# miguelmartin75/txt2vid

Measured on AMD Instinct MI355X. Metric: TGANv2 GAN train throughput (G+D steps x global batch), 16x64x64 videos/sec, higher is better.
Workload: dtype f32; 1 GPU; BASELINE configs[1]: unconditional TGANv2 16x64x64x1, per-GPU batch 32, fp32, RSGAN + GP 0.5, Adam 2e-4 (0.5,0.999), 1 D + 1 G step, subsample_input pyramid 8/16/32/64; global_batch=32, per_gpu_batch=32, parallelism=dp1

## Files before the change

include/t2v_hip.h:

```cpp
#ifndef T2V_HIP_H
#define T2V_HIP_H

#include <stddef.h>
#include <stdint.h>

#ifdef __cplusplus
extern "C" {
#endif

#define T2V_OK 0
#define T2V_EINVAL (-1)
#define T2V_ELAUNCH (-2)

#define T2V_MAX_TAPS 27

typedef struct {
    int32_t N, Cin, D, H, W, Cout;
    int32_t ntaps;
    int8_t dz[T2V_MAX_TAPS], dy[T2V_MAX_TAPS], dx[T2V_MAX_TAPS];
    int8_t pad_[3];
} t2v_conv_geom;

#define T2V_MAX_GROUPS 8
typedef struct {
    const float* x;
    float* y;
    const float* mask;
    int32_t N, D, H, W;
    int32_t ntaps;
    int32_t dstride;
    int32_t ydstride;
    int32_t yoff, Dy;
    int8_t dz[T2V_MAX_TAPS], dy[T2V_MAX_TAPS], dx[T2V_MAX_TAPS], widx[T2V_MAX_TAPS];
} t2v_conv_group;

#define T2V_CONV_BIAS 1
#define T2V_CONV_RELU_IN 2
#define T2V_CONV_ACCUM 4
#define T2V_CONV_ACCUM_BIAS 16
#define T2V_CONV_BF16 32
#define T2V_CONV_MASK_OUT 8

int t2v_pack_weight(const float* w, float* wp, int Cout, int Cin, int T, const int32_t* taps, int ntaps,
                    int mode, void* stream);

int t2v_pack_weight_into(const float* w, float* wp, int Cout, int Cin, int T, const int32_t* taps, int ntaps,
                         int mode, int dst_rows, int dst_cols, int row_off, int col_off, void* stream);

typedef struct {
    const float* src;
    float* dst;
    int32_t Cout, Cin, T, ntaps, mode, dst_rows, dst_cols, row_off, col_off;
    int32_t block_begin;
    int32_t bx, by;
    int8_t taps[T2V_MAX_TAPS];
    int8_t pad_[5];
} t2v_pack_job;
int t2v_pack_job_bytes(void);
int t2v_pack_job_groups(int T, int ntaps, int mode);
int t2v_pack_multi(const void* table , int njobs, int total_blocks, void* stream);

int t2v_conv_fwd(const float* x, const float* wp, const float* bias, float* y, float* ws, const t2v_conv_geom* g,
                 int flags, void* stream);
int64_t t2v_conv_fwd_ws_floats(const t2v_conv_geom* g);

int64_t t2v_conv_wgrad_slab_floats(const t2v_conv_geom* g, int T);
int t2v_conv_wgrad(const float* x, const float* gy, float* dw, float* slab, const t2v_conv_geom* g,
                   const int32_t* taps, int T, int flags, void* stream);

int64_t t2v_conv_fwd_grouped_ws_floats(const t2v_conv_group* groups, int ngroups, int Cin, int Cout);
int t2v_conv_fwd_grouped(const t2v_conv_group* groups, int ngroups, int Cin, int Cout, const float* wp,
                         const float* bias, float* ws, int flags, void* stream);
int64_t t2v_conv_wgrad_grouped_slab_floats(const t2v_conv_group* groups, int ngroups, int Cin, int Cout, int kD,
                                           int kH, int kW);
int t2v_conv_wgrad_grouped(const t2v_conv_group* groups, int ngroups, int Cin, int Cout, int kD, int kH, int kW,
                           float* dw, float* slab, int flags, void* stream);
#define T2V_WGRAD_MAX_SRC 6
typedef struct {
    const float* slab;
    const float* bias_slab;
    int32_t ntaps, S;
    int8_t map[T2V_MAX_TAPS];
    int8_t pad_[5];
    int64_t tap_stride;
    int64_t split_stride;
} t2v_wgrad_src;
typedef struct {
    float* dw;
    float* dbias;
    int64_t CoCi;
    int32_t T, Cout, nsrc;
    int32_t accum, accum_bias;
    int32_t kind;
    int32_t block_begin, nblocks;
    int32_t tap_major;
    int32_t pad_;
    t2v_wgrad_src src[T2V_WGRAD_MAX_SRC];
} t2v_wgrad_dest;
int t2v_conv_wgrad_grouped_partial(const t2v_conv_group* groups, int ngroups, int Cin, int Cout, int kD, int kH, int kW,
                                   float* slab, int want_bias, int flags, t2v_wgrad_src* out_src, void* stream);
int t2v_wgrad_dest_bytes(void);
int t2v_wgrad_reduce_multi(const void* table , int ndest, int total_blocks, void* stream);

int t2v_conv_fwd_plan(const t2v_conv_group* groups, int ngroups, int Cin, int Cout, int flags, int32_t* out);
int t2v_conv_wgrad_plan(const t2v_conv_group* groups, int ngroups, int Cin, int Cout, int kD, int kH, int kW, int32_t* out);
int64_t t2v_conv_wgrad_grouped_bias_slab_floats(const t2v_conv_group* groups, int ngroups, int Cin, int Cout, int kD,
                                                int kH, int kW);
int t2v_conv_wgrad_grouped_bias(const t2v_conv_group* groups, int ngroups, int Cin, int Cout, int kD, int kH, int kW,
                                float* dw, float* dbias, float* slab, int flags, void* stream);

int t2v_pack_weight_bf16(const float* w, void* wpb, int Cout, int Cin, int T, const int32_t* taps, int ntaps, int mode, void* stream);
int t2v_conv_fwd_grouped_bf16_ok(const t2v_conv_group* groups, int ngroups, int Cin, int Cout);
int t2v_conv_fwd_bf16_plan(const t2v_conv_group* groups, int ngroups, int Cin, int Cout, int flags, int32_t* out);
int t2v_conv_fwd_grouped_bf16(const t2v_conv_group* groups, int ngroups, int Cin, int Cout, const void* wpb, const float* bias,
                              float* ws, int flags, void* stream);

int64_t t2v_channel_sum_ws_floats(int N, int C, int64_t S);
int t2v_channel_sum(const float* x, float* out, float* ws, int N, int C, int64_t S, int accum, void* stream);
int64_t t2v_channel_sum_grouped_ws_floats(const t2v_conv_group* groups, int ngroups, int C);
int t2v_channel_sum_grouped(const t2v_conv_group* groups, int ngroups, int C, float* out, float* ws, int accum, void* stream);

int t2v_relu(const float* x, float* y, int64_t n, void* stream);
int t2v_relu_mask(const float* g, const float* x, float* gx, int64_t n, void* stream);
int t2v_add(const float* a, const float* b, float* y, int64_t n, void* stream);
int t2v_axpby(float alpha, const float* a, float beta, const float* b, float* y, int64_t n, void* stream);
int t2v_fill(float* y, float v, int64_t n, void* stream);
int t2v_tanh(const float* x, float* y, int64_t n, void* stream);
int t2v_tanh_bwd(const float* g, const float* y, float* gx, int64_t n, void* stream);

int t2v_avgpool3d(const float* x, const float* x2, float* y, int NC, int D, int H, int W, int Do, int Ho, int Wo,
                  const int32_t k[3], const int32_t s[3], const int32_t p[3], void* stream);
int t2v_avgpool3d_bwd(const float* gy, float* gx, int NC, int D, int H, int W, int Do, int Ho, int Wo,
                      const int32_t k[3], const int32_t s[3], const int32_t p[3], void* stream);
typedef struct t2v_pool_job {
    const float* x; const float* x2; float* y;
    const float* add;
    int32_t NC, D, H, W, Do, Ho, Wo;
    int32_t k[3], s[3], p[3];
} t2v_pool_job;
int t2v_avgpool3d_multi(const t2v_pool_job* jobs, int njobs, void* stream);
int t2v_avgpool3d_bwd_multi(const t2v_pool_job* jobs, int njobs, void* stream);

int t2v_rowsum(const float* x, float* y, int64_t rows, int64_t S, void* stream);
int t2v_rowbcast(const float* g, float* gx, int64_t rows, int64_t S, void* stream);

int t2v_upsample2x(const float* x, float* y, int64_t planes, int H, int W, void* stream);
int t2v_upsample2x_bwd(const float* gy, float* gx, int64_t planes, int H, int W, void* stream);
int t2v_upsample2x_add(const float* x, const float* h, float* y, int64_t planes, int H, int W, void* stream);

int64_t t2v_bn_ws_floats(int N, int C, int64_t S);
int t2v_bn_plan(int N, int C, int64_t S, int32_t* out );
int t2v_bn_stats(const float* x, float* stats, float* running_mean, float* running_var, float* ws, int N, int C,
                 int64_t S, float momentum, float eps, void* stream);
int t2v_bn_apply(const float* x, const float* stats, const float* gamma, const float* beta, float* y,
                 int N, int C, int64_t S, int relu, void* stream);
// ... 281 lines not shown
```

txt2vid_amd/_lib.py:

```python
import ctypes as C
import os

_HERE = os.path.dirname(os.path.abspath(__file__))
LIB_PATH = os.environ.get('T2V_LIB') or os.path.join(_HERE, 'csrc', 'libt2v_hip.so')

MAX_TAPS = 27


class ConvGeom(C.Structure):
    _fields_ = [('N', C.c_int32), ('Cin', C.c_int32), ('D', C.c_int32), ('H', C.c_int32), ('W', C.c_int32),
                ('Cout', C.c_int32), ('ntaps', C.c_int32),
                ('dz', C.c_int8 * MAX_TAPS), ('dy', C.c_int8 * MAX_TAPS), ('dx', C.c_int8 * MAX_TAPS),
                ('pad_', C.c_int8 * 3)]


class ConvGroup(C.Structure):
    _fields_ = [('x', C.c_void_p), ('y', C.c_void_p), ('mask', C.c_void_p), ('N', C.c_int32), ('D', C.c_int32), ('H', C.c_int32), ('W', C.c_int32),
                ('ntaps', C.c_int32), ('dstride', C.c_int32), ('ydstride', C.c_int32), ('yoff', C.c_int32), ('Dy', C.c_int32),
                ('dz', C.c_int8 * MAX_TAPS), ('dy', C.c_int8 * MAX_TAPS), ('dx', C.c_int8 * MAX_TAPS), ('widx', C.c_int8 * MAX_TAPS)]


class AdamJob(C.Structure):
    _fields_ = [('p', C.c_void_p), ('g', C.c_void_p), ('m', C.c_void_p), ('v', C.c_void_p), ('n', C.c_int64)]

# ... 11 lines not shown


class PoolJob(C.Structure):
    _fields_ = [('x', C.c_void_p), ('x2', C.c_void_p), ('y', C.c_void_p), ('add', C.c_void_p), ('NC', C.c_int32), ('D', C.c_int32), ('H', C.c_int32),
                ('W', C.c_int32), ('Do', C.c_int32), ('Ho', C.c_int32), ('Wo', C.c_int32), ('k', C.c_int32 * 3), ('s', C.c_int32 * 3),
                ('p', C.c_int32 * 3)]


class PoolBoxJob(C.Structure):
    _fields_ = [('in_', C.c_void_p), ('mask', C.c_void_p), ('out', C.c_void_p), ('bias', C.c_void_p), ('NC', C.c_int32), ('D', C.c_int32),
                ('H', C.c_int32), ('W', C.c_int32), ('tmode', C.c_int32), ('relu', C.c_int32), ('scale', C.c_float), ('C', C.c_int32)]


class MultiJob(C.Structure):
    _fields_ = [('a', C.c_void_p), ('b', C.c_void_p), ('c', C.c_void_p), ('out', C.c_void_p), ('out2', C.c_void_p), ('n', C.c_int64),
                ('d0', C.c_int32), ('d1', C.c_int32), ('d2', C.c_int32), ('f0', C.c_int32), ('f1', C.c_int32), ('reserved', C.c_int32)]


class PackJob(C.Structure):
    _fields_ = [('src', C.c_void_p), ('dst', C.c_void_p), ('Cout', C.c_int32), ('Cin', C.c_int32), ('T', C.c_int32),
                ('ntaps', C.c_int32), ('mode', C.c_int32), ('dst_rows', C.c_int32), ('dst_cols', C.c_int32),
                ('row_off', C.c_int32), ('col_off', C.c_int32), ('block_begin', C.c_int32), ('bx', C.c_int32), ('by', C.c_int32),
                ('taps', C.c_int8 * MAX_TAPS), ('pad_', C.c_int8 * 5)]


WGRAD_MAX_SRC = 6


class WgradSrc(C.Structure):
    _fields_ = [('slab', C.c_void_p), ('bias_slab', C.c_void_p), ('ntaps', C.c_int32), ('S', C.c_int32),
                ('map', C.c_int8 * MAX_TAPS), ('pad_', C.c_int8 * 5), ('tap_stride', C.c_int64), ('split_stride', C.c_int64)]


class WgradDest(C.Structure):
    _fields_ = [('dw', C.c_void_p), ('dbias', C.c_void_p), ('CoCi', C.c_int64), ('T', C.c_int32), ('Cout', C.c_int32),
                ('nsrc', C.c_int32), ('accum', C.c_int32), ('accum_bias', C.c_int32), ('kind', C.c_int32),
                ('block_begin', C.c_int32), ('nblocks', C.c_int32), ('tap_major', C.c_int32), ('pad_', C.c_int32),
                ('src', WgradSrc * WGRAD_MAX_SRC)]


class AugMember(C.Structure):
    _fields_ = [('x', C.c_void_p), ('y', C.c_void_p), ('u', C.c_void_p), ('N', C.c_int32), ('C', C.c_int32), ('T', C.c_int32),
                ('S', C.c_int32), ('row_stride', C.c_int32), ('rows', C.c_int32), ('policy', C.c_int32), ('reserved', C.c_int32)]


class AdaLevel(C.Structure):
    _fields_ = [('real', C.c_void_p), ('fake', C.c_void_p), ('count', C.c_int32), ('reserved', C.c_int32)]


class LecamGrad(C.Structure):
    _fields_ = [('real', C.c_void_p), ('fake', C.c_void_p), ('d_real', C.c_void_p), ('d_fake', C.c_void_p), ('count', C.c_int32),
                ('reserved', C.c_int32)]


class ProjMember(C.Structure):
    _fields_ = [('g', C.c_void_p), ('f', C.c_void_p), ('s', C.c_void_p), ('base', C.c_void_p), ('out', C.c_void_p), ('b', C.c_int32),
                ('reserved', C.c_int32)]


class MbstdMember(C.Structure):
    _fields_ = [('f', C.c_void_p), ('g', C.c_void_p * 2), ('base', C.c_void_p * 2), ('gam', C.c_void_p), ('y', C.c_void_p * 2),
                ('stat', C.c_void_p), ('out', C.c_void_p), ('b', C.c_int32), ('seg', C.c_int32)]


MAX_GROUPS = 8
_P = C.c_void_p
_I = C.c_int
_L = C.c_int64
_F = C.c_float
_I3 = C.POINTER(C.c_int32)
_G = C.POINTER(ConvGeom)

SIGNATURES = {
    't2v_pack_weight': [_P, _P, _I, _I, _I, _I3, _I, _I, _P],
    't2v_pack_job_bytes': [],
    't2v_pack_multi': [_P, _I, _I, _P],
    't2v_pack_job_groups': [_I, _I, _I],
    't2v_pack_weight_into': [_P, _P, _I, _I, _I, _I3, _I, _I, _I, _I, _I, _I, _P],
    't2v_conv_fwd': [_P, _P, _P, _P, _P, _G, _I, _P],
    't2v_conv_fwd_ws_floats': [_G],
    't2v_conv_wgrad_slab_floats': [_G, _I],
    't2v_conv_fwd_grouped_ws_floats': [_P, _I, _I, _I],
    't2v_conv_fwd_grouped': [_P, _I, _I, _I, _P, _P, _P, _I, _P],
    't2v_conv_wgrad_grouped_slab_floats': [_P, _I, _I, _I, _I, _I, _I],
    't2v_conv_fwd_plan': [_P, _I, _I, _I, _I, _I3],
    't2v_nonlocal_ok': [_I, _I],
    't2v_nonlocal_fwd': [_P, _P, _P, _P, _P, _I, _I, _I, _I, _I, _P],
    't2v_nonlocal_bwd': [_P, _P, _P, _P, _P, _P, _P, _P, _P, _P, _I, _I, _I, _I, _I, _P],
    't2v_conv_wgrad_grouped_partial': [_P, _I, _I, _I, _I, _I, _I, _P, _I, _I, _P, _P],
    't2v_wgrad_dest_bytes': [],
    't2v_wgrad_reduce_multi': [_P, _I, _I, _P],
    't2v_conv_wgrad_plan': [_P, _I, _I, _I, _I, _I, _I, _I3],
    't2v_pack_weight_bf16': [_P, _P, _I, _I, _I, _P, _I, _I, _P],
    't2v_conv_fwd_grouped_bf16_ok': [_P, _I, _I, _I],
    't2v_conv_fwd_bf16_plan': [_P, _I, _I, _I, _I, _I3],
    't2v_conv_fwd_grouped_bf16': [_P, _I, _I, _I, _P, _P, _P, _I, _P],
    't2v_conv_wgrad_grouped': [_P, _I, _I, _I, _I, _I, _I, _P, _P, _I, _P],
    't2v_conv_wgrad_grouped_bias_slab_floats': [_P, _I, _I, _I, _I, _I, _I],
    't2v_conv_wgrad_grouped_bias': [_P, _I, _I, _I, _I, _I, _I, _P, _P, _P, _I, _P],
    't2v_conv_wgrad': [_P, _P, _P, _P, _G, _I3, _I, _I, _P],
    't2v_channel_sum_ws_floats': [_I, _I, _L],
    't2v_channel_sum': [_P, _P, _P, _I, _I, _L, _I, _P],
    't2v_channel_sum_grouped_ws_floats': [_P, _I, _I],
    't2v_channel_sum_grouped': [_P, _I, _I, _P, _P, _I, _P],
    't2v_relu': [_P, _P, _L, _P],
    't2v_relu_mask': [_P, _P, _P, _L, _P],
    't2v_add': [_P, _P, _P, _L, _P],
    't2v_axpby': [_F, _P, _F, _P, _P, _L, _P],
    't2v_fill': [_P, _F, _L, _P],
    't2v_tanh': [_P, _P, _L, _P],
    't2v_tanh_bwd': [_P, _P, _P, _L, _P],
    't2v_avgpool3d': [_P, _P, _P, _I, _I, _I, _I, _I, _I, _I, _I3, _I3, _I3, _P],
    't2v_avgpool3d_bwd': [_P, _P, _I, _I, _I, _I, _I, _I, _I, _I3, _I3, _I3, _P],
    't2v_avgpool3d_multi': [_P, _I, _P],
    't2v_avgpool3d_bwd_multi': [_P, _I, _P],
    't2v_rowsum': [_P, _P, _L, _L, _P],
    't2v_rowbcast': [_P, _P, _L, _L, _P],
    't2v_upsample2x': [_P, _P, _L, _I, _I, _P],
    't2v_upsample2x_bwd': [_P, _P, _L, _I, _I, _P],
    't2v_upsample2x_add': [_P, _P, _P, _L, _I, _I, _P],
    't2v_rsgan_mean_multi': [_P, _I, _P, _P],
    't2v_rsgan_mean_multi_bwd': [_P, _I, _P, _P],
    't2v_bn_ws_floats': [_I, _I, _L],
    't2v_bn_plan': [_I, _I, _L, _I3],
    't2v_bn_stats': [_P, _P, _P, _P, _P, _I, _I, _L, _F, _F, _P],
    't2v_bn_apply': [_P, _P, _P, _P, _P, _I, _I, _L, _I, _P],
    't2v_bn_bwd': [_P, _P, _P, _P, _P, _P, _P, _P, _P, _I, _I, _L, _I, _P],
    't2v_bn_train_fwd': [_P, _P, _P, _P, _P, _P, _P, _P, _I, _I, _L, _F, _F, _I, _P, _P],
    't2v_bn_train_bwd': [_P, _P, _P, _P, _P, _P, _P, _P, _P, _I, _I, _L, _I, _P],
    't2v_bn_train_fwd_up': [_P, _P, _P, _P, _P, _P, _P, _P, _I, _I, _I, _I, _F, _F, _I, _P, _P],
    't2v_bn_train_bwd_up': [_P, _P, _P, _P, _P, _P, _P, _P, _P, _I, _I, _I, _I, _I, _P],
    't2v_bn_train_bwd_add': [_P, _P, _P, _P, _P, _P, _P, _P, _P, _P, _I, _I, _I, _I, _I, _I, _P],
    't2v_bn_eval': [_P, _P, _P, _P, _P, _P, _I, _I, _L, _F, _I, _P],
    't2v_cbn_ws_floats': [_I, _I, _L],
    't2v_cbn_train_fwd': [_P] * 9 + [_I] * 9 + [_F, _F, _I, _P, _P],
    't2v_cbn_train_fwd_up': [_P] * 9 + [_I] * 9 + [_F, _F, _I, _P, _P],
    't2v_cbn_train_bwd': [_P] * 11 + [_I] * 9 + [_I, _P],
    't2v_cbn_train_bwd_up': [_P] * 11 + [_I] * 9 + [_I, _P],
    't2v_cbn_train_bwd_add': [_P] * 12 + [_I] * 9 + [_I, _I, _P],
    't2v_cbn_eval': [_P] * 7 + [_I] * 9 + [_F, _I, _P],
    't2v_lstm_gates': [_P, _P, _P, _P, _P, _I, _L, _P],
    't2v_lstm_gates_bwd': [_P, _P, _P, _P, _P, _P, _P, _I, _L, _P],
    't2v_skinny_gemm_splits': [_I, _I, _I],
    't2v_skinny_gemm_slab': [_P, _P, _P, _I, _I, _I, _P],
    't2v_lstm_gates_slab': [_P, _I, _P, _P, _P, _P, _P, _I, _I, _P],
    't2v_lstm_gates_bwd_slab': [_P, _P, _I, _P, _P, _P, _P, _P, _P, _I, _I, _P],
    't2v_concat4': [_P, _P, _P, _P, _P, _I, _P],
    't2v_lstm_step_fused_ok': [_I, _I, _I],
    't2v_lstm_pack_major': [_P, _P, _I, _I, _P],
    't2v_lstm_step_fused': [_P, _P, _P, _P, _P, _P, _P, _I, _I, _I, _P],
    't2v_lstm_step_bwd_fused': [_P, _P, _P, _P, _P, _P, _P, _P, _P, _I, _I, _P],
    't2v_lstm_pack_cols': [_P, _P, _I, _I, _P],
    't2v_bmm': [_P, _P, _P, _I, _I, _I, _I, _I, _I, _I, _P],
    't2v_lstm_seq_step': [_P, _L, _P, _P, _P, _P, _P, _P, _L, _P, _I, _I, _I, _P],
    't2v_lstm_seq_step2': [_P, _P, _L, _L, _P, _I, _I, _P],
    't2v_lstm_train_step': [_P, _L, _P, _P, _L, _P, _L, _P, _L, _P, _L, _P, _L, _P, _L, _P, _I, _I, _I, _P],
    't2v_lstm_train_step_bwd': [_P, _L, _P, _L, _I, _P, _P, _P, _P, _L, _P, _L, _P, _L, _P, _L, _P, _I, _I, _I, _I, _I, _P],
    't2v_embedding_bwd': [_P, _P, _P, _L, _I, _I, _P],
    't2v_xent_fwd': [_P, _P, _P, _P, _L, _I, _P],
    't2v_xent_bwd': [_P, _P, _P, _P, _P, _L, _I, _P],
    't2v_argmax_rows': [_P, _P, _L, _I, _P],
    't2v_multi_ws_floats': [_I, _P, _I],
    't2v_multi': [_I, _P, _I, _P, _P, _P],
    't2v_rsgan': [_P, _P, _P, _I, _P],
    't2v_rsgan_bwd': [_P, _P, _P, _P, _P, _I, _P],
    't2v_gan_loss': [_P, _P, _P, _I, _I, _I, _I, _F, _P],
# ... 104 lines not shown
```

txt2vid_amd/csrc/conv.hip:

```cpp
#include <hip/hip_runtime.h>
#include <stdint.h>
#include "../../include/t2v_hip.h"

typedef float f32x16 __attribute__((ext_vector_type(16)));

#ifdef T2V_STAMPS
__device__ unsigned long long* g_stamps = nullptr;
__device__ unsigned int g_stamps_cap = 0;
extern "C" int t2v_stamps_set(void* buf, unsigned int cap_records) {
    if (hipMemcpyToSymbol(HIP_SYMBOL(g_stamps), &buf, sizeof(buf)) != hipSuccess) return -1;
    if (hipMemcpyToSymbol(HIP_SYMBOL(g_stamps_cap), &cap_records, sizeof(cap_records)) != hipSuccess) return -1;
    return 0;
}
__device__ __forceinline__ unsigned long long stamp_now() {
    unsigned long long t;
    __builtin_amdgcn_sched_barrier(0);
    asm volatile("s_memtime %0\n\ts_waitcnt lgkmcnt(0)" : "=s"(t) :: "memory");
    __builtin_amdgcn_sched_barrier(0);
    return t;
}
#define STAMP(v) const unsigned long long v = stamp_now()
#define STAMP_ACC(acc, a, b) acc += (b) - (a)
#else
#define STAMP(v)
// ... 206 lines not shown
    }
}

__global__ __launch_bounds__(256) void pack_weight_kernel(const float* __restrict__ w, void* __restrict__ wp,
                                                          int Cout, int Cin, int T, TapList taps, int mode, int dst_rows,
                                                          int dst_cols, int row_off, int col_off) {
    __shared__ float lds[32 * PK_PITCH];
    __shared__ int s_taps[T2V_MAX_TAPS];
    if ((int)threadIdx.x < taps.n) s_taps[threadIdx.x] = taps.t[threadIdx.x];
    __syncthreads();
    const int bx = (Cin + 31) / 32, by = (Cout + 31) / 32;
    const int b = blockIdx.x;
    pack_tile(lds, w, wp, Cout, Cin, T, taps.n, s_taps, mode, dst_rows, dst_cols, row_off, col_off, b % bx, (b / bx) % by, b / (bx * by));
}

extern "C" int t2v_pack_weight_into(const float* w, float* wp, int Cout, int Cin, int T, const int32_t* taps, int ntaps,
                                    int mode, int dst_rows, int dst_cols, int row_off, int col_off, void* stream) {
    if (!w || !wp || ntaps < 1 || ntaps > T2V_MAX_TAPS || T > T2V_MAX_TAPS || row_off < 0 || col_off < 0) return T2V_EINVAL;
    if ((mode & ~8) != 0 && (mode & ~8) != 1) return T2V_EINVAL;
    const int rows = (mode & 7) ? Cout : Cin, cols = (mode & 7) ? Cin : Cout;
    if (row_off + rows > dst_rows || col_off + cols > dst_cols) return T2V_EINVAL;
    TapList tl;
    tl.n = ntaps;
    for (int i = 0; i < ntaps; ++i) {
        if (taps[i] < 0 || taps[i] >= T) return T2V_EINVAL;
        tl.t[i] = taps[i];
    }
    const long nb = (long)((Cin + 31) / 32) * ((Cout + 31) / 32) * pack_job_groups(T, ntaps, mode);
    if (nb > 0x7fffffffL) return T2V_EINVAL;
    T2V_LAUNCH(pack_weight_kernel, dim3((unsigned)nb), dim3(256), 0, (hipStream_t)stream, w, (void*)wp, Cout, Cin, T, tl, mode, dst_rows,
               dst_cols, row_off, col_off);
    return launch_status();
}

extern "C" int t2v_pack_weight(const float* w, float* wp, int Cout, int Cin, int T, const int32_t* taps, int ntaps,
                               int mode, void* stream) {
    return t2v_pack_weight_into(w, wp, Cout, Cin, T, taps, ntaps, mode, (mode & 7) ? Cout : Cin, (mode & 7) ? Cin : Cout, 0, 0, stream);
}


struct PackJob {
    const float* src;
    float* dst;
    int32_t Cout, Cin, T, ntaps, mode, dst_rows, dst_cols, row_off, col_off, block_begin, bx, by;
    int8_t taps[T2V_MAX_TAPS];
    int8_t pad_[5];
};

__global__ __launch_bounds__(256) void pack_multi_kernel(const PackJob* __restrict__ table, int njobs) {
    __shared__ float lds[32 * PK_PITCH];
    __shared__ PackJob job;
    if (threadIdx.x == 0) {
        int lo = 0, hi = njobs - 1;
        while (lo < hi) {
            const int mid = (lo + hi + 1) >> 1;
            if (table[mid].block_begin <= (int)blockIdx.x) lo = mid; else hi = mid - 1;
        }
        job = table[lo];
    }
    __syncthreads();
    const int b = (int)blockIdx.x - __builtin_amdgcn_readfirstlane(job.block_begin);
    const int bx = __builtin_amdgcn_readfirstlane(job.bx), by = __builtin_amdgcn_readfirstlane(job.by);
    const int bxi = b % bx, byi = (b / bx) % by, z = b / (bx * by);
    pack_tile(lds, job.src, job.dst, __builtin_amdgcn_readfirstlane(job.Cout), __builtin_amdgcn_readfirstlane(job.Cin),
              __builtin_amdgcn_readfirstlane(job.T), __builtin_amdgcn_readfirstlane(job.ntaps), job.taps,
              __builtin_amdgcn_readfirstlane(job.mode), job.dst_rows, job.dst_cols, job.row_off, job.col_off, bxi, byi, z);
}

extern "C" int t2v_pack_job_bytes(void) { return (int)sizeof(PackJob); }

extern "C" int t2v_pack_multi(const void* table, int njobs, int total_blocks, void* stream) {
    if (!table || njobs < 1 || total_blocks < 1) return T2V_EINVAL;
    T2V_LAUNCH(pack_multi_kernel, dim3((unsigned)total_blocks), dim3(256), 0, (hipStream_t)stream, (const PackJob*)table, njobs);
    return launch_status();
}

struct GroupTable {
    t2v_conv_group g[T2V_MAX_GROUPS];
    int32_t tile_start[T2V_MAX_GROUPS + 1];
    int64_t out_start[T2V_MAX_GROUPS + 1];
    int32_t n;
};

template <int NCO, int NM, int WCO, int WM>
__device__ __forceinline__ void igemm_epilogue(f32x16 (&acc)[NCO][NM], const GroupTable& tab, const int gi, const t2v_conv_group& gd,
                                               const float* __restrict__ bias, float* __restrict__ slab, const int Cout,
                                               const int flags, const int nsplit, const int m0, const int co0, const int M,
                                               const int DHW, const int wm, const int wco, const int l31, const int hi,
                                               const int yds = 1, const int yoff = 0, const int DHWy = 0, const int HW = 1) {
    const bool split = nsplit > 1;
    const bool has_bias = !split && (flags & T2V_CONV_BIAS) && bias != nullptr;
    const bool accum = !split && (flags & T2V_CONV_ACCUM);
    const bool mask_out = !split && (flags & T2V_CONV_MASK_OUT) && gd.mask != nullptr;
    float* out = split ? slab + (size_t)blockIdx.z * (size_t)tab.out_start[tab.n] + (size_t)tab.out_start[gi] : gd.y;
#pragma unroll
    for (int j = 0; j < NM; ++j) {
        const int m = m0 + wm * WM + j * 32 + l31;
        if (m >= M) continue;
        const int n = m / DHW;
        int sp = m - n * DHW;
        int cs = DHW;
        if (yds == 2) {
            const int e = sp / HW;
            sp += (e + yoff) * HW;
            cs = DHWy;
        }
        float* py = out + (size_t)n * Cout * cs + sp;
        if (mask_out) {
            const float* pm = gd.mask + (size_t)n * Cout * cs + sp;
#pragma unroll
            for (int i = 0; i < NCO; ++i) {
                float mv[16];
#pragma unroll
                for (int r = 0; r < 16; ++r) {
                    const int co = co0 + wco * WCO + i * 32 + (r & 3) + 8 * (r >> 2) + 4 * hi;
                    mv[r] = pm[(size_t)(co < Cout ? co : Cout - 1) * cs];
                }
#pragma unroll
                for (int r = 0; r < 16; ++r) {
                    const int co = co0 + wco * WCO + i * 32 + (r & 3) + 8 * (r >> 2) + 4 * hi;
                    const float v = acc[i][j][r] + (has_bias ? bias[co < Cout ? co : 0] : 0.f);
                    if (co < Cout) py[(size_t)co * cs] = mv[r] > 0.f ? v : 0.f;
                }
            }
        } else if (!accum) {
#pragma unroll
            for (int i = 0; i < NCO; ++i) {
#pragma unroll
                for (int r = 0; r < 16; ++r) {
                    const int co = co0 + wco * WCO + i * 32 + (r & 3) + 8 * (r >> 2) + 4 * hi;
                    if (co < Cout) py[(size_t)co * cs] = acc[i][j][r] + (has_bias ? bias[co] : 0.f);
                }
            }
        } else {
#pragma unroll
            for (int i = 0; i < NCO; ++i) {
#pragma unroll
                for (int r = 0; r < 16; ++r) {
                    const int co = co0 + wco * WCO + i * 32 + (r & 3) + 8 * (r >> 2) + 4 * hi;
                    if (co < Cout) py[(size_t)co * cs] += acc[i][j][r] + (has_bias ? bias[co] : 0.f);
                }
            }
        }
    }
}


template <int BM, int BN, int WAVES_CO, int BKT, bool FAST, bool VECB>
__global__ __launch_bounds__(256) void conv_igemm_kernel(const GroupTable tab, const float* __restrict__ wp,
                                                         const float* __restrict__ bias, float* __restrict__ slab,
                                                         const int Cin, const int Cout, const int flags, const int nsplit) {
    constexpr int WAVES_M = 4 / WAVES_CO;
    constexpr int WCO = BN / WAVES_CO;
    constexpr int WM = BM / WAVES_M;
    constexpr int NCO = WCO / 32, NM = WM / 32;
    constexpr int LA = BKT * BM / 256;
    constexpr int KSA = 256 / BM;
    constexpr int LB = BKT * BN / 256;
    constexpr int KSB = 256 / BN;
    constexpr int NV = BKT * BN / 4;
    constexpr int LBV = NV >= 256 ? NV / 256 : 1;
    constexpr int KSBV = 1024 / BN;
    static_assert(NCO >= 1 && NM >= 1 && LA >= 1 && LB >= 1, "tile");

    __shared__ __attribute__((aligned(16))) float As[2 * BKT * BM];
    __shared__ __attribute__((aligned(16))) float Bs[2 * BKT * BN];
    __shared__ int s_off[T2V_MAX_TAPS];
    __shared__ int s_widx[T2V_MAX_TAPS];

    const int tid = threadIdx.x;
    const int lane = tid & 63, wave = tid >> 6;
    const int l31 = lane & 31, hi = lane >> 5;
    const int wco = wave % WAVES_CO, wm = wave / WAVES_CO;

    const int tile = xcd_remap((int)blockIdx.x, (int)gridDim.x);
    int gi = 0;
#pragma unroll
    for (int k = 1; k < T2V_MAX_GROUPS; ++k)
        if (k < tab.n && tile >= tab.tile_start[k]) gi = k;
    const t2v_conv_group& gd = tab.g[gi];
    const float* __restrict__ x = gd.x;
    const int D = gd.D, H = gd.H, W = gd.W;
    const int HW = H * W, DHW = D * HW;
    const int M = gd.N * DHW;
    const int m0 = (tile - tab.tile_start[gi]) * BM, co0 = blockIdx.y * BN;
    const int ntaps = gd.ntaps;

    const int lane_t = lane < ntaps ? lane : 0;
    const int tab_tdz = gd.dz[lane_t], tab_tdy = gd.dy[lane_t], tab_tdx = gd.dx[lane_t];
    if (tid < ntaps) {
        s_off[tid] = tab_tdz * HW + tab_tdy * W + tab_tdx;
        s_widx[tid] = gd.widx[tid];
    }

    const int ma_l = tid % BM, ka_l = tid / BM;
    const int m_a = m0 + ma_l;
    uint32_t tapmask = 0;
    size_t xbase = 0;
    if (m_a < M) {
        int n = m_a / DHW, sp = m_a - n * DHW;
        int d = sp / HW, r = sp - d * HW;
        int h = r / W, w_ = r - h * W;
        xbase = (size_t)n * Cin * DHW + sp;
        for (int t = 0; t < ntaps; ++t) {
            int dd = d + __builtin_amdgcn_readlane(tab_tdz, t), hh = h + __builtin_amdgcn_readlane(tab_tdy, t),
                ww = w_ + __builtin_amdgcn_readlane(tab_tdx, t);
            if ((unsigned)dd < (unsigned)D && (unsigned)hh < (unsigned)H && (unsigned)ww < (unsigned)W) tapmask |= 1u << t;
        }
    }
    const int cob_l = tid % BN, kb_l = tid / BN;
    const int cv_l = (tid % (BN / 4)) * 4, kv_l = tid / (BN / 4);
    const bool vact = (NV >= 256) || (tid < NV);
    const bool co_ok = VECB ? (vact && (co0 + cv_l) < Cout) : (co0 + cob_l) < Cout;
    const bool relu_in = flags & T2V_CONV_RELU_IN;

    f32x16 acc[NCO][NM];
#pragma unroll
    for (int i = 0; i < NCO; ++i)
#pragma unroll
        for (int j = 0; j < NM; ++j)
#pragma unroll
            for (int r = 0; r < 16; ++r) acc[i][j][r] = 0.f;

    float ra[LA];
    float rb[VECB ? 1 : LB];
    float4 rbv[VECB ? LBV : 1];
    const int Ktot = ntaps * Cin;
    const int nchunks = FAST ? ntaps * (Cin / BKT) : (Ktot + BKT - 1) / BKT;
    const int cps = (nchunks + nsplit - 1) / nsplit;
    const int q0 = blockIdx.z * cps;
    int q1 = q0 + cps;
    if (q1 > nchunks) q1 = nchunks;
    __syncthreads();

// ... 19 lines not shown
                for (int j = 0; j < LB; ++j) rb[j] = pw[(size_t)j * KSB * Cout];
            }
        } else {
            pend_a = 0;
#pragma unroll
            for (int j = 0; j < LA; ++j) {
                const int kk = q * BKT + ka_l + j * KSA;
                const int kc = kk < Ktot ? kk : Ktot - 1;
                const int tt = kc / Cin, ci = kc - tt * Cin;
                const bool v = kk < Ktot && ((tapmask >> tt) & 1u);
                pend_a |= (v ? 1u : 0u) << j;
                const ptrdiff_t off = v ? (ptrdiff_t)s_off[tt] : 0;
                ra[j] = x[xbase + off + (size_t)ci * DHW];
            }
#pragma unroll
            for (int j = 0; j < LB; ++j) {
                const int kk = q * BKT + kb_l + j * KSB;
                const int kc = kk < Ktot ? kk : Ktot - 1;
                const int tt = kc / Cin, ci = kc - tt * Cin;
                rb[j] = wp[((size_t)s_widx[tt] * Cin + ci) * Cout + (co_ok ? co0 + cob_l : 0)];
            }
        }
    };

    int t_cur = 0, c_cur = 0;
    if (FAST) {
        const int cpt = Cin / BKT;
        t_cur = q0 / cpt;
        c_cur = (q0 - t_cur * cpt) * BKT;
    }
    auto advance = [&]() {
        c_cur += BKT;
        if (FAST && c_cur >= Cin) { c_cur = 0; ++t_cur; }
    };
    auto stage = [&](int b) {
        float* as = As + b * (BKT * BM);
        float* bs = Bs + b * (BKT * BN);
#pragma unroll
        for (int j = 0; j < LA; ++j) {
            float val = ((pend_a >> j) & 1u) ? ra[j] : 0.f;
            as[(ka_l + j * KSA) * BM + ma_l] = relu_in ? fmaxf(val, 0.f) : val;
        }
        if (VECB) {
#pragma unroll
            for (int j = 0; j < LBV; ++j)
                if (vact) *reinterpret_cast<float4*>(&bs[(kv_l + j * KSBV) * BN + cv_l]) = co_ok ? rbv[j] : make_float4(0.f, 0.f, 0.f, 0.f);
        } else {
#pragma unroll
            for (int j = 0; j < LB; ++j) bs[(kb_l + j * KSB) * BN + cob_l] = co_ok ? rb[j] : 0.f;
        }
    };
    int cur = 0;
    if (q0 < q1) {
        load_chunk(q0, t_cur, c_cur);
        stage(0);
        __syncthreads();
        if (q0 + 1 < q1) { advance(); load_chunk(q0 + 1, t_cur, c_cur); }
    }
    for (int q = q0; q < q1; ++q) {
        const float* as = As + cur * (BKT * BM);
        const float* bs = Bs + cur * (BKT * BN);
        __builtin_amdgcn_s_setprio(1);
#pragma unroll
        for (int k2 = 0; k2 < BKT / 2; ++k2) {
            float a[NCO], b[NM];
            const int krow = k2 * 2 + hi;
#pragma unroll
            for (int i = 0; i < NCO; ++i) a[i] = bs[krow * BN + wco * WCO + i * 32 + l31];
#pragma unroll
            for (int j = 0; j < NM; ++j) b[j] = as[krow * BM + wm * WM + j * 32 + l31];
#pragma unroll
            for (int i = 0; i < NCO; ++i)
#pragma unroll
                for (int j = 0; j < NM; ++j)
                    acc[i][j] = __builtin_amdgcn_mfma_f32_32x32x2f32(a[i], b[j], acc[i][j], 0, 0, 0);
        }
        __builtin_amdgcn_s_setprio(0);
        if (q + 1 < q1 && !dbg_nostage) stage(cur ^ 1);
        __syncthreads();
        if (q + 2 < q1) { advance(); load_chunk(q + 2, t_cur, c_cur); }
        cur ^= 1;
    }

    igemm_epilogue<NCO, NM, WCO, WM>(acc, tab, gi, gd, bias, slab, Cout, flags, nsplit, m0, co0, M, DHW, wm, wco, l31, hi);
}

template <int BM, int BN, int WAVES_CO, int BKT, bool VECB>
__global__ __launch_bounds__(256) void conv_igemm_strip_kernel(const GroupTable tab, const float* __restrict__ wp,
                                                               const float* __restrict__ bias, float* __restrict__ slab,
                                                               const int Cin, const int Cout, const int flags, const int nsplit) {
    constexpr int WAVES_M = 4 / WAVES_CO;
    constexpr int WCO = BN / WAVES_CO;
    constexpr int WM = BM / WAVES_M;
    constexpr int NCO = WCO / 32, NM = WM / 32;
    constexpr int AP = BM + 4;
    constexpr int LA = BKT * BM / 256;
    constexpr int KSA = 256 / BM;
    constexpr int LB = BKT * BN / 256;
    constexpr int KSB = 256 / BN;
    constexpr int NV = BKT * BN / 4;
    constexpr int LBV = NV >= 256 ? NV / 256 : 1;
    constexpr int KSBV = 1024 / BN;
    static_assert(NCO >= 1 && NM >= 1 && LA >= 1 && LB >= 1 && 2 * BKT <= 256, "tile");

    __shared__ __attribute__((aligned(16))) float As[2 * BKT * AP];
    __shared__ __attribute__((aligned(16))) float Bs[2 * BKT * BN];

    const int tid = threadIdx.x;
    const int lane = tid & 63, wave = tid >> 6;
    const int l31 = lane & 31, hi = lane >> 5;
    const int wco = wave % WAVES_CO, wm = (wave / WAVES_CO) % WAVES_M;

    const int tile = xcd_remap((int)blockIdx.x, (int)gridDim.x);
    int gi = 0;
#pragma unroll
    for (int k = 1; k < T2V_MAX_GROUPS; ++k)
        if (k < tab.n && tile >= tab.tile_start[k]) gi = k;
    const t2v_conv_group& gd = tab.g[gi];
    const int D = gd.D, H = gd.H, W = gd.W;
    const int HW = H * W, DHW = D * HW;
    const int M = gd.N * DHW;
    const int m0 = (tile - tab.tile_start[gi]) * BM, co0 = blockIdx.y * BN;
    const int ntaps = gd.ntaps;
    const int ndx = gd.dx[0] < 0 ? 3 : 1;
    const int nrow = ntaps / ndx;

    const int lane_r = lane < nrow ? lane : 0, lane_t = lane < ntaps ? lane : 0;
    const int tab_rdz = gd.dz[lane_r * ndx], tab_rdy = gd.dy[lane_r * ndx];
    const int tab_roff = (tab_rdz * HW + tab_rdy * W) * 4;
    const int tab_widx = gd.widx[lane_t];
    const __amdgpu_buffer_rsrc_t rx = __builtin_amdgcn_make_buffer_rsrc((void*)gd.x, 0, (int)((uint32_t)M * (uint32_t)Cin * 4u), 0x00020000);
    const __amdgpu_buffer_rsrc_t rw = __builtin_amdgcn_make_buffer_rsrc((void*)wp, 0, -1, 0x00020000);

    const int ma_l = tid % BM, ka_l = tid / BM;
    const int he = tid / BKT, hk = tid % BKT;
    const bool halo_thread = tid < 2 * BKT;
    uint32_t rowmask = 0, rowmask_h = 0;
    uint32_t xbase = 0, xbase_h = 0;
    {
        const int m_a = m0 + ma_l;
        if (m_a < M) {
            const int n = m_a / DHW, sp = m_a - n * DHW;
            const int d = sp / HW, r = sp - d * HW;
            const int h = r / W;
            xbase = (uint32_t)n * (uint32_t)Cin * (uint32_t)DHW + (uint32_t)sp;
            for (int t = 0; t < nrow; ++t) {
                const int dd = d + __builtin_amdgcn_readlane(tab_rdz, t), hh = h + __builtin_amdgcn_readlane(tab_rdy, t);
                if ((unsigned)dd < (unsigned)D && (unsigned)hh < (unsigned)H) rowmask |= 1u << t;
            }
        }
        const int m_h = he ? m0 + BM : m0 - 1;
        if (halo_thread && m_h >= 0 && m_h < M) {
            const int n = m_h / DHW, sp = m_h - n * DHW;
            const int d = sp / HW, r = sp - d * HW;
            const int h = r / W;
            xbase_h = (uint32_t)n * (uint32_t)Cin * (uint32_t)DHW + (uint32_t)sp;
            for (int t = 0; t < nrow; ++t) {
                const int dd = d + __builtin_amdgcn_readlane(tab_rdz, t), hh = h + __builtin_amdgcn_readlane(tab_rdy, t);
                if ((unsigned)dd < (unsigned)D && (unsigned)hh < (unsigned)H) rowmask_h |= 1u << t;
            }
        }
    }
    bool can_l[NM], can_r[NM];
#pragma unroll
    for (int j = 0; j < NM; ++j) {
        const int m = m0 + wm * WM + j * 32 + l31;
        const int w_ = m % W;
        can_l[j] = w_ > 0;
        can_r[j] = w_ < W - 1;
    }
    const int cob_l = tid % BN, kb_l = tid / BN;
    const int cv_l = (tid % (BN / 4)) * 4, kv_l = tid / (BN / 4);
    const bool vact = (NV >= 256) || (tid < NV);
// ... 42 lines not shown
                ra[j] = __builtin_bit_cast(float, __builtin_amdgcn_raw_buffer_load_b32(rx, vo, sx + j * (KSA * 4) * DHW, 0));
            if (halo_thread) {
                pend_hv = (rowmask_h >> r_cur) & 1u;
                rah = __builtin_bit_cast(float, __builtin_amdgcn_raw_buffer_load_b32(rx, xoff_h + (pend_hv ? (uint32_t)roff : 0u), sx, 0));
            }
        }
        const int t = r_cur * ndx + d_cur;
        const int sw = (__builtin_amdgcn_readlane(tab_widx, t) * Cin + c0) * Cout * 4;
        if (VECB) {
#pragma unroll
            for (int j = 0; j < LBV; ++j)
                rbv[j] = __builtin_bit_cast(float4, __builtin_amdgcn_raw_buffer_load_b128(rw, woff, sw + j * (KSBV * 4) * Cout, 0));
        } else {
#pragma unroll
            for (int j = 0; j < LB; ++j)
                rb[j] = __builtin_bit_cast(float, __builtin_amdgcn_raw_buffer_load_b32(rw, woff, sw + j * (KSB * 4) * Cout, 0));
        }
    };
    auto stage = [&](int ab, int bb) {
        if (pend_has_a) {
            float* as = As + ab * (BKT * AP);
#pragma unroll
            for (int j = 0; j < LA; ++j) {
                as[(ka_l + j * KSA) * AP + 1 + ma_l] = pend_av ? fmaxf(ra[j], relu_floor) : 0.f;
            }
            if (halo_thread) {
                as[hk * AP + (he ? BM + 1 : 0)] = pend_hv ? fmaxf(rah, relu_floor) : 0.f;
            }
        }
        float* bs = Bs + bb * (BKT * BN);
        if (VECB) {
#pragma unroll
            for (int j = 0; j < LBV; ++j)
                if (vact) *reinterpret_cast<float4*>(&bs[(kv_l + j * KSBV) * BN + cv_l]) = co_ok ? rbv[j] : make_float4(0.f, 0.f, 0.f, 0.f);
        } else {
#pragma unroll
            for (int j = 0; j < LB; ++j) bs[(kb_l + j * KSB) * BN + cob_l] = co_ok ? rb[j] : 0.f;
        }
    };

    int acur = 0, bcur = 0, dx_now = 0;
    if (q0 < q1) {
        load_chunk(true);
        stage(0, 0);
        dx_now = pend_dx;
        __syncthreads();
        if (q0 + 1 < q1) { advance(); load_chunk(false); }
    }
    for (int q = q0; q < q1; ++q) {
        const float* as = As + acur * (BKT * AP) + 1 + dx_now + wm * WM + l31;
        const float* bs = Bs + bcur * (BKT * BN) + wco * WCO + l31;
        bool keep[NM];
#pragma unroll
        for (int j = 0; j < NM; ++j) keep[j] = dx_now < 0 ? can_l[j] : (dx_now > 0 ? can_r[j] : true);
        __builtin_amdgcn_s_setprio(1);
#pragma unroll
        for (int k2 = 0; k2 < BKT / 2; ++k2) {
            float a[NCO], b[NM];
            const int krow = k2 * 2 + hi;
#pragma unroll
            for (int i = 0; i < NCO; ++i) a[i] = bs[krow * BN + i * 32];
#pragma unroll
            for (int j = 0; j < NM; ++j) {
                const float v = as[krow * AP + j * 32];
                b[j] = keep[j] ? v : 0.f;
            }
#pragma unroll
            for (int i = 0; i < NCO; ++i)
#pragma unroll
                for (int j = 0; j < NM; ++j)
                    acc[i][j] = __builtin_amdgcn_mfma_f32_32x32x2f32(a[i], b[j], acc[i][j], 0, 0, 0);
        }
        __builtin_amdgcn_s_setprio(0);
        const bool more = q + 1 < q1;
        const bool next_a = more && pend_has_a;
        int dx_next = dx_now;
        if (more) { stage(acur ^ 1, bcur ^ 1); dx_next = pend_dx; }
        __syncthreads();
        if (q + 2 < q1) { advance(); load_chunk(false); }
        bcur ^= 1;
        if (next_a) acur ^= 1;
        dx_now = dx_next;
    }
    igemm_epilogue<NCO, NM, WCO, WM>(acc, tab, gi, gd, bias, slab, Cout, flags, nsplit, m0, co0, M, DHW, wm, wco, l31, hi);
}

#ifndef DB_STAGE_LATE
#define DB_STAGE_LATE 1
#endif
template <int BM, int BKT, int WAVES_CO, bool VECB, bool DB = false>
__global__ __launch_bounds__(256, ((BM == 256 || (DB && BKT == 32)) ? 2 : (DB ? 4 : 3))) void conv_igemm_strip3_kernel(const GroupTable tab, const float* __restrict__ wp,
                                                                const float* __restrict__ bias, float* __restrict__ slab,
                                                                const int Cin, const int Cout, const int flags, const int nsplit) {
#ifdef T2V_STAMPS
    const unsigned long long t_real = __builtin_amdgcn_s_memrealtime();
#endif
    STAMP(t_entry);
    constexpr int BN = 64, WAVES_M = 4 / WAVES_CO;
    constexpr int WCO = BN / WAVES_CO, WM = BM / WAVES_M;
    constexpr int NCO = WCO / 32, NM = WM / 32;
    constexpr int AP = BM + 4;
    constexpr int LA = BKT * BM / 256;
    constexpr int KSA = 256 / BM;
    constexpr int NV = BKT * BN / 4;
    constexpr int LBV = NV / 256;
    constexpr int KSBV = 1024 / BN;
    constexpr int LB = BKT * BN / 256;
    constexpr int KSB = 256 / BN;
    static_assert(NCO >= 1 && NM >= 1 && LA >= 1 && LBV >= 1 && 2 * BKT <= 256, "tile");

    __shared__ __attribute__((aligned(16))) float As[(DB ? 2 : 1) * BKT * AP];
    __shared__ __attribute__((aligned(16))) float Bs[(DB ? 2 : 1) * 3 * BKT * BN];

    const int tid = threadIdx.x;
    const int lane = tid & 63, wave = tid >> 6;
    const int l31 = lane & 31, hi = lane >> 5;
    const int wco = wave % WAVES_CO, wm = wave / WAVES_CO;

    const int tile = xcd_remap((int)blockIdx.x, (int)gridDim.x);
    int gi = 0;
#pragma unroll
    for (int k = 1; k < T2V_MAX_GROUPS; ++k)
        if (k < tab.n && tile >= tab.tile_start[k]) gi = k;
    const t2v_conv_group& gd = tab.g[gi];
    const int D = gd.D, H = gd.H, W = gd.W;
    const int HW = H * W, DHW = D * HW;
    const int ds = gd.dstride == 2 ? 2 : 1;
    const int yds = gd.ydstride == 2 ? 2 : 1;
    const int Do = yds == 2 ? (gd.Dy + 1 - gd.yoff) / 2 : (ds == 2 ? (D + 1) / 2 : D);
    const int DHWo = Do * HW;
    const int M = gd.N * DHWo;
    const int m0 = (tile - tab.tile_start[gi]) * BM, co0 = blockIdx.y * BN;
    const int ntaps = gd.ntaps;
    const int ndx = gd.dx[0] < 0 ? 3 : 1;
    const int nrow = ntaps / ndx;

    const int lane_r = lane < nrow ? lane : 0, lane_t = lane < ntaps ? lane : 0;
    const int tab_rdz = gd.dz[lane_r * ndx], tab_rdy = gd.dy[lane_r * ndx];
    const int tab_roff = (tab_rdz * HW + tab_rdy * W) * 4;
    const int tab_widx = gd.widx[lane_t];
    const __amdgpu_buffer_rsrc_t rx = __builtin_amdgcn_make_buffer_rsrc((void*)gd.x, 0, (int)((uint32_t)(gd.N * DHW) * (uint32_t)Cin * 4u), 0x00020000);
    const __amdgpu_buffer_rsrc_t rw = __builtin_amdgcn_make_buffer_rsrc((void*)wp, 0, -1, 0x00020000);

    const int ma_l = tid % BM, ka_l = tid / BM;
    const int he = tid / BKT, hk = tid % BKT;
    const bool halo_thread = tid < 2 * BKT;
    uint32_t rowmask = 0, rowmask_h = 0;
    uint32_t xbase = 0, xbase_h = 0;
    {
        const int m_a = m0 + ma_l;
        if (m_a < M) {
            const int n = m_a / DHWo, spo = m_a - n * DHWo;
            const int d_o = spo / HW, r = spo - d_o * HW;
            const int d = d_o * ds, sp = d * HW + r;
            const int h = r / W;
            xbase = (uint32_t)n * (uint32_t)Cin * (uint32_t)DHW + (uint32_t)sp;
            for (int t = 0; t < nrow; ++t) {
                const int dd = d + __builtin_amdgcn_readlane(tab_rdz, t), hh = h + __builtin_amdgcn_readlane(tab_rdy, t);
                if ((unsigned)dd < (unsigned)D && (unsigned)hh < (unsigned)H) rowmask |= 1u << t;
            }
        }
        const int m_h = he ? m0 + BM : m0 - 1;
        if (halo_thread && m_h >= 0 && m_h < M) {
            const int n = m_h / DHWo, spo = m_h - n * DHWo;
            const int d_o = spo / HW, r = spo - d_o * HW;
            const int d = d_o * ds, sp = d * HW + r;
            const int h = r / W;
            xbase_h = (uint32_t)n * (uint32_t)Cin * (uint32_t)DHW + (uint32_t)sp;
            for (int t = 0; t < nrow; ++t) {
                const int dd = d + __builtin_amdgcn_readlane(tab_rdz, t), hh = h + __builtin_amdgcn_readlane(tab_rdy, t);
                if ((unsigned)dd < (unsigned)D && (unsigned)hh < (unsigned)H) rowmask_h |= 1u << t;
            }
        }
    }
    bool can_l[NM], can_r[NM];
#pragma unroll
// ... 47 lines not shown
            l_sx[st] = c0 * DHW * 4;
            pav[st] = (rowmask >> r_cur) & 1u;
            phv[st] = halo_thread && ((rowmask_h >> r_cur) & 1u);
            l_vo[st] = xoff + (pav[st] ? (uint32_t)roff : 0u);
            l_vh[st] = xoff_hd + (phv[st] ? (uint32_t)roff : 0u);
#pragma unroll
            for (int d = 0; d < 3; ++d) l_sw[st][d] = (__builtin_amdgcn_readlane(tab_widx, r_cur * 3 + d) * Cin + c0) * Cout * 4;
        };
        auto load_item = [&](int st, int i) {
            if (i < LA) ra2[st][i] = __builtin_bit_cast(float, __builtin_amdgcn_raw_buffer_load_b32(rx, l_vo[st], l_sx[st] + i * (KSA * 4) * DHW, 0));
            else if (i == LA) rah2[st] = __builtin_bit_cast(float, __builtin_amdgcn_raw_buffer_load_b32(rx, l_vh[st], l_sx[st], 0));
            else if (i < LA + 1 + 3 * LBV) {
                const int e = i - LA - 1, d = e / LBV, j = e - d * LBV;
                rb2[st][e] = __builtin_bit_cast(float4, __builtin_amdgcn_raw_buffer_load_b128(rw, woff, l_sw[st][d] + j * (KSBV * 4) * Cout, 0));
            }
        };
        auto stage_item = [&](int st, float* A, float* B, int i) {
            if (i < LA) A[(ka_l + i * KSA) * AP + 1 + ma_l] = pav[st] ? fmaxf(ra2[st][i], relu_floor) : 0.f;
            else if (i == LA) A[halo_row * AP + halo_col] = phv[st] ? fmaxf(rah2[st], relu_floor) : 0.f;
            else if (i < LA + 1 + 3 * LBV) {
                const int e = i - LA - 1, d = e / LBV, j = e - d * LBV;
                *reinterpret_cast<float4*>(&B[d * (BKT * BN) + (kv_l + j * KSBV) * BN + cv_l]) = co_ok ? rb2[st][e] : make_float4(0.f, 0.f, 0.f, 0.f);
            }
        };
        const float* a_tap[3][NM];
#pragma unroll
        for (int d = 0; d < 3; ++d)
#pragma unroll
            for (int j = 0; j < NM; ++j) {
                const bool keep = d == 0 ? can_l[j] : (d == 2 ? can_r[j] : true);
                a_tap[d][j] = keep ? As + d + wm * WM + j * 32 + l31 : As + (BM + 3);
            }
        auto round = [&](auto CUR, int q) {
            constexpr int cur = decltype(CUR)::value, nxt = cur ^ 1;
            prep(cur, q + 2);
            const float* Ab = As + cur * ASZ;
            const float* Bb = Bs + cur * BSZ + wco * WCO + l31;
            float* An = As + nxt * ASZ;
            float* Bn = Bs + nxt * BSZ;
#pragma unroll
            for (int d = 0; d < 3; ++d) {
#pragma unroll
                for (int k2 = 0; k2 < BKT / 2; ++k2) {
                    const int krow = k2 * 2 + hi, slot = d * (BKT / 2) + k2;
                    float a[NCO], b[NM];
#pragma unroll
                    for (int i = 0; i < NCO; ++i) a[i] = Bb[d * (BKT * BN) + krow * BN + i * 32];
#pragma unroll
                    for (int j = 0; j < NM; ++j) b[j] = (a_tap[d][j] + cur * ASZ)[krow * AP];
#pragma unroll
                    for (int i = 0; i < NCO; ++i)
#pragma unroll
                        for (int j = 0; j < NM; ++j) acc[i][j] = __builtin_amdgcn_mfma_f32_32x32x2f32(a[i], b[j], acc[i][j], 0, 0, 0);
                    constexpr int SS = DB_STAGE_LATE ? NSLOT - HS : HS;
#pragma unroll
                    for (int e = 0; e < IPS; ++e) {
                        if (slot < HS) load_item(cur, slot * IPS + e);
                        else if (slot >= SS && slot < SS + HS) stage_item(nxt, An, Bn, (slot - SS) * IPS + e);
                    }
                    if (slot == HS - 1 || slot == SS - 1 || slot == SS + HS - 1) __builtin_amdgcn_sched_barrier(0);
                }
            }
            (void)Ab;
            __syncthreads();
        };
        if (tid < BKT) { As[tid * AP + BM + 3] = 0.f; As[ASZ + tid * AP + BM + 3] = 0.f; }
        if (q0 < q1) {
            prep(0, q0);
#pragma unroll
            for (int i = 0; i < NI; ++i) load_item(0, i);
            prep(1, q0 + 1);
#pragma unroll
            for (int i = 0; i < NI; ++i) load_item(1, i);
#pragma unroll
            for (int i = 0; i < NI; ++i) stage_item(0, As, Bs, i);
        }
        __syncthreads();
        __builtin_amdgcn_s_setprio(1);
        for (int q = q0; q < q1; q += 2) {
            round(std::integral_constant<int, 0>{}, q);
            if (q + 1 < q1) round(std::integral_constant<int, 1>{}, q + 1);
        }
        __builtin_amdgcn_s_setprio(0);
        igemm_epilogue<NCO, NM, WCO, WM>(acc, tab, gi, gd, bias, slab, Cout, flags, nsplit, m0, co0, M, DHWo, wm, wco, l31, hi, yds, gd.yoff,
                                         gd.Dy * HW, HW);
        return;
    }
    float ra[LA], rah = 0.f;
    float rb[VECB ? 1 : 3 * LB];
    float4 rbv[VECB ? 3 * LBV : 1];
    const int ncb = Cin / BKT;
    const int nrounds = nrow * ncb;
    const int rps = (nrounds + nsplit - 1) / nsplit;
    const int q0 = blockIdx.z * rps;
    int q1 = q0 + rps;
    if (q1 > nrounds) q1 = nrounds;
    bool pend_av = false, pend_hv = false;

    auto load_round = [&](int q) {
        const int r_cur = q / ncb, cb = q - r_cur * ncb;
        const int c0 = cb * BKT;
        const int roff = __builtin_amdgcn_readlane(tab_roff, r_cur);
        const int sx = c0 * DHW * 4;
        pend_av = (rowmask >> r_cur) & 1u;
        const uint32_t vo = xoff + (pend_av ? (uint32_t)roff : 0u);
#pragma unroll
        for (int j = 0; j < LA; ++j)
            ra[j] = __builtin_bit_cast(float, __builtin_amdgcn_raw_buffer_load_b32(rx, vo, sx + j * (KSA * 4) * DHW, 0));
        if (halo_thread) {
            pend_hv = (rowmask_h >> r_cur) & 1u;
            rah = __builtin_bit_cast(float, __builtin_amdgcn_raw_buffer_load_b32(rx, xoff_h + (pend_hv ? (uint32_t)roff : 0u), sx, 0));
        }
#pragma unroll
        for (int d = 0; d < 3; ++d) {
            if (d < ndx) {
                const int sw = (__builtin_amdgcn_readlane(tab_widx, r_cur * ndx + d) * Cin + c0) * Cout * 4;
                if (VECB) {
#pragma unroll
                    for (int j = 0; j < LBV; ++j)
                        rbv[d * LBV + j] = __builtin_bit_cast(float4, __builtin_amdgcn_raw_buffer_load_b128(rw, woff, sw + j * (KSBV * 4) * Cout, 0));
                } else {
#pragma unroll
                    for (int j = 0; j < LB; ++j)
                        rb[d * LB + j] = __builtin_bit_cast(float, __builtin_amdgcn_raw_buffer_load_b32(rw, woff, sw + j * (KSB * 4) * Cout, 0));
                }
            }
        }
    };
    auto stage = [&]() {
#pragma unroll
        for (int j = 0; j < LA; ++j) As[(ka_l + j * KSA) * AP + 1 + ma_l] = pend_av ? fmaxf(ra[j], relu_floor) : 0.f;
        if (halo_thread) As[hk * AP + (he ? BM + 1 : 0)] = pend_hv ? fmaxf(rah, relu_floor) : 0.f;
#pragma unroll
        for (int d = 0; d < 3; ++d) {
            if (d < ndx) {
                float* bs = Bs + d * (BKT * BN);
                if (VECB) {
#pragma unroll
                    for (int j = 0; j < LBV; ++j)
                        *reinterpret_cast<float4*>(&bs[(kv_l + j * KSBV) * BN + cv_l]) = co_ok ? rbv[d * LBV + j] : make_float4(0.f, 0.f, 0.f, 0.f);
                } else {
#pragma unroll
                    for (int j = 0; j < LB; ++j) bs[(kb_l + j * KSB) * BN + cob_l] = co_ok ? rb[d * LB + j] : 0.f;
                }
            }
        }
    };

    if (tid < BKT) As[tid * AP + BM + 3] = 0.f;
    if (q0 < q1) load_round(q0);
#ifdef T2V_STAMPS
    unsigned long long st_stage = 0, st_bar1 = 0, st_load = 0, st_mfma = 0, st_bar2 = 0;
#endif
#ifdef T2V_ABLATION
    const bool ab_noload = flags & 64, ab_nostage = flags & 128, ab_nobar = flags & 256, ab_nomfma = flags & 512, ab_nostore = flags & 1024;
#else
    constexpr bool ab_noload = false, ab_nostage = false, ab_nobar = false, ab_nomfma = false, ab_nostore = false;
#endif
    STAMP(t_loop0);
    for (int q = q0; q < q1; ++q) {
        STAMP(ta);
        if (!ab_nostage || q == q0) stage();
        STAMP(tb);
        if (!ab_nobar || q == q0) __syncthreads();
        STAMP(tc);
        if (q + 1 < q1 && !ab_noload) load_round(q + 1);
        STAMP(td);
        __builtin_amdgcn_s_setprio(1);
#pragma unroll
        for (int d = 0; d < 3; ++d) {
            if (d < ndx && !ab_nomfma) {
                const int dx = ndx == 3 ? d - 1 : 0;
                const float* bs = Bs + d * (BKT * BN) + wco * WCO + l31;
                const float* as[NM];
#pragma unroll
                for (int j = 0; j < NM; ++j) {
                    const bool keep = dx < 0 ? can_l[j] : (dx > 0 ? can_r[j] : true);
                    as[j] = keep ? As + 1 + dx + wm * WM + j * 32 + l31 : As + (BM + 3);
                }
#pragma unroll
                for (int k2 = 0; k2 < BKT / 2; ++k2) {
                    const int krow = k2 * 2 + hi;
                    float a[NCO], b[NM];
#pragma unroll
                    for (int i = 0; i < NCO; ++i) a[i] = bs[krow * BN + i * 32];
#pragma unroll
                    for (int j = 0; j < NM; ++j) b[j] = as[j][krow * AP];
#pragma unroll
                    for (int i = 0; i < NCO; ++i)
#pragma unroll
                        for (int j = 0; j < NM; ++j)
                            acc[i][j] = __builtin_amdgcn_mfma_f32_32x32x2f32(a[i], b[j], acc[i][j], 0, 0, 0);
                }
            }
        }
        __builtin_amdgcn_s_setprio(0);
        STAMP(te);
        if (!ab_nobar) __syncthreads();
        STAMP(tf);
        STAMP_ACC(st_stage, ta, tb); STAMP_ACC(st_bar1, tb, tc); STAMP_ACC(st_load, tc, td); STAMP_ACC(st_mfma, td, te); STAMP_ACC(st_bar2, te, tf);
    }
    STAMP(t_loop1);
    if (ab_nostore && acc[0][0][0] != 12345.678f) return;
    igemm_epilogue<NCO, NM, WCO, WM>(acc, tab, gi, gd, bias, slab, Cout, flags, nsplit, m0, co0, M, DHWo, wm, wco, l31, hi, yds, gd.yoff,
                                     gd.Dy * HW, HW);
#ifdef T2V_STAMPS
    {
        STAMP(t_exit);
        const unsigned int rec = ((blockIdx.z * gridDim.y + blockIdx.y) * gridDim.x + blockIdx.x) * 4 + wave;
        if (g_stamps && rec < g_stamps_cap && lane == 0) {
            unsigned long long* o = g_stamps + (size_t)rec * 16;
            o[0] = t_entry; o[1] = t_loop0; o[2] = t_loop1; o[3] = t_exit;
            o[4] = st_stage; o[5] = st_bar1; o[6] = st_load; o[7] = st_mfma; o[8] = st_bar2;
            o[9] = (unsigned long long)(q1 - q0);
            o[10] = __builtin_amdgcn_s_getreg((4) | (0 << 6) | (31 << 11));
            o[11] = __builtin_amdgcn_s_getreg((20) | (0 << 6) | (31 << 11));
            o[12] = t_real;
            o[13] = (unsigned long long)gi;
            o[14] = __builtin_amdgcn_s_memrealtime();
        }
    }
#endif
}

template <int BM, bool DB = false>
__global__ __launch_bounds__(256, 3) void conv_pool_fwd_kernel(const GroupTable tab, const float* __restrict__ wp,
                                                               const float* __restrict__ bias, float* __restrict__ slab,
                                                               const int Cin, const int Cout, const int flags, const int nsplit) {
    constexpr bool VECB = true;
    constexpr int BN = 64, BKT = DB ? 16 : 32, WAVES_CO = 2, WAVES_M = 2;
    constexpr int WCO = BN / WAVES_CO, WM = BM / WAVES_M;
    constexpr int NCO = WCO / 32, NM = WM / 32;
    constexpr int AP = BM + 4;
    constexpr int LA = BKT * BM / 256;
    constexpr int KSA = 256 / BM;
    constexpr int NV = BKT * BN / 4;
    constexpr int LBV = NV / 256;
    constexpr int KSBV = 1024 / BN;
    constexpr int LB = BKT * BN / 256;
    constexpr int KSB = 256 / BN;
    static_assert(NCO == 1 && NM >= 1 && LA >= 1 && LBV >= 1, "tile");

    __shared__ __attribute__((aligned(16))) float As[(DB ? 2 : 1) * 3 * BKT * AP];
    __shared__ __attribute__((aligned(16))) float Bs[(DB ? 2 : 1) * 3 * BKT * BN];

    const int tid = threadIdx.x;
    const int lane = tid & 63, wave = tid >> 6;
    const int l31 = lane & 31, hi = lane >> 5;
    const int wco = wave % WAVES_CO, wm = wave / WAVES_CO;

    const int tile = xcd_remap((int)blockIdx.x, (int)gridDim.x);
    int gi = 0;
#pragma unroll
    for (int k = 1; k < T2V_MAX_GROUPS; ++k)
        if (k < tab.n && tile >= tab.tile_start[k]) gi = k;
    const t2v_conv_group& gd = tab.g[gi];
    const int tm = gd.dstride;
    const int Dn = tm ? gd.D / 2 : 1, Hn = gd.H / 2, Wn = gd.W / 2;
    const int Hp = gd.H + 1, Wp = gd.W + 2, Dp = tm ? gd.D + 1 : 1;
    const int Vp = Dp * Hp * Wp;
    const int HWn = Hn * Wn, DHWn = Dn * HWn;
    const int M = gd.N * DHWn;
    const int m0 = (tile - tab.tile_start[gi]) * BM, co0 = blockIdx.y * BN;
    const int ntaps = gd.ntaps;
    const int nrow = ntaps / 3;

    const int lane_r = lane < nrow ? lane : 0, lane_t = lane < ntaps ? lane : 0;
    const int tab_roff = ((tm ? gd.dz[lane_r * 3] + 1 : 0) * Hp + gd.dy[lane_r * 3] + 1) * Wp * 4;
    const int tab_widx = gd.widx[lane_t];
    const __amdgpu_buffer_rsrc_t rx = __builtin_amdgcn_make_buffer_rsrc((void*)gd.x, 0, (int)((uint32_t)(gd.N * Vp) * (uint32_t)Cin * 4u), 0x00020000);
    const __amdgpu_buffer_rsrc_t rw = __builtin_amdgcn_make_buffer_rsrc((void*)wp, 0, -1, 0x00020000);

    const int ma_l = tid % BM, ka_l = tid / BM;
    uint32_t xbase = 0;
    {
        const int m_a = m0 + ma_l;
        if (m_a < M) {
            const int n = m_a / DHWn, sp = m_a - n * DHWn;
            const int e = sp / HWn, r = sp - e * HWn;
            const int i = r / Wn, j = r - i * Wn;
            xbase = (uint32_t)n * (uint32_t)Cin * (uint32_t)Vp + (uint32_t)(((tm ? 2 * e : 0) * Hp + 2 * i) * Wp + 2 * j);
        }
    }
    const int cob_l = tid % BN, kb_l = tid / BN;
    const int cv_l = (tid % (BN / 4)) * 4, kv_l = tid / (BN / 4);
    const bool co_ok = VECB ? (co0 + cv_l) < Cout : (co0 + cob_l) < Cout;
    const uint32_t xoff = (xbase + (uint32_t)ka_l * (uint32_t)Vp) * 4u;
    const uint32_t woff = co_ok ? (uint32_t)((VECB ? kv_l : kb_l) * Cout + co0 + (VECB ? cv_l : cob_l)) * 4u : 0u;

    f32x16 acc[NM];
#pragma unroll
    for (int j = 0; j < NM; ++j)
#pragma unroll
        for (int r = 0; r < 16; ++r) acc[j][r] = 0.f;

    if constexpr (DB) {
        static_assert(BM == 64 && NM == 1 && LA == 4 && LBV == 1, "double-buffered form: 64 x 64 x 16 tiles");
        constexpr int ASZ = 3 * BKT * AP, BSZ = 3 * BKT * BN;
        constexpr int NSLOT = 3 * (BKT / 2);
        constexpr int NLD = 2 * LA + 3 * LBV;
        constexpr int NST = 3 * LA + 3 * LBV;
        const int ncb = Cin / BKT;
        const int nrounds = nrow * ncb;
        const int rps = (nrounds + nsplit - 1) / nsplit;
        const int q0 = blockIdx.z * rps;
        int q1 = q0 + rps;
        if (q1 > nrounds) q1 = nrounds;
        float2 ra2[2][LA];
        float ra1[2][LA];
        float4 rb2[2][3 * LBV];
        uint32_t l_vo[2] = {0u, 0u};
        int l_sx[2] = {0, 0}, l_sw[2][3] = {{0, 0, 0}, {0, 0, 0}};
        auto prep = [&](int st, int q) {
            const int qq = q < q1 ? q : q1 - 1;
            const int r_cur = qq / ncb, cb = qq - r_cur * ncb;
            const int c0 = cb * BKT;
            l_vo[st] = xoff + (uint32_t)__builtin_amdgcn_readlane(tab_roff, r_cur);
            l_sx[st] = c0 * Vp * 4;
#pragma unroll
            for (int d = 0; d < 3; ++d) l_sw[st][d] = (__builtin_amdgcn_readlane(tab_widx, r_cur * 3 + d) * Cin + c0) * Cout * 4;
        };
        auto load_item = [&](int st, int i) {
            if (i < LA) ra2[st][i] = __builtin_bit_cast(float2, __builtin_amdgcn_raw_buffer_load_b64(rx, l_vo[st], l_sx[st] + i * (KSA * 4) * Vp, 0));
            else if (i < 2 * LA) ra1[st][i - LA] = __builtin_bit_cast(float, __builtin_amdgcn_raw_buffer_load_b32(rx, l_vo[st] + 8u, l_sx[st] + (i - LA) * (KSA * 4) * Vp, 0));
            else if (i < NLD) {
                const int d = i - 2 * LA;
                rb2[st][d] = __builtin_bit_cast(float4, __builtin_amdgcn_raw_buffer_load_b128(rw, woff, l_sw[st][d], 0));
            }
        };
        auto stage_item = [&](int st, float* A, float* B, int i) {
            if (i < 3 * LA) {
                const int j = i / 3, d = i - j * 3;
                A[d * (BKT * AP) + (ka_l + j * KSA) * AP + ma_l] = d == 0 ? ra2[st][j].x : (d == 1 ? ra2[st][j].y : ra1[st][j]);
            } else if (i < NST) {
                const int d = i - 3 * LA;
                *reinterpret_cast<float4*>(&B[d * (BKT * BN) + kv_l * BN + cv_l]) = co_ok ? rb2[st][d] : make_float4(0.f, 0.f, 0.f, 0.f);
            }
        };
        auto round = [&](auto CUR, int q) {
            constexpr int cur = decltype(CUR)::value, nxt = cur ^ 1;
            prep(cur, q + 2);
            const float* Ab = As + cur * ASZ + wm * WM + l31;
            const float* Bb = Bs + cur * BSZ + wco * WCO + l31;
            float* An = As + nxt * ASZ;
            float* Bn = Bs + nxt * BSZ;
#pragma unroll
            for (int d = 0; d < 3; ++d) {
#pragma unroll
                for (int k2 = 0; k2 < BKT / 2; ++k2) {
                    const int krow = k2 * 2 + hi, slot = d * (BKT / 2) + k2;
                    const float a = Bb[d * (BKT * BN) + krow * BN];
                    const float b = Ab[d * (BKT * AP) + krow * AP];
                    acc[0] = __builtin_amdgcn_mfma_f32_32x32x2f32(a, b, acc[0], 0, 0, 0);
                    if (2 * slot < NLD) load_item(cur, 2 * slot);
                    if (2 * slot + 1 < NLD) load_item(cur, 2 * slot + 1);
                    if (slot >= NSLOT - NST) stage_item(nxt, An, Bn, slot - (NSLOT - NST));
                    if (slot == (NLD + 1) / 2 - 1 || slot == NSLOT - NST - 1) __builtin_amdgcn_sched_barrier(0);
                }
            }
            __syncthreads();
        };
        if (q0 < q1) {
            prep(0, q0);
#pragma unroll
            for (int i = 0; i < NLD; ++i) load_item(0, i);
            prep(1, q0 + 1);
#pragma unroll
            for (int i = 0; i < NLD; ++i) load_item(1, i);
#pragma unroll
            for (int i = 0; i < NST; ++i) stage_item(0, As, Bs, i);
        }
        __syncthreads();
        __builtin_amdgcn_s_setprio(1);
        for (int q = q0; q < q1; q += 2) {
            round(std::integral_constant<int, 0>{}, q);
            if (q + 1 < q1) round(std::integral_constant<int, 1>{}, q + 1);
        }
        __builtin_amdgcn_s_setprio(0);
        f32x16 (&accd)[1][NM] = reinterpret_cast<f32x16 (&)[1][NM]>(acc);
        igemm_epilogue<1, NM, WCO, WM>(accd, tab, gi, gd, bias, slab, Cout, flags, nsplit, m0, co0, M, DHWn, wm, wco, l31, hi);
        return;
    }
    float2 ra2[LA];
    float ra1[LA];
    float rb[VECB ? 1 : 3 * LB];
    float4 rbv[VECB ? 3 * LBV : 1];
    const int ncb = Cin / BKT;
    const int nrounds = nrow * ncb;
    const int rps = (nrounds + nsplit - 1) / nsplit;
    const int q0 = blockIdx.z * rps;
    int q1 = q0 + rps;
    if (q1 > nrounds) q1 = nrounds;

    auto load_round = [&](int q) {
        const int r_cur = q / ncb, cb = q - r_cur * ncb;
        const int c0 = cb * BKT;
        const uint32_t vo = xoff + (uint32_t)__builtin_amdgcn_readlane(tab_roff, r_cur);
        const int sx = c0 * Vp * 4;
#pragma unroll
        for (int j = 0; j < LA; ++j) {
            ra2[j] = __builtin_bit_cast(float2, __builtin_amdgcn_raw_buffer_load_b64(rx, vo, sx + j * (KSA * 4) * Vp, 0));
            ra1[j] = __builtin_bit_cast(float, __builtin_amdgcn_raw_buffer_load_b32(rx, vo + 8u, sx + j * (KSA * 4) * Vp, 0));
        }
#pragma unroll
        for (int d = 0; d < 3; ++d) {
            const int sw = (__builtin_amdgcn_readlane(tab_widx, r_cur * 3 + d) * Cin + c0) * Cout * 4;
            if (VECB) {
#pragma unroll
                for (int j = 0; j < LBV; ++j)
                    rbv[d * LBV + j] = __builtin_bit_cast(float4, __builtin_amdgcn_raw_buffer_load_b128(rw, woff, sw + j * (KSBV * 4) * Cout, 0));
            } else {
#pragma unroll
                for (int j = 0; j < LB; ++j)
                    rb[d * LB + j] = __builtin_bit_cast(float, __builtin_amdgcn_raw_buffer_load_b32(rw, woff, sw + j * (KSB * 4) * Cout, 0));
            }
        }
    };
    auto stage = [&]() {
#pragma unroll
        for (int j = 0; j < LA; ++j) {
            float* a = As + (ka_l + j * KSA) * AP + ma_l;
            a[0] = ra2[j].x;
            a[BKT * AP] = ra2[j].y;
            a[2 * BKT * AP] = ra1[j];
        }
#pragma unroll
        for (int d = 0; d < 3; ++d) {
            float* bs = Bs + d * (BKT * BN);
            if (VECB) {
#pragma unroll
                for (int j = 0; j < LBV; ++j)
                    *reinterpret_cast<float4*>(&bs[(kv_l + j * KSBV) * BN + cv_l]) = co_ok ? rbv[d * LBV + j] : make_float4(0.f, 0.f, 0.f, 0.f);
            } else {
#pragma unroll
                for (int j = 0; j < LB; ++j) bs[(kb_l + j * KSB) * BN + cob_l] = co_ok ? rb[d * LB + j] : 0.f;
            }
        }
    };

    if (q0 < q1) load_round(q0);
    for (int q = q0; q < q1; ++q) {
        stage();
        __syncthreads();
        if (q + 1 < q1) load_round(q + 1);
        __builtin_amdgcn_s_setprio(1);
#pragma unroll
        for (int d = 0; d < 3; ++d) {
            const float* bs = Bs + d * (BKT * BN) + wco * WCO + l31;
            const float* as = As + d * (BKT * AP) + wm * WM + l31;
#pragma unroll
            for (int k2 = 0; k2 < BKT / 2; ++k2) {
                const int krow = k2 * 2 + hi;
                const float a = bs[krow * BN];
                float b[NM];
#pragma unroll
                for (int j = 0; j < NM; ++j) b[j] = as[krow * AP + j * 32];
#pragma unroll
                for (int j = 0; j < NM; ++j) acc[j] = __builtin_amdgcn_mfma_f32_32x32x2f32(a, b[j], acc[j], 0, 0, 0);
            }
        }
        __builtin_amdgcn_s_setprio(0);
        __syncthreads();
    }
    f32x16 (&acc2)[1][NM] = reinterpret_cast<f32x16 (&)[1][NM]>(acc);
    igemm_epilogue<1, NM, WCO, WM>(acc2, tab, gi, gd, bias, slab, Cout, flags, nsplit, m0, co0, M, DHWn, wm, wco, l31, hi);
}

template <bool DB>
__global__ __launch_bounds__(256, 3) void conv_pool_dgrad_kernel(const GroupTable tab, const float* __restrict__ wp,
                                                                 const int K, const int C) {
    constexpr bool VECB = true;
    constexpr int BM = 64, BN = 64, BKT = DB ? 16 : 32, WAVES_CO = 2;
    constexpr int WCO = 32, WM = 32;
    constexpr int AP = BM + 4;
    constexpr int LA = BKT * BM / 256;
    constexpr int KSA = 256 / BM;
    constexpr int LBV = BKT * BN / 4 / 256;
    constexpr int KSBV = 1024 / BN;
    constexpr int LB = BKT * BN / 256;
    constexpr int KSB = 256 / BN;

    __shared__ __attribute__((aligned(16))) float As[(DB ? 2 : 1) * BKT * AP];
    __shared__ __attribute__((aligned(16))) float Bs[(DB ? 2 : 1) * 3 * BKT * BN];

    const int tid = threadIdx.x;
    const int lane = tid & 63, wave = tid >> 6;
    const int l31 = lane & 31, hi = lane >> 5;
    const int wco = wave % WAVES_CO, wm = wave / WAVES_CO;

    const int tile = xcd_remap((int)blockIdx.x, (int)gridDim.x);
    int gi = 0;
#pragma unroll
    for (int k = 1; k < T2V_MAX_GROUPS; ++k)
        if (k < tab.n && tile >= tab.tile_start[k]) gi = k;
    const t2v_conv_group& gd = tab.g[gi];
    const int tm = gd.dstride;
    const int nct = (int)gridDim.y >> 2;
    const int pair = (int)blockIdx.y / nct, ct = pair >> 1, cy = pair & 1;
    if (tm == 0 && ct) return;
    const int co0 = ((int)blockIdx.y - pair * nct) * BN;
    const int Dn = tm ? gd.D / 2 : 1, Hn = gd.H / 2, Wn = gd.W / 2;
    const int Dq = tm ? Dn + 1 : 1, Hq = Hn + 1, Wq = Wn + 1;
    const int HWn = Hn * Wn, Vn = Dn * HWn;
    const int HWq = Hq * Wq, Vq = Dq * HWq;
    const int De = (tm && ct) ? Dn : Dq, He = cy ? Hn : Hq;
    const int HWe = He * Wq, Ve = De * HWe;
    const int M = gd.N * Ve;
    const int m0 = (tile - tab.tile_start[gi]) * BM;
    if (m0 >= M) return;
    const int ndz = (tm && ct == 0) ? 2 : 1, ndy = cy == 0 ? 2 : 1;
    const int nrow = ndz * ndy;
    const int lane_t = lane < 27 ? lane : 0;
    const int tab_widx = gd.widx[lane_t];
    const __amdgpu_buffer_rsrc_t rx = __builtin_amdgcn_make_buffer_rsrc((void*)gd.x, 0, (int)((uint32_t)(gd.N * Vn) * (uint32_t)K * 4u), 0x00020000);
    const __amdgpu_buffer_rsrc_t rw = __builtin_amdgcn_make_buffer_rsrc((void*)wp, 0, -1, 0x00020000);

    const int ma_l = tid % BM, ka_l = tid / BM;
    const int hk = tid % BKT;
    const bool halo_thread = tid < BKT;
    int s_at = 0, s_a = 0, s_b = Wn;
    uint32_t s_n = 0;
    int h_at = 0, h_a = 0, h_b = Wn;
    uint32_t h_n = 0;
    {
        const int m_a = m0 + ma_l;
        if (m_a < M) {
            const int n = m_a / Ve, sp = m_a - n * Ve;
            s_at = sp / HWe;
            const int r = sp - s_at * HWe;
            s_a = r / Wq;
            s_b = r - s_a * Wq;
            s_n = (uint32_t)n;
        }
        if (m0 < M) {
            const int n = m0 / Ve, sp = m0 - n * Ve;
            h_at = sp / HWe;
            const int r = sp - h_at * HWe;
            h_a = r / Wq;
            h_b = r - h_a * Wq - 1;
            h_n = (uint32_t)n;
            if (h_b < 0) h_b = Wn;
        }
    }
    bool can_l[1];
    {
        const int m = m0 + wm * WM + l31;
        can_l[0] = (m % Wq) >= 1;
    }
// ... 140 lines not shown
#pragma unroll
        for (int d = 0; d < 3; ++d) {
            const int sw = (__builtin_amdgcn_readlane(tab_widx, f0 + d) * K + c0) * C * 4;
            if (VECB) {
#pragma unroll
                for (int j = 0; j < LBV; ++j)
                    rbv[d * LBV + j] = __builtin_bit_cast(float4, __builtin_amdgcn_raw_buffer_load_b128(rw, woff, sw + j * (KSBV * 4) * C, 0));
            } else {
#pragma unroll
                for (int j = 0; j < LB; ++j)
                    rb[d * LB + j] = __builtin_bit_cast(float, __builtin_amdgcn_raw_buffer_load_b32(rw, woff, sw + j * (KSB * 4) * C, 0));
            }
        }
    };
    auto stage = [&]() {
#pragma unroll
        for (int j = 0; j < LA; ++j) As[(ka_l + j * KSA) * AP + 1 + ma_l] = pend_av ? ra[j] : 0.f;
        if (halo_thread) As[hk * AP] = pend_hv ? rah : 0.f;
#pragma unroll
        for (int d = 0; d < 3; ++d) {
            float* bs = Bs + d * (BKT * BN);
            if (VECB) {
#pragma unroll
                for (int j = 0; j < LBV; ++j)
                    *reinterpret_cast<float4*>(&bs[(kv_l + j * KSBV) * BN + cv_l]) = co_ok ? rbv[d * LBV + j] : make_float4(0.f, 0.f, 0.f, 0.f);
            } else {
#pragma unroll
                for (int j = 0; j < LB; ++j) bs[(kb_l + j * KSB) * BN + cob_l] = co_ok ? rb[d * LB + j] : 0.f;
            }
        }
    };

    if (tid < BKT) As[tid * AP + BM + 3] = 0.f;
    if (nrounds > 0) load_round(0);
    for (int q = 0; q < nrounds; ++q) {
        stage();
        __syncthreads();
        if (q + 1 < nrounds) load_round(q + 1);
        __builtin_amdgcn_s_setprio(1);
        {
            const float* a_own = As + 1 + wm * WM + l31;
            const float* a_left = can_l[0] ? As + wm * WM + l31 : As + (BM + 3);
            const float* b0 = Bs + 0 * (BKT * BN) + wco * WCO + l31;
            const float* b1 = Bs + 1 * (BKT * BN) + wco * WCO + l31;
            const float* b2 = Bs + 2 * (BKT * BN) + wco * WCO + l31;
#pragma unroll
            for (int k2 = 0; k2 < BKT / 2; ++k2) {
                const int krow = k2 * 2 + hi;
                const float xo = a_own[krow * AP], xl = a_left[krow * AP];
                acc0 = __builtin_amdgcn_mfma_f32_32x32x2f32(b0[krow * BN], xo, acc0, 0, 0, 0);
                acc1 = __builtin_amdgcn_mfma_f32_32x32x2f32(b1[krow * BN], xo, acc1, 0, 0, 0);
                acc0 = __builtin_amdgcn_mfma_f32_32x32x2f32(b2[krow * BN], xl, acc0, 0, 0, 0);
            }
        }
        __builtin_amdgcn_s_setprio(0);
        __syncthreads();
    }
    }
    const int m = m0 + wm * WM + l31;
    if (m < M) {
        const int n = m / Ve, spe = m - n * Ve;
        const int at = spe / HWe, r2 = spe - at * HWe;
        const int a = r2 / Wq, b = r2 - a * Wq;
        const int sp = (at * Hq + a) * Wq + b;
        constexpr bool row_ok = true;
        const bool ok1 = b < Wn;
        const size_t plane = (size_t)gd.N * C * Vq;
        float* p0 = gd.y + ((size_t)blockIdx.z * 8 + (size_t)((ct * 2 + cy) * 2 + 0)) * plane + (size_t)n * C * Vq + sp;
        float* p1 = p0 + plane;
#pragma unroll
        for (int r = 0; r < 16; ++r) {
            const int co = co0 + wco * WCO + (r & 3) + 8 * (r >> 2) + 4 * hi;
            if (co < C) {
                if (row_ok) p0[(size_t)co * Vq] = acc0[r];
                if (ok1) p1[(size_t)co * Vq] = acc1[r];
            }
        }
    }
}

typedef __attribute__((ext_vector_type(8))) __bf16 bf16x8;
#define B16_KP 40

template <int BM>
__global__ __launch_bounds__(256) void conv_igemm_bf16_kernel(const GroupTable tab, const __bf16* __restrict__ wpb,
                                                              const float* __restrict__ bias, float* __restrict__ slab,
                                                              const int Cin, const int Cout, const int flags, const int nsplit) {
    constexpr int BN = 64, BKT = 32, WAVES_CO = 2;
    constexpr int WAVES_M = 2;
    constexpr int WCO = BN / WAVES_CO, WM = BM / WAVES_M;
    constexpr int NCO = WCO / 32, NM = WM / 32;
    constexpr int KPT = BKT * BM / 256;
    static_assert(NCO == 1 && NM >= 1 && (KPT == 16 || KPT == 8), "tile");
    __shared__ __attribute__((aligned(16))) __bf16 Xs[2 * BM * B16_KP];
    __shared__ __attribute__((aligned(16))) __bf16 Ws[2 * BN * B16_KP];
    __shared__ int s_off[T2V_MAX_TAPS];
    __shared__ int s_widx[T2V_MAX_TAPS];

    const int tid = threadIdx.x;
    const int lane = tid & 63, wave = tid >> 6;
    const int l31 = lane & 31, hi = lane >> 5;
    const int wco = wave % WAVES_CO, wm = wave / WAVES_CO;
    const int tile = xcd_remap((int)blockIdx.x, (int)gridDim.x);
    int gi = 0;
#pragma unroll
    for (int k = 1; k < T2V_MAX_GROUPS; ++k)
        if (k < tab.n && tile >= tab.tile_start[k]) gi = k;
    const t2v_conv_group& gd = tab.g[gi];
    const float* __restrict__ x = gd.x;
    const int D = gd.D, H = gd.H, W = gd.W;
    const int HW = H * W, DHW = D * HW;
    const int M = gd.N * DHW;
    const int m0 = (tile - tab.tile_start[gi]) * BM, co0 = blockIdx.y * BN;
    const int ntaps = gd.ntaps;
    const int lane_t = lane < ntaps ? lane : 0;
    const int tab_tdz = gd.dz[lane_t], tab_tdy = gd.dy[lane_t], tab_tdx = gd.dx[lane_t];
    if (tid < ntaps) {
        s_off[tid] = tab_tdz * HW + tab_tdy * W + tab_tdx;
        s_widx[tid] = gd.widx[tid];
    }
    const int ma_l = tid % BM, kq = tid / BM;
    const int m_a = m0 + ma_l;
    uint32_t tapmask = 0;
    size_t xbase = 0;
    if (m_a < M) {
        const int n = m_a / DHW, sp = m_a - n * DHW;
        const int d = sp / HW, r = sp - d * HW;
        const int h = r / W, w_ = r - h * W;
        xbase = (size_t)n * Cin * DHW + sp;
        for (int t = 0; t < ntaps; ++t) {
            const int dd = d + __builtin_amdgcn_readlane(tab_tdz, t), hh = h + __builtin_amdgcn_readlane(tab_tdy, t),
                      ww = w_ + __builtin_amdgcn_readlane(tab_tdx, t);
            if ((unsigned)dd < (unsigned)D && (unsigned)hh < (unsigned)H && (unsigned)ww < (unsigned)W) tapmask |= 1u << t;
        }
    }
    const int wc_l = tid >> 2, wk_l = (tid & 3) * 8;
    const bool w_ok = co0 + wc_l < Cout;
    const bool relu_in = flags & T2V_CONV_RELU_IN;

    f32x16 acc[NCO][NM];
#pragma unroll
    for (int j = 0; j < NM; ++j)
#pragma unroll
        for (int r = 0; r < 16; ++r) acc[0][j][r] = 0.f;

    float ra[KPT];
    bf16x8 rw;
    bool pend_v = false;
    const int cpt = Cin / BKT;
    const int nchunks = ntaps * cpt;
    const int cps = (nchunks + nsplit - 1) / nsplit;
    const int q0 = blockIdx.z * cps;
    int q1 = q0 + cps;
    if (q1 > nchunks) q1 = nchunks;
    __syncthreads();

    int t_cur = q0 / cpt, c_cur = (q0 - t_cur * cpt) * BKT;
    auto advance = [&]() {
        c_cur += BKT;
        if (c_cur >= Cin) { c_cur = 0; ++t_cur; }
    };
    auto load_chunk = [&]() {
        pend_v = (tapmask >> t_cur) & 1u;
        const float* px = x + xbase + (pend_v ? (ptrdiff_t)s_off[t_cur] : 0) + (size_t)(c_cur + kq * KPT) * DHW;
#pragma unroll
        for (int j = 0; j < KPT; ++j) ra[j] = px[(size_t)j * DHW];
        const __bf16* pw = wpb + ((size_t)s_widx[t_cur] * Cout + (w_ok ? co0 + wc_l : 0)) * Cin + c_cur + wk_l;
        rw = *reinterpret_cast<const bf16x8*>(pw);
    };
    auto stage = [&](int b) {
        __bf16* xs = Xs + b * (BM * B16_KP) + ma_l * B16_KP + kq * KPT;
#pragma unroll
        for (int g = 0; g < KPT / 8; ++g) {
            bf16x8 v;
#pragma unroll
            for (int j = 0; j < 8; ++j) {
                float f = pend_v ? ra[g * 8 + j] : 0.f;
                if (relu_in) f = fmaxf(f, 0.f);
                v[j] = (__bf16)f;
            }
            *reinterpret_cast<bf16x8*>(xs + g * 8) = v;
        }
        bf16x8 wv = rw;
        if (!w_ok) {
#pragma unroll
            for (int j = 0; j < 8; ++j) wv[j] = (__bf16)0.f;
        }
        *reinterpret_cast<bf16x8*>(Ws + b * (BN * B16_KP) + wc_l * B16_KP + wk_l) = wv;
    };

    int cur = 0;
    if (q0 < q1) {
        load_chunk();
        stage(0);
        __syncthreads();
        if (q0 + 1 < q1) { advance(); load_chunk(); }
    }
    for (int q = q0; q < q1; ++q) {
        const __bf16* xs = Xs + cur * (BM * B16_KP) + (wm * WM + l31) * B16_KP + 8 * hi;
        const __bf16* ws = Ws + cur * (BN * B16_KP) + (wco * WCO + l31) * B16_KP + 8 * hi;
#pragma unroll
        for (int ks = 0; ks < BKT / 16; ++ks) {
            const bf16x8 a = *reinterpret_cast<const bf16x8*>(ws + ks * 16);
#pragma unroll
            for (int j = 0; j < NM; ++j) {
                const bf16x8 b = *reinterpret_cast<const bf16x8*>(xs + j * 32 * B16_KP + ks * 16);
                acc[0][j] = __builtin_amdgcn_mfma_f32_32x32x16_bf16(a, b, acc[0][j], 0, 0, 0);
            }
        }
        if (q + 1 < q1) stage(cur ^ 1);
        __syncthreads();
        if (q + 2 < q1) { advance(); load_chunk(); }
        cur ^= 1;
    }
    igemm_epilogue<NCO, NM, WCO, WM>(acc, tab, gi, gd, bias, slab, Cout, flags, nsplit, m0, co0, M, DHW, wm, wco, l31, hi);
}

template <int BM>
__global__ __launch_bounds__(256) void conv_igemm_bf16_strip3_kernel(const GroupTable tab, const __bf16* __restrict__ wpb,
                                                                     const float* __restrict__ bias, float* __restrict__ slab,
                                                                     const int Cin, const int Cout, const int flags, const int nsplit) {
    constexpr int BN = 64, BKT = 32, WAVES_CO = 2, WAVES_M = 2;
    constexpr int WCO = BN / WAVES_CO, WM = BM / WAVES_M;
    constexpr int NCO = WCO / 32, NM = WM / 32;
    constexpr int KPT = BKT * BM / 256;
    constexpr int HT = BKT / KPT;
    constexpr int ZROW = BM + 2;
    static_assert(NCO == 1 && NM >= 1 && (KPT == 16 || KPT == 8), "tile");
    __shared__ __attribute__((aligned(16))) __bf16 Xs[(BM + 3) * B16_KP];
    __shared__ __attribute__((aligned(16))) __bf16 Ws[3 * BN * B16_KP];

    const int tid = threadIdx.x;
    const int lane = tid & 63, wave = tid >> 6;
    const int l31 = lane & 31, hi = lane >> 5;
    const int wco = wave % WAVES_CO, wm = wave / WAVES_CO;
    const int tile = xcd_remap((int)blockIdx.x, (int)gridDim.x);
    int gi = 0;
#pragma unroll
    for (int k = 1; k < T2V_MAX_GROUPS; ++k)
        if (k < tab.n && tile >= tab.tile_start[k]) gi = k;
    const t2v_conv_group& gd = tab.g[gi];
    const int D = gd.D, H = gd.H, W = gd.W;
    const int HW = H * W, DHW = D * HW;
    const int ds = gd.dstride == 2 ? 2 : 1;
    const int yds = gd.ydstride == 2 ? 2 : 1;
    const int Do = yds == 2 ? (gd.Dy + 1 - gd.yoff) / 2 : (ds == 2 ? (D + 1) / 2 : D);
    const int DHWo = Do * HW;
    const int M = gd.N * DHWo;
    const int m0 = (tile - tab.tile_start[gi]) * BM, co0 = blockIdx.y * BN;
    const int ntaps = gd.ntaps;
    const int ndx = gd.dx[0] < 0 ? 3 : 1;
    const int nrow = ntaps / ndx;

    const int lane_r = lane < nrow ? lane : 0, lane_t = lane < ntaps ? lane : 0;
    const int tab_rdz = gd.dz[lane_r * ndx], tab_rdy = gd.dy[lane_r * ndx];
    const int tab_roff = (tab_rdz * HW + tab_rdy * W) * 4;
    const int tab_widx = gd.widx[lane_t];
    const __amdgpu_buffer_rsrc_t rx = __builtin_amdgcn_make_buffer_rsrc((void*)gd.x, 0, (int)((uint32_t)(gd.N * DHW) * (uint32_t)Cin * 4u), 0x00020000);
    const __amdgpu_buffer_rsrc_t rw = __builtin_amdgcn_make_buffer_rsrc((void*)wpb, 0, -1, 0x00020000);

    const int ma_l = tid % BM, kq = tid / BM;
    const bool halo_thread = tid < 2 * HT;
    const int he = tid / HT, hq = tid % HT;
    uint32_t rowmask = 0, rowmask_h = 0;
    uint32_t xbase = 0, xbase_h = 0;
    {
        const int m_a = m0 + ma_l;
        if (m_a < M) {
            const int n = m_a / DHWo, spo = m_a - n * DHWo;
            const int d_o = spo / HW, r = spo - d_o * HW;
            const int d = d_o * ds, sp = d * HW + r;
            const int h = r / W;
            xbase = (uint32_t)n * (uint32_t)Cin * (uint32_t)DHW + (uint32_t)sp;
            for (int t = 0; t < nrow; ++t) {
                const int dd = d + __builtin_amdgcn_readlane(tab_rdz, t), hh = h + __builtin_amdgcn_readlane(tab_rdy, t);
                if ((unsigned)dd < (unsigned)D && (unsigned)hh < (unsigned)H) rowmask |= 1u << t;
            }
        }
        const int m_h = he ? m0 + BM : m0 - 1;
        if (halo_thread && m_h >= 0 && m_h < M) {
            const int n = m_h / DHWo, spo = m_h - n * DHWo;
            const int d_o = spo / HW, r = spo - d_o * HW;
            const int d = d_o * ds, sp = d * HW + r;
            const int h = r / W;
            xbase_h = (uint32_t)n * (uint32_t)Cin * (uint32_t)DHW + (uint32_t)sp;
            for (int t = 0; t < nrow; ++t) {
                const int dd = d + __builtin_amdgcn_readlane(tab_rdz, t), hh = h + __builtin_amdgcn_readlane(tab_rdy, t);
                if ((unsigned)dd < (unsigned)D && (unsigned)hh < (unsigned)H) rowmask_h |= 1u << t;
            }
        }
    }
    bool can_l[NM], can_r[NM];
#pragma unroll
    for (int j = 0; j < NM; ++j) {
        const int m = m0 + wm * WM + j * 32 + l31;
        const int w_ = m % W;
        can_l[j] = w_ > 0;
        can_r[j] = w_ < W - 1;
    }
    const int wc_l = tid >> 2, wk_l = (tid & 3) * 8;
    const bool w_ok = co0 + wc_l < Cout;
    const float relu_floor = (flags & T2V_CONV_RELU_IN) ? 0.f : -__builtin_inff();
    const uint32_t xoff = (xbase + (uint32_t)(kq * KPT) * (uint32_t)DHW) * 4u, xoff_h = (xbase_h + (uint32_t)(hq * KPT) * (uint32_t)DHW) * 4u;
    const uint32_t woff = w_ok ? (uint32_t)((co0 + wc_l) * Cin + wk_l) * 2u : 0u;
// ... 7 lines not shown
    float ra[KPT], rh[KPT];
    bf16x8 rw8[3];
    const int ncb = Cin / BKT;
    const int nrounds = nrow * ncb;
    const int rps = (nrounds + nsplit - 1) / nsplit;
    const int q0 = blockIdx.z * rps;
    int q1 = q0 + rps;
    if (q1 > nrounds) q1 = nrounds;
    bool pend_av = false, pend_hv = false;

    auto load_round = [&](int q) {
        const int r_cur = q / ncb, cb = q - r_cur * ncb;
        const int c0 = cb * BKT;
        const int roff = __builtin_amdgcn_readlane(tab_roff, r_cur);
        const int sx = c0 * DHW * 4;
        pend_av = (rowmask >> r_cur) & 1u;
        const uint32_t vo = xoff + (pend_av ? (uint32_t)roff : 0u);
#pragma unroll
        for (int j = 0; j < KPT; ++j) ra[j] = __builtin_bit_cast(float, __builtin_amdgcn_raw_buffer_load_b32(rx, vo, sx + j * 4 * DHW, 0));
        if (halo_thread) {
            pend_hv = (rowmask_h >> r_cur) & 1u;
            const uint32_t vh = xoff_h + (pend_hv ? (uint32_t)roff : 0u);
#pragma unroll
            for (int j = 0; j < KPT; ++j) rh[j] = __builtin_bit_cast(float, __builtin_amdgcn_raw_buffer_load_b32(rx, vh, sx + j * 4 * DHW, 0));
        }
#pragma unroll
        for (int d = 0; d < 3; ++d) {
            if (d < ndx) {
                const int sw = (__builtin_amdgcn_readlane(tab_widx, r_cur * ndx + d) * Cout * Cin + c0) * 2;
                rw8[d] = __builtin_bit_cast(bf16x8, __builtin_amdgcn_raw_buffer_load_b128(rw, woff, sw, 0));
            }
        }
    };
    auto put_row = [&](__bf16* dst, const float* v, bool ok) {
#pragma unroll
        for (int g = 0; g < KPT / 8; ++g) {
            bf16x8 o;
#pragma unroll
            for (int j = 0; j < 8; ++j) o[j] = (__bf16)(ok ? fmaxf(v[g * 8 + j], relu_floor) : 0.f);
            *reinterpret_cast<bf16x8*>(dst + g * 8) = o;
        }
    };
    bf16x8 zero8;
#pragma unroll
    for (int j = 0; j < 8; ++j) zero8[j] = (__bf16)0.f;
    auto stage = [&]() {
        put_row(Xs + (1 + ma_l) * B16_KP + kq * KPT, ra, pend_av);
        if (halo_thread) put_row(Xs + (he ? BM + 1 : 0) * B16_KP + hq * KPT, rh, pend_hv);
#pragma unroll
        for (int d = 0; d < 3; ++d)
            if (d < ndx) *reinterpret_cast<bf16x8*>(Ws + d * (BN * B16_KP) + wc_l * B16_KP + wk_l) = w_ok ? rw8[d] : zero8;
    };

    if (tid < 4) *reinterpret_cast<bf16x8*>(Xs + ZROW * B16_KP + tid * 8) = zero8;
    if (q0 < q1) load_round(q0);
    for (int q = q0; q < q1; ++q) {
        stage();
        __syncthreads();
        if (q + 1 < q1) load_round(q + 1);
#pragma unroll
        for (int d = 0; d < 3; ++d) {
            if (d < ndx) {
                const int dx = ndx == 3 ? d - 1 : 0;
                const __bf16* ws = Ws + d * (BN * B16_KP) + (wco * WCO + l31) * B16_KP + 8 * hi;
                const __bf16* xs[NM];
#pragma unroll
                for (int j = 0; j < NM; ++j) {
                    const bool keep = dx < 0 ? can_l[j] : (dx > 0 ? can_r[j] : true);
                    xs[j] = Xs + (keep ? 1 + dx + wm * WM + j * 32 + l31 : ZROW) * B16_KP + 8 * hi;
                }
#pragma unroll
                for (int ks = 0; ks < BKT / 16; ++ks) {
                    const bf16x8 a = *reinterpret_cast<const bf16x8*>(ws + ks * 16);
#pragma unroll
                    for (int j = 0; j < NM; ++j) {
                        const bf16x8 b = *reinterpret_cast<const bf16x8*>(xs[j] + ks * 16);
                        acc[0][j] = __builtin_amdgcn_mfma_f32_32x32x16_bf16(a, b, acc[0][j], 0, 0, 0);
                    }
                }
            }
        }
        __syncthreads();
    }
    igemm_epilogue<NCO, NM, WCO, WM>(acc, tab, gi, gd, bias, slab, Cout, flags, nsplit, m0, co0, M, DHWo, wm, wco, l31, hi, yds, gd.yoff,
                                     gd.Dy * HW, HW);
}

extern "C" int t2v_pack_weight_bf16(const float* w, void* wpb, int Cout, int Cin, int T, const int32_t* taps, int ntaps, int mode,
                                    void* stream) {
    if (!w || !wpb || !taps || Cout < 1 || Cin < 1 || T < 1 || ntaps < 1 || ntaps > T2V_MAX_TAPS) return T2V_EINVAL;
    mode = mode ? 1 : 0;
    TapList tl;
    tl.n = ntaps;
    for (int i = 0; i < T2V_MAX_TAPS; ++i) tl.t[i] = i < ntaps ? taps[i] : 0;
    const long nb = (long)((Cin + 31) / 32) * ((Cout + 31) / 32) * pack_job_groups(T, ntaps, 2 + mode);
    if (nb > 0x7fffffffL) return T2V_EINVAL;
    T2V_LAUNCH(pack_weight_kernel, dim3((unsigned)nb), dim3(256), 0, (hipStream_t)stream, w, wpb, Cout, Cin, T, tl, 2 + mode,
               mode ? Cin : Cout, mode ? Cout : Cin, 0, 0);
    return launch_status();
}

__global__ __launch_bounds__(256) void splitk_reduce_kernel(const GroupTable tab, const float* __restrict__ slab,
                                                            const float* __restrict__ bias, int S, int Cout, int flags) {
    const bool has_bias = (flags & T2V_CONV_BIAS) && bias != nullptr;
    const bool accum = flags & T2V_CONV_ACCUM;
    const long total = tab.out_start[tab.n];
    for (long i = (long)blockIdx.x * 256 + threadIdx.x; i < total; i += (long)gridDim.x * 256) {
        int gi = 0;
#pragma unroll
        for (int k = 1; k < T2V_MAX_GROUPS; ++k)
            if (k < tab.n && i >= tab.out_start[k]) gi = k;
        const long li = i - tab.out_start[gi];
        float v = 0.f;
#pragma unroll 8
        for (int s = 0; s < S; ++s) v += slab[(size_t)s * total + i];
        if (has_bias) {
            const int DHW = tab.g[gi].D * tab.g[gi].H * tab.g[gi].W;
            v += bias[(li / DHW) % Cout];
        }
        float* y = tab.g[gi].y;
        if ((flags & T2V_CONV_MASK_OUT) && tab.g[gi].mask) v = tab.g[gi].mask[li] > 0.f ? v : 0.f;
        y[li] = accum ? y[li] + v : v;
    }
}


#define THIN_MAX_W 16384

template <int NC>
__global__ __launch_bounds__(256) void conv_thin_kernel(const GroupTable tab, const float* __restrict__ wp,
                                                        const float* __restrict__ bias, const int Cin, const int Cout,
                                                        const int nslots, const int flags) {
    __shared__ float sw[THIN_MAX_W];
    __shared__ int s_off[T2V_MAX_TAPS];
    __shared__ int s_widx[T2V_MAX_TAPS];
    const int tid = threadIdx.x;
    int gi = 0;
#pragma unroll
    for (int k = 1; k < T2V_MAX_GROUPS; ++k)
        if (k < tab.n && (int)blockIdx.x >= tab.tile_start[k]) gi = k;
    const t2v_conv_group& gd = tab.g[gi];
    const int D = gd.D, H = gd.H, W = gd.W, HW = H * W, DHW = D * HW;
    const int M = gd.N * DHW;
    const int ntaps = gd.ntaps;
    for (int i = tid; i < nslots * Cin * Cout; i += 256) sw[i] = wp[i];
    __shared__ int s_d3[T2V_MAX_TAPS];
    if (tid < ntaps) {
        const int dz = gd.dz[tid], dy = gd.dy[tid], dx = gd.dx[tid];
        s_off[tid] = dz * HW + dy * W + dx;
        s_d3[tid] = (dz + 1) | ((dy + 1) << 2) | ((dx + 1) << 4);
        s_widx[tid] = gd.widx[tid];
    }
    __syncthreads();
    const int m = ((int)blockIdx.x - tab.tile_start[gi]) * 256 + tid;
    if (m >= M) return;
    const int n = m / DHW, sp = m - n * DHW;
    const int d = sp / HW, r = sp - d * HW;
    const int h = r / W, w_ = r - h * W;
    const float* __restrict__ px = gd.x + (size_t)n * Cin * DHW + sp;
    const bool relu_in = flags & T2V_CONV_RELU_IN;
    float acc[NC];
#pragma unroll
    for (int c = 0; c < NC; ++c) acc[c] = 0.f;
    for (int t = 0; t < ntaps; ++t) {
        const int d3 = s_d3[t];
        const int dd = d + (d3 & 3) - 1, hh = h + ((d3 >> 2) & 3) - 1, ww = w_ + ((d3 >> 4) & 3) - 1;
        if (!((unsigned)dd < (unsigned)D && (unsigned)hh < (unsigned)H && (unsigned)ww < (unsigned)W)) continue;
// ... 280 lines not shown
#pragma unroll
    for (int t = 0; t < T2V_MAX_TAPS; ++t) {
        const bool live = t < ntaps;
        const int dd = d + __builtin_amdgcn_readlane(tab_dz, t), hh = h + __builtin_amdgcn_readlane(tab_dy, t);
        const int ww = w_ + __builtin_amdgcn_readlane(tab_dx, t);
        const bool ok = live && mv && (unsigned)dd < (unsigned)D && (unsigned)hh < (unsigned)H && (unsigned)ww < (unsigned)W;
        const int off = ok ? (dd * H + hh) * W + ww : 0;
#pragma unroll
        for (int ci = 0; ci < CIN; ++ci) {
            const float v = px[(size_t)ci * DHW + off];
            xv[t * CIN + ci] = ok ? (relu ? fmaxf(v, 0.f) : v) : 0.f;
        }
    }
    float* __restrict__ py = gd.y + (size_t)n * Cout * DHW + sp;
    for (int co = 0; co < Cout; co += 4) {
        float a0 = has_bias ? bias[co] : 0.f, a1 = has_bias ? bias[co + 1] : 0.f;
        float a2 = has_bias ? bias[co + 2] : 0.f, a3 = has_bias ? bias[co + 3] : 0.f;
#pragma unroll
        for (int t = 0; t < T2V_MAX_TAPS; ++t) {
            const float* __restrict__ wt = wp + __builtin_amdgcn_readlane(tab_w, t) + co;
#pragma unroll
            for (int ci = 0; ci < CIN; ++ci) {
                const float4 w4 = *reinterpret_cast<const float4*>(wt + ci * Cout);
                const float v = xv[t * CIN + ci];
                a0 = fmaf(w4.x, v, a0); a1 = fmaf(w4.y, v, a1); a2 = fmaf(w4.z, v, a2); a3 = fmaf(w4.w, v, a3);
            }
        }
        if (mv) {
            py[(size_t)co * DHW] = a0;
            py[(size_t)(co + 1) * DHW] = a1;
            py[(size_t)(co + 2) * DHW] = a2;
            py[(size_t)(co + 3) * DHW] = a3;
        }
    }
}
static bool stem_ok(const t2v_conv_group* groups, int ngroups, int Cin, int Cout, int flags) {
    if ((Cin != 1 && Cin != 3) || Cout < 8 || Cout > 256 || (Cout % 4) != 0) return false;
    if (flags & (T2V_CONV_ACCUM | T2V_CONV_MASK_OUT)) return false;
    long M = 0;
    int taps = 0;
    for (int i = 0; i < ngroups; ++i) {
        if (groups[i].dstride == 2 || groups[i].ydstride == 2) return false;
        M += (long)groups[i].N * groups[i].D * groups[i].H * groups[i].W;
        if (groups[i].ntaps > taps) taps = groups[i].ntaps;
    }
    return M >= 65536 && taps > 18;
}

static bool thin_two_pass(const t2v_conv_group* groups, int ngroups, int Cin, int Cout, int nslots) {
    if (Cout != 1 || nslots < 9 || Cin < 16 || nslots * Cin > THIN_MAX_W) return false;
    long M = 0;
    for (int i = 0; i < ngroups; ++i) M += (long)groups[i].N * groups[i].D * groups[i].H * groups[i].W;
    return M >= 16384;
}

static bool thin_ok(const t2v_conv_group* groups, int ngroups, int Cin, int Cout, int& nslots) {
    if (Cout > 4) return false;
    nslots = 0;
    for (int i = 0; i < ngroups; ++i)
        for (int t = 0; t < groups[i].ntaps; ++t)
            if (groups[i].widx[t] + 1 > nslots) nslots = groups[i].widx[t] + 1;
    return (long)nslots * Cin * Cout <= THIN_MAX_W;
}

struct Tunables {
    long tile128_min;
    long tile256_min;
    long nosplit_chunks;
    long force_splits;
    long split_target;
    bool strip;
    long strip3_db;
    bool strip3_db256;
    bool occ_pad;
    long wgrad_target;
    long wgrad_scap;
    bool wgrad_quantise;
    long wgrad_min_cps;
    bool wgrad_thin;
    bool pool_fwd_db;
    bool pool_dgrad_db;
    long pool_dgrad_split_below;
    long pool_wgrad_min_cps;
};
static long env_long(const char* name, long dflt) { const char* e = getenv(name); return e ? atol(e) : dflt; }
static const Tunables& tun() {
    static const Tunables t = {env_long("T2V_TILE128_MIN", 768), env_long("T2V_TILE256_MIN", 512), env_long("T2V_NOSPLIT_CHUNKS", 8),
                               env_long("T2V_FORCE_S", 0), env_long("T2V_SPLIT_TARGET", 768), getenv("T2V_NO_STRIP") == nullptr,
                               env_long("T2V_STRIP3_DB", 16), env_long("T2V_STRIP3_DB256", 1) != 0, getenv("T2V_NO_OCC_PAD") == nullptr,
                               env_long("T2V_WGRAD_TARGET", 0), env_long("T2V_WGRAD_SCAP", 256), getenv("T2V_WGRAD_NOQ") == nullptr,
                               env_long("T2V_WGRAD_MINCPS", 4), getenv("T2V_NO_WGRAD_THIN") == nullptr,
                               env_long("T2V_POOL_FWD_DB", 1) != 0, env_long("T2V_POOL_DGRAD_DB", 0) != 0,
                               env_long("T2V_POOL_DGRAD_SPLIT_BELOW", 576), env_long("T2V_POOL_WGRAD_MINCPS", 4)};
    return t;
}

static inline int out_frames(const t2v_conv_group& g) {
    if (g.ydstride == 2) return (g.Dy + 1 - g.yoff) / 2;
    return g.dstride == 2 ? (g.D + 1) / 2 : g.D;
}
static inline long samples(const t2v_conv_group& g) { return g.N; }
static inline long voxels(const t2v_conv_group& g) { return (long)g.N * g.D * g.H * g.W; }
static inline long gemm_rows(const t2v_conv_group& g) { return (long)g.N * out_frames(g) * g.H * g.W; }

static long retile(GroupTable& tab, const t2v_conv_group* groups, int ngroups, int rows_per_tile, long (*rows_of)(const t2v_conv_group&)) {
    long mt = 0;
    for (int i = 0; i < ngroups; ++i) {
        tab.tile_start[i] = (int32_t)mt;
        mt += (rows_of(groups[i]) + rows_per_tile - 1) / rows_per_tile;
    }
    for (int i = ngroups; i <= T2V_MAX_GROUPS; ++i) tab.tile_start[i] = (int32_t)mt;
    return mt;
}

struct FwdStats { double flops = 0; long rows = 0; int taps = 0; };
static FwdStats fwd_stats(const t2v_conv_group* groups, int ngroups, int Cin, int Cout, long (*rows_of)(const t2v_conv_group&) = gemm_rows) {
    FwdStats st;
    for (int i = 0; i < ngroups; ++i) {
        st.flops += 2.0 * (double)rows_of(groups[i]) * Cout * Cin * groups[i].ntaps;
        st.rows += rows_of(groups[i]);
        if (groups[i].ntaps > st.taps) st.taps = groups[i].ntaps;
    }
    return st;
}

static void launch_splitk_reduce(const GroupTable& tab, const float* ws, const float* bias, int S, int Cin, int Cout, int flags,
                                 const FwdStats& st, hipStream_t s) {
    long blocks = (tab.out_start[tab.n] + 255) / 256;
    if (blocks > 2048) blocks = 2048;
    ProfScope prof_r(4, 0.0, s, st.rows, Cin, Cout, st.taps, tab.n, S);
    T2V_LAUNCH_PROF(splitk_reduce_kernel, dim3((unsigned)blocks), dim3(256), 0, s, tab, ws, bias, S, Cout, flags);
}

static bool group_ok(const t2v_conv_group& g, bool need_ptrs) {
    if (need_ptrs && (!g.x || !g.y)) return false;
    if (g.dstride < 0 || g.dstride > 2 || g.ydstride < 0 || g.ydstride > 2) return false;
    if (g.ydstride == 2 && (g.dstride == 2 || g.yoff < 0 || g.yoff > 1 || g.Dy < 1 || (g.Dy + 1 - g.yoff) / 2 < 1 || g.D < (g.Dy + 1) / 2)) return false;
    if (g.N < 1 || g.D < 1 || g.H < 1 || g.W < 1 || g.ntaps < 1 || g.ntaps > T2V_MAX_TAPS) return false;
    for (int t = 0; t < g.ntaps; ++t) {
        if (g.dz[t] < -1 || g.dz[t] > 1 || g.dy[t] < -1 || g.dy[t] > 1 || g.dx[t] < -1 || g.dx[t] > 1) return false;
        if (g.widx[t] < 0 || g.widx[t] >= T2V_MAX_TAPS) return false;
    }
    return true;
}

struct ConvPlan { int bm, bn, bk; bool fast, vecb; int S; long tiles; bool dstride2; };

static bool build_table(const t2v_conv_group* groups, int ngroups, int Cin, int Cout, bool need_ptrs, GroupTable& tab,
                        ConvPlan& p) {
    if (!groups || ngroups < 1 || ngroups > T2V_MAX_GROUPS || Cin < 1 || Cout < 1) return false;
    long Mtot = 0;
    int max_chunk_taps = 1;
    p.dstride2 = false;
    for (int i = 0; i < ngroups; ++i) {
        if (!group_ok(groups[i], need_ptrs)) return false;
        if (voxels(groups[i]) * (long)(Cin > Cout ? Cin : Cout) >= (1L << 31)) return false;
        if (groups[i].dstride == 2 || groups[i].ydstride == 2) p.dstride2 = true;
        Mtot += gemm_rows(groups[i]);
        if (groups[i].ntaps > max_chunk_taps) max_chunk_taps = groups[i].ntaps;
    }
    p.bk = (Cin % 64 == 0) ? 64 : (Cin % 32 == 0) ? 32 : 16;
    p.fast = (Cin % 16 == 0);
    p.vecb = (Cout % 4 == 0);
    if (Cout <= 32) { p.bm = 128; p.bn = 32; if (p.bk > 32) p.bk = 32; }
    else {
        p.bn = 64;
        const long t128 = ((Mtot + 127) / 128) * ((Cout + 63) / 64);
        p.bm = (t128 >= tun().tile128_min) ? 128 : 64;
        if (p.fast && ((Mtot + 255) / 256) * ((Cout + 63) / 64) >= tun().tile256_min) { p.bm = 256; p.bk = 16; }
        if (p.bk > 32 && p.bm != 256) p.bk = 32;
    }
    if (!p.fast) p.bk = 16;
    long ot = 0;
    tab.n = ngroups;
    for (int i = 0; i < ngroups; ++i) {
        tab.g[i] = groups[i];
        tab.out_start[i] = ot;
// ... 4 lines not shown
    const long min_chunks = p.fast ? (long)max_chunk_taps * (Cin / p.bk) : ((long)max_chunk_taps * Cin + p.bk - 1) / p.bk;
    long S = 1;
    if (p.tiles < 384 && min_chunks > tun().nosplit_chunks) {
        S = (tun().split_target + p.tiles - 1) / p.tiles;
        long maxS = min_chunks / 2;
        if (S > maxS) S = maxS;
        if (S > 64) S = 64;
        while (S > 1 && (double)S * ot * 4.0 > 256e6) --S;
        if (S < 1) S = 1;
    }
    if (p.dstride2) S = 1;
    const long force_S = tun().force_splits;
    if (force_S > 0 && !p.dstride2) S = force_S > min_chunks / 2 ? (min_chunks / 2 > 0 ? min_chunks / 2 : 1) : force_S;
    p.S = (int)S;
    return true;
}

static bool strip_ok(const GroupTable& tab) {
    bool any3 = false;
    for (int i = 0; i < tab.n; ++i) {
        const t2v_conv_group& g = tab.g[i];
        const int ndx = g.dx[0] < 0 ? 3 : 1;
        if (g.ntaps % ndx) return false;
        for (int r = 0; r < g.ntaps / ndx; ++r)
            for (int d = 0; d < ndx; ++d) {
                const int t = r * ndx + d;
                if (g.dx[t] != (ndx == 3 ? d - 1 : 0) || g.dz[t] != g.dz[r * ndx] || g.dy[t] != g.dy[r * ndx]) return false;
            }
        if (ndx == 3 && g.W < 2) return false;
        any3 = any3 || ndx == 3;
    }
    return any3;
}
static bool strip_fits32(const GroupTable& tab, int Cin) {
    for (int i = 0; i < tab.n; ++i)
        if (voxels(tab.g[i]) * (long)Cin >= (1L << 30)) return false;
    return true;
}

struct OccInfo { int occ = 0, lds = 0, cus = 0; };
template <class K>
static int occupancy_pad(K kernel, OccInfo& info, long nwg) {
    if (!info.occ) {
        hipFuncAttributes a;
        int dev = 0, n = 0, cus = 0;
        if (hipFuncGetAttributes(&a, (const void*)kernel) != hipSuccess || hipGetDevice(&dev) != hipSuccess ||
            hipDeviceGetAttribute(&cus, hipDeviceAttributeMultiprocessorCount, dev) != hipSuccess ||
            hipOccupancyMaxActiveBlocksPerMultiprocessor(&n, kernel, 256, 0) != hipSuccess || n < 1 || cus < 1) {
            (void)hipGetLastError();
            info.occ = -1;
        } else {
            info.occ = n; info.lds = (int)a.sharedSizeBytes; info.cus = cus;
        }
    }
    if (info.occ < 3 || !tun().occ_pad) return 0;
    long best = -1;
    int pick = info.occ;
    for (int o = info.occ; o >= 2; --o) {
        const long cost = ((nwg + (long)info.cus * o - 1) / ((long)info.cus * o)) * o;
        if (best < 0 || cost < best) { best = cost; pick = o; }
    }
    if (pick == info.occ) return 0;
    const int lds_total = 160 * 1024;
    const int need = lds_total / (pick + 1) + 512;
    return need > info.lds ? need - info.lds : 0;
}

enum class FwdKernel {
    Igemm = 0,
    Strip = 1,
    Thin = 2,
    Linear = 3,
    ThinTwoPass = 4,
    Strip3 = 5,
    Stem = 12
};
static inline bool is_gemm(FwdKernel k) { return k == FwdKernel::Igemm || k == FwdKernel::Strip || k == FwdKernel::Strip3; }
struct FwdLaunch : ConvPlan {
    FwdKernel kernel;
    int db;
    bool occ_pad;
    int nslots;
    dim3 grid, block;
    bool reduce;
    int64_t ws_floats;
    bool needs_ws;
    bool launchable;
    int64_t ws_query;
};

static int strip3_db(const GroupTable& tab, const ConvPlan& p) {
    const long db = tun().strip3_db;
    if (!p.vecb || p.bn != 64 || (p.bm != 64 && p.bm != 256)) return 0;
    if (p.bm == 64 ? (db != 16 && db != 32) : !tun().strip3_db256) return 0;
    for (int i = 0; i < tab.n; ++i)
        if (tab.g[i].dx[0] >= 0) return 0;
    return p.bm == 64 ? (int)db : 16;
}

static bool decide_fwd(const t2v_conv_group* groups, int ngroups, int Cin, int Cout, int flags, bool need_ptrs, GroupTable& tab,
                       FwdLaunch& d) {
    if (!build_table(groups, ngroups, Cin, Cout, need_ptrs, tab, d)) return false;
    const int64_t out_floats = tab.out_start[ngroups];
    const int S_gemm = d.S;
    const bool strip = d.fast && (d.bk == 32 || d.bm == 256) && (Cin % d.bk) == 0 && tun().strip && strip_ok(tab) && strip_fits32(tab, Cin);
    const bool strip3 = strip && d.bn == 64;
    bool one_voxel = Cout <= 4, slot0 = true;
    for (int i = 0; i < ngroups; ++i) {
        one_voxel = one_voxel && groups[i].D == 1 && groups[i].H == 1 && groups[i].W == 1 && groups[i].ntaps == 1;
        slot0 = slot0 && groups[i].widx[0] == 0;
    }
    const bool thin = thin_ok(groups, ngroups, Cin, Cout, d.nslots);
    d.db = 0;
    d.block = dim3(256);
    d.ws_floats = 0;
    d.launchable = !d.dstride2 || (!thin && !(flags & T2V_CONV_ACCUM) && strip3);
    if (one_voxel && slot0) {
        d.kernel = FwdKernel::Linear;
        d.bm = 0; d.bn = Cout == 1 ? 1 : 4;
        d.grid = dim3((unsigned)((retile(tab, groups, ngroups, 1, samples) + 3) / 4));
    } else if (thin) {
        const bool two_pass = thin_two_pass(groups, ngroups, Cin, Cout, d.nslots);
        d.kernel = two_pass ? FwdKernel::ThinTwoPass : FwdKernel::Thin;
        d.bm = 256; d.bn = Cout == 1 ? 1 : 4;
        d.grid = dim3((unsigned)retile(tab, groups, ngroups, 256, voxels));
        if (two_pass) d.ws_floats = (int64_t)d.nslots * out_floats;
    } else if (stem_ok(groups, ngroups, Cin, Cout, flags)) {
        d.kernel = FwdKernel::Stem;
        d.bm = 256; d.bn = Cin;
        d.grid = dim3((unsigned)retile(tab, groups, ngroups, 256, voxels));
        if (Cin == 1 && (Cout % 32) == 0) d.block = dim3(512);
    } else {
        d.kernel = strip3 ? FwdKernel::Strip3 : strip ? FwdKernel::Strip : FwdKernel::Igemm;
        if (strip3) d.db = strip3_db(tab, d);
        d.grid = dim3((unsigned)tab.tile_start[ngroups], (unsigned)((Cout + d.bn - 1) / d.bn), (unsigned)d.S);
        if (d.S > 1) d.ws_floats = (int64_t)d.S * out_floats;
    }
    if (!is_gemm(d.kernel)) { d.bk = 0; d.fast = d.vecb = false; d.S = 1; }
    d.occ_pad = d.kernel == FwdKernel::Strip3 && d.bm == 256 && !d.db;
    d.reduce = d.S > 1;
    d.needs_ws = d.reduce || (d.kernel == FwdKernel::Linear && !thin && S_gemm > 1);
    d.ws_query = d.ws_floats;
    if (d.kernel == FwdKernel::Stem && S_gemm > 1) d.ws_query = (int64_t)S_gemm * out_floats;
    if (is_gemm(d.kernel) && one_voxel) d.ws_query = 0;
    return true;
}

static void fwd_plan_out(const FwdLaunch& d, int32_t* out) {
    const int32_t v[8] = {(int32_t)d.kernel, d.bm, d.bn, d.db ? d.db : d.bk, d.fast ? 1 : 0, (d.fast && d.vecb) ? 1 : 0,
                          is_gemm(d.kernel) ? (d.db ? 2 : 1) : 0, d.S};
    for (int i = 0; i < 8; ++i) out[i] = v[i];
}
extern "C" int t2v_conv_fwd_plan(const t2v_conv_group* groups, int ngroups, int Cin, int Cout, int flags, int32_t* out) {
    GroupTable tab;
    FwdLaunch d;
    if (!out || !decide_fwd(groups, ngroups, Cin, Cout, flags, false, tab, d)) return T2V_EINVAL;
    fwd_plan_out(d, out);
    return T2V_OK;
}
extern "C" int64_t t2v_conv_fwd_grouped_ws_floats(const t2v_conv_group* groups, int ngroups, int Cin, int Cout) {
    GroupTable tab;
    FwdLaunch d;
    if (!decide_fwd(groups, ngroups, Cin, Cout, 0, false, tab, d)) return T2V_EINVAL;
    return d.ws_query;
}

template <int BM, int BN, int WAVES_CO, int BKT>
static void launch_gemm_tile(const FwdLaunch& d, const GroupTable& tab, const float* wp, const float* bias, float* slab, int Cin,
                             int Cout, int flags, hipStream_t s) {
#define GEMM_LAUNCH(kernel, pad) T2V_LAUNCH_PROF(kernel, d.grid, d.block, pad, s, tab, wp, bias, slab, Cin, Cout, flags, d.S)
    switch (d.kernel) {
    case FwdKernel::Strip3:
        if constexpr (BN == 64 && ((BM != 256 && BKT == 32) || (BM == 256 && BKT == 16))) {
            constexpr int WCO3 = BM == 256 ? 1 : 2;
            const long nwg = (long)d.grid.x * d.grid.y * d.grid.z;
            if constexpr (BM == 256) {
                if (d.db) { GEMM_LAUNCH((conv_igemm_strip3_kernel<256, 16, 1, true, true>), 0); return; }
            }
            if constexpr (BM == 64) {
                if (d.db == 32) { GEMM_LAUNCH((conv_igemm_strip3_kernel<64, 32, 2, true, true>), 0); return; }
                if (d.db == 16) { GEMM_LAUNCH((conv_igemm_strip3_kernel<64, 16, 2, true, true>), 0); return; }
            }
            if (d.vecb) {
                static OccInfo oi;
                GEMM_LAUNCH((conv_igemm_strip3_kernel<BM, BKT, WCO3, true>), d.occ_pad ? occupancy_pad(conv_igemm_strip3_kernel<BM, BKT, WCO3, true>, oi, nwg) : 0);
            } else {
                static OccInfo oi;
                GEMM_LAUNCH((conv_igemm_strip3_kernel<BM, BKT, WCO3, false>), d.occ_pad ? occupancy_pad(conv_igemm_strip3_kernel<BM, BKT, WCO3, false>, oi, nwg) : 0);
            }
        }
        return;
    case FwdKernel::Strip:
        if constexpr (BN == 32) {
            if (d.vecb) GEMM_LAUNCH((conv_igemm_strip_kernel<BM, BN, WAVES_CO, BKT, true>), 0);
            else GEMM_LAUNCH((conv_igemm_strip_kernel<BM, BN, WAVES_CO, BKT, false>), 0);
        }
        return;
    default:
        if (!d.fast) GEMM_LAUNCH((conv_igemm_kernel<BM, BN, WAVES_CO, 16, false, false>), 0);
        else if (d.vecb) GEMM_LAUNCH((conv_igemm_kernel<BM, BN, WAVES_CO, BKT, true, true>), 0);
        else GEMM_LAUNCH((conv_igemm_kernel<BM, BN, WAVES_CO, BKT, true, false>), 0);
    }
#undef GEMM_LAUNCH
}

extern "C" int t2v_conv_fwd_grouped(const t2v_conv_group* groups, int ngroups, int Cin, int Cout, const float* wp,
                                    const float* bias, float* ws, int flags, void* stream) {
    GroupTable tab;
    FwdLaunch d;
    if (!wp || !decide_fwd(groups, ngroups, Cin, Cout, flags, true, tab, d)) return T2V_EINVAL;
    if (flags & T2V_CONV_MASK_OUT) {
        if (flags & T2V_CONV_ACCUM) return T2V_EINVAL;
        for (int i = 0; i < ngroups; ++i)
            if (!groups[i].mask) return T2V_EINVAL;
    }
    if ((d.needs_ws && !ws) || !d.launchable) return T2V_EINVAL;
    hipStream_t s = (hipStream_t)stream;
#ifdef T2V_ABLATION
    if (const char* e = getenv("T2V_DEBUG_FLAGS")) flags |= atoi(e);
#endif
    const FwdStats st = fwd_stats(groups, ngroups, Cin, Cout);
    const int taps = d.kernel == FwdKernel::Linear ? 1 : st.taps;
    int32_t plan_[8];
    fwd_plan_out(d, plan_);
    FwdKernel kernel = d.kernel;
    if (kernel == FwdKernel::ThinTwoPass && !ws) kernel = FwdKernel::Thin;
    {
        ProfScope prof(is_gemm(kernel) ? 0 : 3, st.flops, s, st.rows, Cin, Cout, taps, ngroups, d.S);
        ProfScope::set_plan(plan_, 8);
        switch (kernel) {
        case FwdKernel::Linear:
            if (Cout == 1) T2V_LAUNCH_PROF(linear_thin_kernel<1>, d.grid, d.block, 0, s, tab, wp, bias, Cin, Cout, flags);
            else T2V_LAUNCH_PROF(linear_thin_kernel<4>, d.grid, d.block, 0, s, tab, wp, bias, Cin, Cout, flags);
            break;
        case FwdKernel::Thin:
            if (Cout == 1) T2V_LAUNCH_PROF(conv_thin_kernel<1>, d.grid, d.block, 0, s, tab, wp, bias, Cin, Cout, d.nslots, flags);
            else T2V_LAUNCH_PROF(conv_thin_kernel<4>, d.grid, d.block, 0, s, tab, wp, bias, Cin, Cout, d.nslots, flags);
            break;
        case FwdKernel::ThinTwoPass:
            if (Cin == 64) T2V_LAUNCH_PROF(thin_taps_mfma_kernel<32>, d.grid, dim3(512), 0, s, tab, wp, ws, d.nslots, flags);
            else if (Cin == 32) T2V_LAUNCH_PROF(thin_taps_mfma_kernel<16>, d.grid, dim3(512), 0, s, tab, wp, ws, d.nslots, flags);
            else if (Cin == 16) T2V_LAUNCH_PROF(thin_taps_mfma_kernel<8>, d.grid, dim3(512), 0, s, tab, wp, ws, d.nslots, flags);
            else if (Cin == 128) T2V_LAUNCH_PROF(thin_taps_mfma_kernel<64>, d.grid, dim3(512), 0, s, tab, wp, ws, d.nslots, flags);
            else T2V_LAUNCH_PROF(thin_taps_kernel, d.grid, d.block, 0, s, tab, wp, ws, Cin, d.nslots, flags);
            break;
        case FwdKernel::Stem:
            if (Cin == 1 && (Cout % 32) == 0) T2V_LAUNCH_PROF(conv_stem_mfma_kernel, d.grid, d.block, 0, s, tab, wp, bias, Cout, flags);
            else if (Cin == 1) T2V_LAUNCH_PROF(conv_stem_kernel<1>, d.grid, d.block, 0, s, tab, wp, bias, Cout, flags);
            else T2V_LAUNCH_PROF(conv_stem_kernel<3>, d.grid, d.block, 0, s, tab, wp, bias, Cout, flags);
            break;
        default:
            if (d.bn == 32) {
                if (d.bk == 32) launch_gemm_tile<128, 32, 1, 32>(d, tab, wp, bias, ws, Cin, Cout, flags, s);
                else launch_gemm_tile<128, 32, 1, 16>(d, tab, wp, bias, ws, Cin, Cout, flags, s);
            } else if (d.bm == 256) {
                launch_gemm_tile<256, 64, 1, 16>(d, tab, wp, bias, ws, Cin, Cout, flags, s);
            } else if (d.bm == 128) {
                if (d.bk == 32) launch_gemm_tile<128, 64, 2, 32>(d, tab, wp, bias, ws, Cin, Cout, flags, s);
                else launch_gemm_tile<128, 64, 2, 16>(d, tab, wp, bias, ws, Cin, Cout, flags, s);
            } else {
                if (d.bk == 32) launch_gemm_tile<64, 64, 2, 32>(d, tab, wp, bias, ws, Cin, Cout, flags, s);
                else launch_gemm_tile<64, 64, 2, 16>(d, tab, wp, bias, ws, Cin, Cout, flags, s);
            }
        }
    }
    if (kernel == FwdKernel::ThinTwoPass) {
        ProfScope prof2(3, 0.0, s, st.rows, Cin, Cout, taps, ngroups, 2);
        T2V_LAUNCH_PROF(thin_shift_sum_kernel, d.grid, d.block, 0, s, tab, ws, bias, d.nslots, flags);
    }
    int st_ = launch_status();
    if (st_ || !d.reduce) return st_;
    launch_splitk_reduce(tab, ws, bias, d.S, Cin, Cout, flags, st, s);
    return launch_status();
}

extern "C" int t2v_conv_fwd_grouped_bf16_ok(const t2v_conv_group* groups, int ngroups, int Cin, int Cout) {
    GroupTable tab;
    ConvPlan p;
    int nslots;
    if (!build_table(groups, ngroups, Cin, Cout, false, tab, p)) return 0;
    if ((Cin % 32) != 0 || Cout <= 4 || thin_ok(groups, ngroups, Cin, Cout, nslots)) return 0;
    return 1;
}
enum class Bf16Kernel {
    Igemm = 6,
    Strip3 = 8
};
struct Bf16Launch : ConvPlan {
    Bf16Kernel kernel;
    dim3 grid, block;
    bool reduce;
};
static bool decide_bf16(const t2v_conv_group* groups, int ngroups, int Cin, int Cout, int flags, bool need_ptrs, GroupTable& tab,
                        Bf16Launch& d) {
    if (!t2v_conv_fwd_grouped_bf16_ok(groups, ngroups, Cin, Cout) || !build_table(groups, ngroups, Cin, Cout, need_ptrs, tab, d)) return false;
    if (d.bn != 64 || d.bm == 256) {
        d.bn = 64;
        d.bm = 128;
        retile(tab, groups, ngroups, d.bm, gemm_rows);
    }
    d.bk = 32;
    const long wbytes = 2L * T2V_MAX_TAPS * Cout * Cin;
    const bool strip3 = tun().strip && strip_ok(tab) && strip_fits32(tab, Cin) && wbytes < (1L << 31);
    if (d.dstride2 && (!strip3 || (flags & T2V_CONV_ACCUM))) return false;
    d.kernel = strip3 ? Bf16Kernel::Strip3 : Bf16Kernel::Igemm;
    d.grid = dim3((unsigned)tab.tile_start[ngroups], (unsigned)((Cout + 63) / 64), (unsigned)d.S);
    d.block = dim3(256);
    d.reduce = d.S > 1;
    return true;
}
static void bf16_plan_out(const Bf16Launch& d, int32_t* out) {
    const int32_t v[8] = {(int32_t)d.kernel, d.bm, d.bn, d.bk, d.dstride2 ? 1 : 0, 0, 0, d.S};
    for (int i = 0; i < 8; ++i) out[i] = v[i];
}
extern "C" int t2v_conv_fwd_bf16_plan(const t2v_conv_group* groups, int ngroups, int Cin, int Cout, int flags, int32_t* out) {
    GroupTable tab;
    Bf16Launch d;
    if (!out || !decide_bf16(groups, ngroups, Cin, Cout, flags, false, tab, d)) return T2V_EINVAL;
    bf16_plan_out(d, out);
    return T2V_OK;
}
extern "C" int t2v_conv_fwd_grouped_bf16(const t2v_conv_group* groups, int ngroups, int Cin, int Cout, const void* wpb,
                                         const float* bias, float* ws, int flags, void* stream) {
    GroupTable tab;
    Bf16Launch d;
    if (!wpb || !decide_bf16(groups, ngroups, Cin, Cout, flags, true, tab, d)) return T2V_EINVAL;
    if (flags & T2V_CONV_MASK_OUT) {
        if (flags & T2V_CONV_ACCUM) return T2V_EINVAL;
        for (int i = 0; i < ngroups; ++i)
            if (!groups[i].mask) return T2V_EINVAL;
    }
    if (d.reduce && !ws) return T2V_EINVAL;
    hipStream_t s = (hipStream_t)stream;
    const FwdStats st = fwd_stats(groups, ngroups, Cin, Cout);
    const __bf16* w = (const __bf16*)wpb;
    {
        ProfScope prof(5, st.flops, s, st.rows, Cin, Cout, st.taps, ngroups, d.S);
        int32_t plan_[8];
        bf16_plan_out(d, plan_);
        ProfScope::set_plan(plan_, 8);
        if (d.kernel == Bf16Kernel::Strip3) {
            if (d.bm == 128) T2V_LAUNCH_PROF(conv_igemm_bf16_strip3_kernel<128>, d.grid, d.block, 0, s, tab, w, bias, ws, Cin, Cout, flags, d.S);
            else T2V_LAUNCH_PROF(conv_igemm_bf16_strip3_kernel<64>, d.grid, d.block, 0, s, tab, w, bias, ws, Cin, Cout, flags, d.S);
        } else if (d.bm == 128) T2V_LAUNCH_PROF(conv_igemm_bf16_kernel<128>, d.grid, d.block, 0, s, tab, w, bias, ws, Cin, Cout, flags, d.S);
        else T2V_LAUNCH_PROF(conv_igemm_bf16_kernel<64>, d.grid, d.block, 0, s, tab, w, bias, ws, Cin, Cout, flags, d.S);
    }
    int st_ = launch_status();
    if (st_ || !d.reduce) return st_;
    launch_splitk_reduce(tab, ws, bias, d.S, Cin, Cout, flags, st, s);
    return launch_status();
}

static bool geom_ok(const t2v_conv_geom* g) {
    if (!g) return false;
    if (g->N < 1 || g->Cin < 1 || g->Cout < 1 || g->D < 1 || g->H < 1 || g->W < 1) return false;
    if (g->ntaps < 1 || g->ntaps > T2V_MAX_TAPS) return false;
    return true;
}
static t2v_conv_group group_of(const t2v_conv_geom* g, const float* x, float* y) {
    t2v_conv_group q;
    q.x = x; q.y = y; q.mask = nullptr;
    q.N = g->N; q.D = g->D; q.H = g->H; q.W = g->W; q.ntaps = g->ntaps; q.dstride = 0; q.ydstride = 0; q.yoff = 0; q.Dy = 0;
    for (int t = 0; t < T2V_MAX_TAPS; ++t) {
        q.dz[t] = t < g->ntaps ? g->dz[t] : 0; q.dy[t] = t < g->ntaps ? g->dy[t] : 0; q.dx[t] = t < g->ntaps ? g->dx[t] : 0;
        q.widx[t] = (int8_t)(t < g->ntaps ? t : 0);
    }
    return q;
}
extern "C" int64_t t2v_conv_fwd_ws_floats(const t2v_conv_geom* g) {
    if (!geom_ok(g)) return T2V_EINVAL;
    t2v_conv_group q = group_of(g, nullptr, nullptr);
    return t2v_conv_fwd_grouped_ws_floats(&q, 1, g->Cin, g->Cout);
}
extern "C" int t2v_conv_fwd(const float* x, const float* wp, const float* bias, float* y, float* ws, const t2v_conv_geom* g,
                            int flags, void* stream) {
    if (!x || !wp || !y || !geom_ok(g)) return T2V_EINVAL;
    t2v_conv_group q = group_of(g, x, y);
    return t2v_conv_fwd_grouped(&q, 1, g->Cin, g->Cout, wp, bias, ws, flags, stream);
}

#define WG_BK 32
#define WG_PITCH (WG_BK + 1)

struct WGroupTable {
    t2v_conv_group g[T2V_MAX_GROUPS];
    int32_t chunk_start[T2V_MAX_GROUPS + 1];
    int32_t n;
};

struct LiveTaps { int8_t t[T2V_MAX_TAPS]; int32_t n; };

__global__ __launch_bounds__(256) void conv_wgrad_kernel(const WGroupTable tab, float* __restrict__ slab, const int Cin,
                                                         const int Cout, const int T, const int kH, const int kW,
                                                         const int flags, const int chunks_per_split, const LiveTaps live,
                                                         float* __restrict__ bias_slab) {
    __shared__ __attribute__((aligned(16))) float As[64 * WG_PITCH];
    __shared__ __attribute__((aligned(16))) float Bs[64 * WG_PITCH];

    const int tid = threadIdx.x, lane = tid & 63, wave = tid >> 6;
    const int l31 = lane & 31, hi = lane >> 5;
    const int wco = wave & 1, wci = wave >> 1;
    const int nco_t = (Cout + 63) / 64;
    const int co0 = (blockIdx.x % nco_t) * 64, ci0 = (blockIdx.x / nco_t) * 64;
    const int lin = xcd_remap((int)(blockIdx.y + blockIdx.z * gridDim.y), (int)(gridDim.y * gridDim.z));
    const int slot = lin % (int)gridDim.y;
    const int split = lin / (int)gridDim.y;
    const int t = live.t[slot];
    const bool relu_in = flags & T2V_CONV_RELU_IN;
    const int kD = T / (kH * kW);
    const int ta = t / (kH * kW), tb = (t / kW) % kH, tc = t % kW;
    const int dz = ta - kD / 2, dy = tb - kH / 2, dx = tc - kW / 2;

    const int ml = tid & 31, rl = tid >> 5;
    f32x16 acc;
#pragma unroll
    for (int r = 0; r < 16; ++r) acc[r] = 0.f;

    const int nchunks = tab.chunk_start[tab.n];
    const int q0 = split * chunks_per_split;
    int q1 = q0 + chunks_per_split;
    if (q1 > nchunks) q1 = nchunks;

    float ra[8], rb[8];
    bool pend_v = false;
    const bool do_bias = bias_slab != nullptr && ci0 == 0 && t == T / 2;
    bool pend_mv = false;
    float bsum[8];
#pragma unroll
    for (int p = 0; p < 8; ++p) bsum[p] = 0.f;
    const bool full = co0 + 64 <= Cout && ci0 + 64 <= Cin;
    int g_i = -1, g_begin = 0, g_end = 0;
// ... 1411 lines not shown
#ifdef T2V_ABLATION
    if (const char* e = getenv("T2V_DEBUG_FLAGS")) flags |= atoi(e);
#endif
    const int T = kD * kH * kW;
    TapMap map;
    LiveTaps live;
    live.n = 0;
    for (int t = 0; t < T2V_MAX_TAPS; ++t) {
        live.t[t] = 0;
        map.j[t] = -1;
    }
    LiveRows lrows;
    lrows.n = 0;
    for (int r = 0; r < 9; ++r) lrows.r[r] = 0;
    if (d.kernel == WgradKernel::Rows3) {
        for (int r = 0; r < kD * kH; ++r)
            if ((d.liverows >> r) & 1u) {
                for (int c = 0; c < 3; ++c) map.j[r * 3 + c] = lrows.n * 3 + c;
                lrows.r[lrows.n++] = (int8_t)r;
            }
    } else {
        for (int t = 0; t < T; ++t)
            if ((d.live >> t) & 1u) { map.j[t] = live.n; live.t[live.n++] = (int8_t)t; }
    }
    double flops = 0;
    for (int i = 0; i < ngroups; ++i) {
        int live_g = 0;
        for (int a = 0; a < kD; ++a) for (int b = 0; b < kH; ++b) for (int c = 0; c < kW; ++c) {
            const int dz = a - kD / 2, dy = b - kH / 2, dx = c - kW / 2;
            if (!((groups[i].D == 1 && dz) || (groups[i].H == 1 && dy) || (groups[i].W == 1 && dx))) ++live_g;
        }
        flops += 2.0 * (double)gemm_rows(groups[i]) * Cout * Cin * live_g;
    }
    {
        ProfScope prof(1, flops, s, d.nchunks * WG_BK, Cin, Cout, d.nlive, ngroups, d.S);
        int32_t plan_[8];
        wgrad_plan_out(d, plan_, 8);
        ProfScope::set_plan(plan_, 8);
        switch (d.kernel) {
        case WgradKernel::Gemm:
            T2V_LAUNCH_PROF(conv_wgrad_gemm_kernel, d.grid, d.block, 0, s, tab, slab, Cin, Cout, flags, d.cps, bias_part);
            break;
        case WgradKernel::Rows3:
            if (d.bf16) T2V_LAUNCH_PROF(conv_wgrad3_kernel<true>, d.grid, d.block, 0, s, tab, slab, Cin, Cout, kD, kH, flags, d.cps, lrows, bias_part);
            else T2V_LAUNCH_PROF(conv_wgrad3_kernel<false>, d.grid, d.block, 0, s, tab, slab, Cin, Cout, kD, kH, flags, d.cps, lrows, bias_part);
            break;
        case WgradKernel::Thin:
            T2V_LAUNCH_PROF(conv_wgrad_thin_kernel, d.grid, d.block, 0, s, tab, slab, Cin, Cout, T, kH, kW, flags, d.cps, live, bias_part);
            break;
        case WgradKernel::Cols:
            T2V_LAUNCH_PROF(conv_wgrad_cols_kernel, d.grid, d.block, 0, s, tab, slab, Cin, Cout, T, kH, kW, flags, d.cps, live, bias_part);
            break;
        default:
            if (d.bf16) T2V_LAUNCH_PROF(conv_wgrad_bf16_kernel, d.grid, d.block, 0, s, tab, slab, Cin, Cout, T, kH, kW, flags, d.cps, live, bias_part);
            else T2V_LAUNCH_PROF(conv_wgrad_kernel, d.grid, d.block, 0, s, tab, slab, Cin, Cout, T, kH, kW, flags, d.cps, live, bias_part);
        }
    }
    int st = launch_status();
    if (st) return st;
    return wgrad_finish(d, T, map, slab, bias_part, dw, dbias, Cin, Cout, flags, s, out_src);
}
extern "C" int t2v_conv_wgrad_grouped(const t2v_conv_group* groups, int ngroups, int Cin, int Cout, int kD, int kH, int kW,
                                      float* dw, float* slab, int flags, void* stream) {
    return wgrad_impl(groups, ngroups, Cin, Cout, kD, kH, kW, dw, nullptr, false, slab, flags, stream, nullptr);
}
extern "C" int t2v_conv_wgrad_grouped_bias(const t2v_conv_group* groups, int ngroups, int Cin, int Cout, int kD, int kH, int kW,
                                           float* dw, float* dbias, float* slab, int flags, void* stream) {
    if (!dbias) return T2V_EINVAL;
    return wgrad_impl(groups, ngroups, Cin, Cout, kD, kH, kW, dw, dbias, true, slab, flags, stream, nullptr);
}

extern "C" int t2v_conv_wgrad_grouped_partial(const t2v_conv_group* groups, int ngroups, int Cin, int Cout, int kD, int kH,
                                              int kW, float* slab, int want_bias, int flags, t2v_wgrad_src* out_src,
                                              void* stream) {
    if (!out_src) return T2V_EINVAL;
    return wgrad_impl(groups, ngroups, Cin, Cout, kD, kH, kW, nullptr, nullptr, want_bias != 0, slab, flags, stream, out_src);
}
enum class PoolKernel { Fwd = 9, Dgrad = 10 };
struct PoolLaunch {
    PoolKernel kernel;
    bool db;
    bool vecb;
    int S;
    long tiles;
    dim3 grid, block;
    int64_t ws_floats;
};
static bool pool_member_ok(const t2v_conv_group& g, bool need_ptrs) {
    if (need_ptrs && (!g.x || !g.y)) return false;
    if (g.N < 1 || g.H < 2 || g.W < 2 || (g.H & 1) || (g.W & 1)) return false;
    if (g.dstride == 0) return g.D == 1;
    if (g.dstride != 1 && g.dstride != 2) return false;
    return g.D >= 2 && !(g.D & 1);
}
static inline long pool_rows(const t2v_conv_group& g) { return (long)g.N * (g.dstride ? g.D / 2 : 1) * (g.H / 2) * (g.W / 2); }
static inline long pool_padded(const t2v_conv_group& g) { return (long)(g.dstride ? g.D + 1 : 1) * (g.H + 1) * (g.W + 2); }
static inline long pool_grid(const t2v_conv_group& g) { return (long)(g.dstride ? g.D / 2 + 1 : 1) * (g.H / 2 + 1) * (g.W / 2 + 1); }
static inline long pool_grid_rows(const t2v_conv_group& g) { return (long)g.N * pool_grid(g); }

static bool decide_pool_fwd(const t2v_conv_group* groups, int ngroups, int Cin, int Cout, bool need_ptrs, GroupTable& tab, PoolLaunch& d) {
    if (!groups || ngroups < 1 || ngroups > T2V_MAX_GROUPS || Cin < 32 || (Cin % 32) || Cout < 4 || (Cout % 4)) return false;
    long ot = 0;
    int max_rows = 1;
    tab.n = ngroups;
    for (int i = 0; i < ngroups; ++i) {
        const t2v_conv_group& g = groups[i];
        if (!pool_member_ok(g, need_ptrs)) return false;
        if ((long)g.N * pool_padded(g) * Cin >= (1L << 29) || pool_rows(g) * Cout >= (1L << 31)) return false;
        if (g.ntaps != 9 && g.ntaps != 27) return false;
        if (g.dstride == 0 && g.ntaps != 9) return false;
        for (int r = 0; r < g.ntaps / 3; ++r)
            for (int dd = 0; dd < 3; ++dd) {
                const int t = r * 3 + dd;
                if (g.dx[t] != dd - 1 || g.dz[t] != g.dz[r * 3] || g.dy[t] != g.dy[r * 3] || g.dz[t] < -1 || g.dz[t] > 1 || g.dy[t] < -1 ||
                    g.dy[t] > 1 || g.widx[t] < 0 || g.widx[t] >= T2V_MAX_TAPS)
                    return false;
                if (g.dstride == 0 && g.dz[t] != 0) return false;
            }
        if (g.ntaps / 3 > max_rows) max_rows = g.ntaps / 3;
        tab.g[i] = g;
        tab.out_start[i] = ot;
        ot += pool_rows(g) * Cout;
    }
    for (int i = ngroups; i <= T2V_MAX_GROUPS; ++i) tab.out_start[i] = ot;
    const long mt = retile(tab, groups, ngroups, 64, pool_rows);
    d.kernel = PoolKernel::Fwd;
    d.db = tun().pool_fwd_db;
    d.tiles = mt * ((Cout + 63) / 64);
    d.vecb = (Cout % 4) == 0;
    const long rounds = (long)max_rows * (Cin / 32);
    long S = 1;
    if (d.tiles < 384 && rounds > tun().nosplit_chunks) {
        S = (768 + d.tiles - 1) / d.tiles;
        if (S > rounds / 2) S = rounds / 2;
        if (S > 64) S = 64;
        while (S > 1 && (double)S * ot * 4.0 > 256e6) --S;
        if (S < 1) S = 1;
    }
    d.S = (int)S;
    d.grid = dim3((unsigned)mt, (unsigned)((Cout + 63) / 64), (unsigned)d.S);
    d.block = dim3(256);
    d.ws_floats = d.S > 1 ? (int64_t)d.S * ot : 0;
    return true;
}
static bool decide_pool_dgrad(const t2v_conv_group* groups, int ngroups, int K, int C, bool need_ptrs, GroupTable& tab, PoolLaunch& d) {
    if (!groups || ngroups < 1 || ngroups > T2V_MAX_GROUPS || K < 32 || (K % 32) || C < 4 || (C % 4)) return false;
    tab.n = ngroups;
    for (int i = 0; i < ngroups; ++i) {
        const t2v_conv_group& g = groups[i];
        if (!pool_member_ok(g, need_ptrs)) return false;
        if (pool_rows(g) * K >= (1L << 29) || pool_grid_rows(g) * C * 8 >= (1L << 31)) return false;
        for (int f = 0; f < 27; ++f) {
            const bool live = g.dstride != 0 || (f / 9) == 1;
            if (live && (g.widx[f] < 0 || g.widx[f] >= T2V_MAX_TAPS)) return false;
        }
        tab.g[i] = g;
    }
    for (int i = 0; i <= T2V_MAX_GROUPS; ++i) tab.out_start[i] = 0;
    const long mt = retile(tab, groups, ngroups, 64, pool_grid_rows);
    d.kernel = PoolKernel::Dgrad;
    d.db = tun().pool_dgrad_db;
    d.tiles = mt * 4 * ((C + 63) / 64);
    d.vecb = (C % 4) == 0;
    long S = 1;
    const long ncb = K / 32;
    if (d.tiles < tun().pool_dgrad_split_below && ncb >= 4) {
        S = (768 + d.tiles - 1) / d.tiles;
        if (S > ncb / 2) S = ncb / 2;
        if (S > 8) S = 8;
        if (S < 1) S = 1;
    }
    d.S = (int)S;
    d.grid = dim3((unsigned)mt, (unsigned)(4 * ((C + 63) / 64)), (unsigned)d.S);
    d.block = dim3(256);
    d.ws_floats = 0;
    return true;
}
static bool decide_pool_wgrad(const t2v_conv_group* groups, int ngroups, int Cin, int Cout, int kD, bool need_ptrs, WGroupTable& tab, WgradLaunch& d) {
    if (!groups || ngroups < 1 || ngroups > T2V_MAX_GROUPS || Cin < 1 || Cout < 1 || (kD != 1 && kD != 3)) return false;
    long nch = 0;
    bool any_t = false;
    tab.n = ngroups;
    for (int i = 0; i < ngroups; ++i) {
        const t2v_conv_group& g = groups[i];
        if (!pool_member_ok(g, need_ptrs)) return false;
        if ((long)g.N * pool_padded(g) * Cin >= (1L << 29) || pool_rows(g) * Cout >= (1L << 29)) return false;
        any_t = any_t || g.dstride != 0;
        if (kD == 1 && g.dstride != 0) return false;
        tab.g[i] = g;
        tab.chunk_start[i] = (int32_t)nch;
        nch += (pool_rows(g) + WG_BK - 1) / WG_BK;
    }
    for (int i = ngroups; i <= T2V_MAX_GROUPS; ++i) tab.chunk_start[i] = (int32_t)nch;
    d.kernel = WgradKernel::PoolRows3;
    d.bf16 = d.strided = false;
    d.nchunks = nch;
    d.liverows = any_t ? 0x1ffu : 0x038u;
    d.nrows = any_t ? 9 : 3;
    d.live = any_t ? 0x7ffffffu : (0x1ffu << 9);
    d.nlive = d.nrows * 3;
    d.grid = dim3((unsigned)(((Cout + 63) / 64) * ((Cin + 63) / 64)), (unsigned)d.nrows);
    wgrad_set_splits(d, wgrad_ksplit((long)d.grid.x * d.grid.y, nch, tun().pool_wgrad_min_cps), 1, Cin, Cout);
    return true;
}

static void pool_plan_out(const PoolLaunch& d, int32_t* out) {
    const int32_t v[8] = {(int32_t)d.kernel, 64, 64, d.db ? 16 : 32, 1, d.vecb ? 1 : 0, d.db ? 2 : 1, d.S};
    for (int i = 0; i < 8; ++i) out[i] = v[i];
}
extern "C" int t2v_pool_conv_plan(int what, const t2v_conv_group* groups, int ngroups, int Cin, int Cout, int32_t* out) {
    if (!out) return T2V_EINVAL;
    for (int i = 0; i < 8; ++i) out[i] = 0;
    if (what == 0 || what == 1) {
        GroupTable tab;
        PoolLaunch d;
        if (!(what == 0 ? decide_pool_fwd(groups, ngroups, Cin, Cout, false, tab, d) : decide_pool_dgrad(groups, ngroups, Cin, Cout, false, tab, d)))
            return T2V_EINVAL;
        pool_plan_out(d, out);
        return T2V_OK;
    }
    if (what == 2) {
        WGroupTable tab;
        WgradLaunch d;
        if (!decide_pool_wgrad(groups, ngroups, Cin, Cout, 3, false, tab, d)) return T2V_EINVAL;
        wgrad_plan_out(d, out, 8);
        return T2V_OK;
    }
    return T2V_EINVAL;
}
extern "C" int64_t t2v_pool_conv_fwd_ws_floats(const t2v_conv_group* groups, int ngroups, int Cin, int Cout) {
    GroupTable tab;
    PoolLaunch d;
    if (!decide_pool_fwd(groups, ngroups, Cin, Cout, false, tab, d)) return T2V_EINVAL;
    return d.ws_floats;
}
extern "C" int t2v_pool_conv_dgrad_splits(const t2v_conv_group* groups, int ngroups, int K, int C) {
    GroupTable tab;
    PoolLaunch d;
    if (!decide_pool_dgrad(groups, ngroups, K, C, false, tab, d)) return T2V_EINVAL;
    return d.S;
}
extern "C" int64_t t2v_pool_conv_wgrad_slab_floats(const t2v_conv_group* groups, int ngroups, int Cin, int Cout, int kD, int want_bias) {
    WGroupTable tab;
    WgradLaunch d;
    if (!decide_pool_wgrad(groups, ngroups, Cin, Cout, kD, false, tab, d)) return T2V_EINVAL;
    return d.slab_floats + (want_bias ? d.bias_floats : 0);
}

extern "C" int t2v_pool_conv_fwd(const t2v_conv_group* groups, int ngroups, int Cin, int Cout, const float* wp, const float* bias,
                                 float* ws, int flags, void* stream) {
    GroupTable tab;
    PoolLaunch d;
    if (!wp || !decide_pool_fwd(groups, ngroups, Cin, Cout, true, tab, d)) return T2V_EINVAL;
    if (flags & ~(T2V_CONV_BIAS | T2V_CONV_ACCUM)) return T2V_EINVAL;
    if (d.S > 1 && !ws) return T2V_EINVAL;
    hipStream_t s = (hipStream_t)stream;
    const FwdStats st = fwd_stats(groups, ngroups, Cin, Cout, pool_rows);
    {
        ProfScope prof(0, st.flops, s, st.rows, Cin, Cout, st.taps, ngroups, d.S);
        int32_t plan_[8];
        pool_plan_out(d, plan_);
        ProfScope::set_plan(plan_, 8);
        if (d.db) T2V_LAUNCH_PROF((conv_pool_fwd_kernel<64, true>), d.grid, d.block, 0, s, tab, wp, bias, ws, Cin, Cout, flags, d.S);
        else T2V_LAUNCH_PROF(conv_pool_fwd_kernel<64>, d.grid, d.block, 0, s, tab, wp, bias, ws, Cin, Cout, flags, d.S);
    }
    int st_ = launch_status();
    if (st_ || d.S == 1) return st_;
    for (int i = 0; i < ngroups; ++i) {
        tab.g[i].D = groups[i].dstride ? groups[i].D / 2 : 1;
        tab.g[i].H = groups[i].H / 2;
        tab.g[i].W = groups[i].W / 2;
    }
    launch_splitk_reduce(tab, ws, bias, d.S, Cin, Cout, flags, st, s);
    return launch_status();
}
extern "C" int t2v_pool_conv_dgrad(const t2v_conv_group* groups, int ngroups, int K, int C, const float* wp, void* stream) {
    GroupTable tab;
    PoolLaunch d;
    if (!wp || !decide_pool_dgrad(groups, ngroups, K, C, true, tab, d)) return T2V_EINVAL;
    hipStream_t s = (hipStream_t)stream;
    double flops = 0;
    long Mtot = 0;
    for (int i = 0; i < ngroups; ++i) {
        flops += 2.0 * (double)pool_rows(groups[i]) * K * C * (groups[i].dstride ? 27 : 9);
        Mtot += pool_grid_rows(groups[i]);
    }
    ProfScope prof(0, flops, s, Mtot, K, C, 27, ngroups, d.S);
    int32_t plan_[8];
    pool_plan_out(d, plan_);
    ProfScope::set_plan(plan_, 8);
    if (d.db) T2V_LAUNCH_PROF(conv_pool_dgrad_kernel<true>, d.grid, d.block, 0, s, tab, wp, K, C);
    else T2V_LAUNCH_PROF(conv_pool_dgrad_kernel<false>, d.grid, d.block, 0, s, tab, wp, K, C);
    return launch_status();
}
static int pool_wgrad_impl(const t2v_conv_group* groups, int ngroups, int Cin, int Cout, int kD, float* dw, float* dbias, bool want_bias,
                           float* slab, int flags, void* stream, t2v_wgrad_src* out_src) {
    WGroupTable tab;
    WgradLaunch d;
    if ((!dw && !out_src) || !slab || !decide_pool_wgrad(groups, ngroups, Cin, Cout, kD, true, tab, d)) return T2V_EINVAL;
    hipStream_t s = (hipStream_t)stream;
    float* bias_part = want_bias ? slab + d.slab_floats : (float*)nullptr;
    const int T = kD * 9;
    TapMap map;
    for (int t = 0; t < T2V_MAX_TAPS; ++t) map.j[t] = -1;
    LiveRows lrows;
    lrows.n = 0;
    for (int r = 0; r < 9; ++r) lrows.r[r] = 0;
    for (int r = 0; r < 9; ++r)
        if ((d.liverows >> r) & 1u) {
            const int rw = kD == 3 ? r : r - 3;
            for (int c = 0; c < 3; ++c) map.j[rw * 3 + c] = lrows.n * 3 + c;
            lrows.r[lrows.n++] = (int8_t)r;
        }
    double flops = 0;
    for (int i = 0; i < ngroups; ++i) flops += 2.0 * (double)pool_rows(groups[i]) * Cout * Cin * (groups[i].dstride ? 27 : 9);
    {
        ProfScope prof(1, flops, s, d.nchunks * WG_BK, Cin, Cout, d.nlive, ngroups, d.S);
        int32_t plan_[8];
        wgrad_plan_out(d, plan_, 8);
        ProfScope::set_plan(plan_, 8);
        T2V_LAUNCH_PROF(conv_pool_wgrad_kernel, d.grid, d.block, 0, s, tab, slab, Cin, Cout, d.cps, lrows, bias_part);
    }
    int st = launch_status();
    if (st) return st;
    return wgrad_finish(d, T, map, slab, bias_part, dw, dbias, Cin, Cout, flags, s, out_src);
}
extern "C" int t2v_pool_conv_wgrad(const t2v_conv_group* groups, int ngroups, int Cin, int Cout, int kD, float* dw, float* dbias,
                                   float* slab, int flags, void* stream) {
    if (!dw) return T2V_EINVAL;
    return pool_wgrad_impl(groups, ngroups, Cin, Cout, kD, dw, dbias, dbias != nullptr, slab, flags, stream, nullptr);
}
extern "C" int t2v_pool_conv_wgrad_partial(const t2v_conv_group* groups, int ngroups, int Cin, int Cout, int kD, float* slab,
                                           int want_bias, int flags, t2v_wgrad_src* out_src, void* stream) {
    if (!out_src) return T2V_EINVAL;
    return pool_wgrad_impl(groups, ngroups, Cin, Cout, kD, nullptr, nullptr, want_bias != 0, slab, flags, stream, out_src);
}

extern "C" int t2v_wgrad_dest_bytes(void) { return (int)sizeof(t2v_wgrad_dest); }


__global__ __launch_bounds__(256) void wgrad_reduce_multi_kernel(const t2v_wgrad_dest* __restrict__ table, int ndest) {
    __shared__ __attribute__((aligned(16))) float tile[256 * T2V_MAX_TAPS];
    __shared__ __attribute__((aligned(16))) float part[4][256];
    __shared__ int s_dest;
    if (threadIdx.x == 0) {
        int lo = 0, hi = ndest - 1;
        while (lo < hi) {
            const int mid = (lo + hi + 1) >> 1;
            if (table[mid].block_begin <= (int)blockIdx.x) lo = mid; else hi = mid - 1;
        }
// ... 309 lines not shown
```

txt2vid_amd/functional.py:

```python
import contextlib
import ctypes as C
import os
import weakref

import torch
from torch.autograd import Function
from torch.autograd.function import once_differentiable

from ._lib import lib, check, ConvGeom, ConvGroup, PackJob, WgradSrc, WgradDest, WGRAD_MAX_SRC, MAX_TAPS, MAX_GROUPS

FLAG_BIAS, FLAG_RELU_IN, FLAG_ACCUM, FLAG_MASK_OUT, FLAG_ACCUM_BIAS, FLAG_BF16 = 1, 2, 4, 8, 16, 32


from ._ops import _stream, _p, _c


def tap_major(w):
    nd = w.dim()
    fwd = tuple(range(2, nd)) + (0, 1)
    back = tuple(range(nd - 2, nd)) + tuple(range(nd - 2))
    return w.permute(*fwd).contiguous().permute(*back)


def is_tap_major(w):
# ... 1880 lines not shown

def copy_into(src, dst):
    src = _c(src)
    n = src.numel()
    _copy2d(src, 0, n, dst, 0, n, 1, n)


class CatBatch(Function):

    @staticmethod
    def forward(ctx, a, b):
        a, b = _c(a), _c(b)
        ctx.na = a.shape[0]
        out = torch.empty((a.shape[0] + b.shape[0],) + tuple(a.shape[1:]), device=a.device, dtype=torch.float32)
        na, nb = a.numel(), b.numel()
        _copy2d(a, 0, na, out, 0, na, 1, na)
        _copy2d(b, 0, nb, out, na, nb, 1, nb)
        return out

    @staticmethod
    def backward(ctx, g):
        return (g[:ctx.na] if ctx.needs_input_grad[0] else None), (g[ctx.na:] if ctx.needs_input_grad[1] else None)


def cat_batch(a, b):
    return CatBatch.apply(a, b)


from .draws import HostDraws, StaticDraws


draws = HostDraws()


def set_draws(d):
    global draws
    draws = d



class _TapSet(object):
    __slots__ = ('taps', 'taps_c', 'T', 'mask')


_tapset_cache = {}


def _tapset(T, mask):
    key = (T, mask)
    ts = _tapset_cache.get(key)
    if ts is None:
        ts = _TapSet()
        ts.taps = [t for t in range(T) if (mask >> t) & 1]
        ts.taps_c = (C.c_int32 * len(ts.taps))(*ts.taps)
        ts.T, ts.mask = T, mask
        _tapset_cache[key] = ts
    return ts


def _group_table(ins, outs, geoms, slot_of, masks=None, dstride=0):
    arr = (ConvGroup * len(ins))()
    for i, (xi, yi, g) in enumerate(zip(ins, outs, geoms)):
        a = arr[i]
        a.dstride = dstride
        a.x, a.y = xi.data_ptr(), (yi.data_ptr() if yi is not None else 0)
        a.mask = masks[i].data_ptr() if masks is not None else None
        a.N, a.D, a.H, a.W, a.ntaps = g.cg.N, g.cg.D, g.cg.H, g.cg.W, g.cg.ntaps
        for j, t in enumerate(g.taps):
            a.dz[j], a.dy[j], a.dx[j] = g.cg.dz[j], g.cg.dy[j], g.cg.dx[j]
            a.widx[j] = slot_of[t] if slot_of is not None else 0
    return arr


def _conv_table(ins, outs, cin, cout, k, masks=None, dstride=0):
    geoms = [conv_geom(t.shape[0], cin, t.shape[2], t.shape[3], t.shape[4], cout, k[0], k[1], k[2]) for t in ins]
    mask = 0
    for g in geoms:
        mask |= g.mask
    ts = _tapset(geoms[0].T, mask)
    slot_of = {t: j for j, t in enumerate(ts.taps)}
    return _group_table(ins, outs, geoms, slot_of, masks, dstride), ts


def _fwd_workspace(arr, n, cin, cout, device):
    nws = int(lib().t2v_conv_fwd_grouped_ws_floats(arr, n, cin, cout))
    if nws < 0:
        raise RuntimeError('bad grouped conv geometry')
    return torch.empty((nws,), device=device, dtype=torch.float32) if nws > 0 else None


def conv_group_raw(xs5, w5, bias=None, relu_in=False, mode=0, masks=None, outs=None, accum=False, even_frames=False):
    if len(xs5) > MAX_GROUPS:
        raise ValueError('at most %d tensors per grouped convolution' % MAX_GROUPS)
    if even_frames and (mode != 0 or masks is not None or accum or outs is not None):
        raise ValueError('even_frames is a plain forward option')
    xs5 = [_c(t) for t in xs5]
    w5 = _c(w5)
    Cout_w, Cin_w = w5.shape[0], w5.shape[1]
    cin, cout = (Cin_w, Cout_w) if mode == 0 else (Cout_w, Cin_w)
    ys = outs if outs is not None else [torch.empty((t.shape[0], cout, (t.shape[2] + 1) // 2 if even_frames else t.shape[2]) + tuple(t.shape[3:]),
                                                    device=t.device, dtype=torch.float32) for t in xs5]
    if masks is not None:
        masks = [_c(m) for m in masks]
        if any(m.shape != y.shape for m, y in zip(masks, ys)):
            raise ValueError('mask / output shape mismatch')
    arr, ts = _conv_table(xs5, ys, cin, cout, tuple(w5.shape[2:]), masks, 2 if even_frames else 0)
    ws = _fwd_workspace(arr, len(xs5), cin, cout, xs5[0].device)
    flags = ((FLAG_BIAS if bias is not None else 0) | (FLAG_RELU_IN if relu_in else 0) | (FLAG_MASK_OUT if masks is not None else 0) |
             (FLAG_ACCUM if accum else 0))
    if CONV_PRECISION == 'bf16' and lib().t2v_conv_fwd_grouped_bf16_ok(arr, len(xs5), cin, cout):
        wpb = packed_weight_bf16(w5, ts, mode)
        check(lib().t2v_conv_fwd_grouped_bf16(arr, len(xs5), cin, cout, _p(wpb), _p(bias), _p(ws), flags, _stream()),
              't2v_conv_fwd_grouped_bf16')
        return ys
    wp = packed_weight(w5, ts, mode)
    check(lib().t2v_conv_fwd_grouped(arr, len(xs5), cin, cout, _p(wp), _p(bias), _p(ws), flags, _stream()), 't2v_conv_fwd_grouped')
    return ys


def _wgrad_table(xs5, gys5, wshape, want_bias, even_frames, sink=None):
    Cout, Cin = wshape[0], wshape[1]
    k = tuple(wshape[2:])
    geoms = [conv_geom(t.shape[0], Cin, t.shape[2], t.shape[3], t.shape[4], Cout, k[0], k[1], k[2]) for t in xs5]
    arr = _group_table(xs5, gys5, geoms, None, None, 2 if even_frames else 0)
    query = lib().t2v_conv_wgrad_grouped_bias_slab_floats if want_bias else lib().t2v_conv_wgrad_grouped_slab_floats
    n = int(query(arr, len(xs5), Cin, Cout, k[0], k[1], k[2]))
    if n <= 0:
        raise RuntimeError('bad grouped wgrad geometry')
    slab = sink.alloc_slab(n, xs5[0].device) if sink is not None else torch.empty((n,), device=xs5[0].device, dtype=torch.float32)
    return arr, slab


def conv_group_wgrad_raw(xs5, gys5, wshape, relu_in=False, out=None, accum=False, dbias=None, accum_bias=False, even_frames=False):
    xs5, gys5 = [_c(t) for t in xs5], [_c(t) for t in gys5]
    Cout, Cin = wshape[0], wshape[1]
    k = tuple(wshape[2:])
    arr, slab = _wgrad_table(xs5, gys5, wshape, dbias is not None, even_frames)
    dw = out if out is not None else torch.empty(tuple(wshape), device=xs5[0].device, dtype=torch.float32)
    flags = (FLAG_RELU_IN if relu_in else 0) | (FLAG_ACCUM if accum else 0) | (FLAG_BF16 if CONV_PRECISION == 'bf16' else 0)
    if dbias is not None:
        check(lib().t2v_conv_wgrad_grouped_bias(arr, len(xs5), Cin, Cout, k[0], k[1], k[2], _p(dw), _p(dbias), _p(slab),
                                                flags | (FLAG_ACCUM_BIAS if accum_bias else 0), _stream()),
              't2v_conv_wgrad_grouped_bias')
    else:
        check(lib().t2v_conv_wgrad_grouped(arr, len(xs5), Cin, Cout, k[0], k[1], k[2], _p(dw), _p(slab), flags, _stream()),
              't2v_conv_wgrad_grouped')
    return dw


def _wgrad_partial_launch(xs5, gys5, wshape, relu_in, want_bias, sink=None, even_frames=False):
    xs5, gys5 = [_c(t) for t in xs5], [_c(t) for t in gys5]
    Cout, Cin = wshape[0], wshape[1]
    k = tuple(wshape[2:])
    arr, slab = _wgrad_table(xs5, gys5, wshape, want_bias, even_frames, sink)
    src = WgradSrc()
    flags = (FLAG_RELU_IN if relu_in else 0) | (FLAG_BF16 if CONV_PRECISION == 'bf16' else 0)
    check(lib().t2v_conv_wgrad_grouped_partial(arr, len(xs5), Cin, Cout, k[0], k[1], k[2], _p(slab), 1 if want_bias else 0, flags,
                                               C.byref(src), _side.fork(xs5, gys5) if sink is not None else _stream()),
          't2v_conv_wgrad_grouped_partial')
    return src, slab


def conv_group_wgrad_partial(xs5, gys5, wshape, relu_in, sink, wbase, dw, wacc, b, dbias, bacc, even_frames=False):
    src, slab = _wgrad_partial_launch(xs5, gys5, wshape, relu_in, b is not None, sink, even_frames)
    k = tuple(wshape[2:])
    sink.add_partial(wbase, dw, wacc, b, dbias, bacc, src, slab, k[0] * k[1] * k[2], wshape[0], wshape[0] * wshape[1])

# ... 490 lines not shown
```

txt2vid_amd/functional_pool.py:

```python
import ctypes as C
import os

import torch
from torch.autograd import Function
from torch.autograd.function import once_differentiable

from ._lib import lib, check, ConvGroup, PoolBoxJob, WgradSrc, MAX_GROUPS
from ._ops import _stream, _p, _c

_DISABLED = os.environ.get('T2V_NO_POOLCONV') is not None
_NO_UPCONV = os.environ.get('T2V_NO_UPCONV') is not None


def _TF():
    from . import functional
    return functional


def pool_tmode(shape, stem):
    D, H, W = shape[2], shape[3], shape[4]
    if H < 2 or W < 2 or H % 2 or W % 2:
        return None
    if D == 1:
        return 0
# ... 12 lines not shown
        return False
    if w.shape[0] % 32 or w.shape[1] % 32 or not xs[0].is_cuda:
        return False
    return all(x.dim() == 5 and pool_tmode(x.shape, stem) is not None for x in xs)


def pooled_shape(shape, tmode):
    N, _, D, H, W = shape
    return (N, D // 2 if tmode else 1, H // 2, W // 2)



def _box_jobs(ins, masks, outs, shapes, tmodes, relu, scale=None, bias=None):
    arr = (PoolBoxJob * len(ins))()
    for a, t, sh, tm, i in zip(arr, ins, shapes, tmodes, range(len(ins))):
        a.in_, a.out = t.data_ptr(), outs[i].data_ptr()
        a.mask = masks[i].data_ptr() if masks is not None else None
        a.bias = bias.data_ptr() if bias is not None else None
        a.NC, a.D, a.H, a.W, a.C = sh[0] * sh[1], sh[2], sh[3], sh[4], sh[1]
        a.tmode, a.relu, a.scale = tm, int(relu), pool_scale(tm) if scale is None else scale
    return arr


def boxsum_raw(ins, tmodes, relu, masks=None, scale=None):
    ins = [_c(t) for t in ins]
    masks = [_c(m) for m in masks] if masks is not None else None
    shapes = [tuple(t.shape) for t in ins]
    outs = [torch.empty((sh[0], sh[1], sh[2] + 1 if tm else 1, sh[3] + 1, sh[4] + 2), device=t.device, dtype=torch.float32)
            for t, sh, tm in zip(ins, shapes, tmodes)]
    check(lib().t2v_pool_boxsum(_box_jobs(ins, masks, outs, shapes, tmodes, relu, scale), len(ins), _stream()), 't2v_pool_boxsum')
    return outs


def unbox_raw(planes, shapes, tmodes, masks=None, scale=None, bias=None):
    masks = [_c(m) for m in masks] if masks is not None else None
    outs = [torch.empty(tuple(sh), device=p.device, dtype=torch.float32) for p, sh in zip(planes, shapes)]
    sets = planes[0].shape[0] if planes[0].dim() == 7 else 1
    check(lib().t2v_pool_unbox(_box_jobs(planes, masks, outs, shapes, tmodes, sets, scale, bias), len(planes), _stream()), 't2v_pool_unbox')
    return outs


def _tap_union(tmodes, kD=3):
    TF = _TF()
    if kD == 1:
        if any(tmodes):
            raise ValueError('a 2-D kernel cannot serve members with a time axis')
        return TF._tapset(9, 0x1ff)
    mask = (1 << 27) - 1 if any(tmodes) else 0x1ff << 9
    return TF._tapset(27, mask)


def _tap_index(ts, dz, dy, dx):
    return (dy + 1) * 3 + dx + 1 if ts.T == 9 else ((dz + 1) * 3 + dy + 1) * 3 + dx + 1


def _fwd_table(xs, ys, shapes, tmodes, ts):
    slot_of = {t: j for j, t in enumerate(ts.taps)}
    arr = (ConvGroup * len(xs))()
    for a, x, y, sh, tm in zip(arr, xs, ys, shapes, tmodes):
        a.x, a.y, a.mask = x.data_ptr(), (y.data_ptr() if y is not None else 0), None
        a.N, a.D, a.H, a.W = sh[0], sh[2], sh[3], sh[4]
        a.dstride = tm
        j = 0
        for dz in ((-1, 0, 1) if tm else (0,)):
            for dy in (-1, 0, 1):
                for dx in (-1, 0, 1):
                    a.dz[j], a.dy[j], a.dx[j] = dz, dy, dx
                    a.widx[j] = slot_of[_tap_index(ts, dz, dy, dx)]
                    j += 1
        a.ntaps = j
    return arr


def pool_fwd_raw(rts, shapes, tmodes, w5, bias=None, transpose=False):
    TF = _TF()
    w5 = _c(w5)
    cout, cin = (w5.shape[1], w5.shape[0]) if transpose else (w5.shape[0], w5.shape[1])
    ts = _tap_union(tmodes, w5.shape[2])
    zs = []
    for sh, tm, t in zip(shapes, tmodes, rts):
        n, d, h, w_ = pooled_shape(sh, tm)
        zs.append(torch.empty((n, cout, d, h, w_), device=t.device, dtype=torch.float32))
    arr = _fwd_table(rts, zs, shapes, tmodes, ts)
    nws = int(lib().t2v_pool_conv_fwd_ws_floats(arr, len(rts), cin, cout))
    if nws < 0:
        raise RuntimeError('bad pooled-convolution geometry')
    ws = torch.empty((nws,), device=rts[0].device, dtype=torch.float32) if nws > 0 else None
    wp = TF.packed_weight(w5, ts, 1 if transpose else 0)
    check(lib().t2v_pool_conv_fwd(arr, len(rts), cin, cout, _p(wp), _p(bias), _p(ws), TF.FLAG_BIAS if bias is not None else 0, _stream()),
          't2v_pool_conv_fwd')
    return zs


def pool_dgrad_raw(gzs, shapes, tmodes, w5, transpose=False):
    TF = _TF()
    gzs = [_c(g) for g in gzs]
    w5 = _c(w5)
    cout, cin = (w5.shape[1], w5.shape[0]) if transpose else (w5.shape[0], w5.shape[1])
    ts = _tap_union(tmodes, w5.shape[2])
    slot_of = {t: j for j, t in enumerate(ts.taps)}
    arr = (ConvGroup * len(gzs))()
    for a, g, sh, tm in zip(arr, gzs, shapes, tmodes):
        if tuple(g.shape) != (sh[0], cout) + pooled_shape(sh, tm)[1:]:
            raise ValueError('pooled gradient of shape %s for a member of shape %s' % (tuple(g.shape), tuple(sh)))
        a.x, a.y, a.mask = g.data_ptr(), None, None
        a.N, a.D, a.H, a.W = sh[0], sh[2], sh[3], sh[4]
        a.dstride, a.ntaps = tm, 27
        for f in range(27):
            a.widx[f] = slot_of.get(26 - f, -1) if ts.T == 27 else (slot_of.get(8 - (f - 9), -1) if 9 <= f < 18 else -1)
    S = int(lib().t2v_pool_conv_dgrad_splits(arr, len(gzs), cout, cin))
    if S < 1:
        raise RuntimeError('bad pooled data-gradient geometry')
    planes = [torch.empty((S, 8, sh[0], cin, sh[2] // 2 + 1 if tm else 1, sh[3] // 2 + 1, sh[4] // 2 + 1), device=g.device, dtype=torch.float32)
              for g, sh, tm in zip(gzs, shapes, tmodes)]
    for a, pl in zip(arr, planes):
        a.y = pl.data_ptr()
    wp = TF.packed_weight(w5, ts, 0 if transpose else 1)
    check(lib().t2v_pool_conv_dgrad(arr, len(gzs), cout, cin, _p(wp), _stream()), 't2v_pool_conv_dgrad')
    return planes


def _wgrad_table(rts, gzs, shapes, tmodes):
    arr = (ConvGroup * len(rts))()
    for a, x, g, sh, tm in zip(arr, rts, gzs, shapes, tmodes):
        a.x, a.y, a.mask = x.data_ptr(), g.data_ptr(), None
        a.N, a.D, a.H, a.W = sh[0], sh[2], sh[3], sh[4]
        a.dstride, a.ntaps = tm, 27 if tm else 9
    return arr


def pool_wgrad_raw(rts, gzs, shapes, tmodes, wshape, out=None, accum=False, dbias=None, accum_bias=False):
    TF = _TF()
    gzs = [_c(g) for g in gzs]
    cout, cin, kD = wshape[0], wshape[1], wshape[2]
    arr = _wgrad_table(rts, gzs, shapes, tmodes)
    n = int(lib().t2v_pool_conv_wgrad_slab_floats(arr, len(rts), cin, cout, kD, 1 if dbias is not None else 0))
    if n <= 0:
        raise RuntimeError('bad pooled weight-gradient geometry')
    slab = torch.empty((n,), device=rts[0].device, dtype=torch.float32)
    dw = out if out is not None else torch.empty(tuple(wshape), device=rts[0].device, dtype=torch.float32)
    flags = (TF.FLAG_ACCUM if accum else 0) | (TF.FLAG_ACCUM_BIAS if accum_bias else 0)
    check(lib().t2v_pool_conv_wgrad(arr, len(rts), cin, cout, kD, _p(dw), _p(dbias), _p(slab), flags, _stream()), 't2v_pool_conv_wgrad')
    return dw


def _pool_wgrad_to_sink(w, b, rts, gzs, shapes, tmodes, need_b):
    TF = _TF()
    sink = TF._grad_sink
    if sink is None or torch.is_grad_enabled():
        return False, None, None
    wbase = w._base if w._base is not None else w
    if id(wbase) not in sink.slots or (need_b and id(b) not in sink.slots):
        return False, None, None
    gzs = [_c(g) for g in gzs]
    cout, cin = w.shape[0], w.shape[1]
    wflat, wacc = sink.take(wbase, sink.defer)
    bflat, bacc = sink.take(b, sink.defer) if need_b else (None, False)
    if sink.defer:
        arr = _wgrad_table(rts, gzs, shapes, tmodes)
        n = int(lib().t2v_pool_conv_wgrad_slab_floats(arr, len(rts), cin, cout, 3, 1 if need_b else 0))
        if n <= 0:
            raise RuntimeError('bad pooled weight-gradient geometry')
        slab = sink.alloc_slab(n, rts[0].device)
        src = WgradSrc()
        check(lib().t2v_pool_conv_wgrad_partial(arr, len(rts), cin, cout, 3, _p(slab), 1 if need_b else 0, 0, C.byref(src),
                                                TF._side.fork(rts, gzs)), 't2v_pool_conv_wgrad_partial')
# ... 180 lines not shown
```

Measured before the change: 3078 videos/s.

## Fuse split-K reduction into conv kernels via per-tile arrival counters

Adds a fused split-K path in which each split block writes its partial tile to the slab and increments a per-tile atomic counter. The last-arriving block reloads and sums all partials, then runs the normal bias/accum/mask epilogue, so the separate split-K reduce kernel launch is skipped. A device counter buffer is allocated lazily from Python and registered per device, and the path is gated by a size threshold (S*bm*bn*4 bytes, default 64KB) with bm=256 excluded. The cost is extra atomics, a last-block serial reload, and reliance on the counters being reset, all to save a kernel launch and a pass over the slab.

```diff
diff --git a/include/t2v_hip.h b/include/t2v_hip.h
--- a/include/t2v_hip.h
+++ b/include/t2v_hip.h
@@ -71,6 +71,7 @@
 int64_t t2v_conv_fwd_grouped_ws_floats(const t2v_conv_group* groups, int ngroups, int Cin, int Cout);
 int t2v_conv_fwd_grouped(const t2v_conv_group* groups, int ngroups, int Cin, int Cout, const float* wp,
                          const float* bias, float* ws, int flags, void* stream);
+int t2v_splitk_counters(void* words, int64_t n);
 int64_t t2v_conv_wgrad_grouped_slab_floats(const t2v_conv_group* groups, int ngroups, int Cin, int Cout, int kD,
                                            int kH, int kW);
 int t2v_conv_wgrad_grouped(const t2v_conv_group* groups, int ngroups, int Cin, int Cout, int kD, int kH, int kW,
diff --git a/txt2vid_amd/_lib.py b/txt2vid_amd/_lib.py
--- a/txt2vid_amd/_lib.py
+++ b/txt2vid_amd/_lib.py
@@ -117,6 +117,7 @@
     't2v_conv_wgrad_slab_floats': [_G, _I],
     't2v_conv_fwd_grouped_ws_floats': [_P, _I, _I, _I],
     't2v_conv_fwd_grouped': [_P, _I, _I, _I, _P, _P, _P, _I, _P],
+    't2v_splitk_counters': [_P, _L],
     't2v_conv_wgrad_grouped_slab_floats': [_P, _I, _I, _I, _I, _I, _I],
     't2v_conv_fwd_plan': [_P, _I, _I, _I, _I, _I3],
     't2v_nonlocal_ok': [_I, _I],
diff --git a/txt2vid_amd/csrc/conv.hip b/txt2vid_amd/csrc/conv.hip
--- a/txt2vid_amd/csrc/conv.hip
+++ b/txt2vid_amd/csrc/conv.hip
@@ -312,13 +312,83 @@
     int32_t n;
 };
 
+#define SPLITK_DEPTH 2
 template <int NCO, int NM, int WCO, int WM>
+__device__ __forceinline__ void splitk_reload(f32x16 (&acc)[NCO][NM], const float* slab, const uint32_t total, const uint32_t out_start,
+                                              const int Cout, const int nsplit, const int m0, const int co0, const int DHW,
+                                              const int wm, const int wco, const int l31, const int hi) {
+    const __amdgpu_buffer_rsrc_t rs = __builtin_amdgcn_make_buffer_rsrc((void*)slab, 0, (int)((uint32_t)nsplit * total * 4u), 0x00020000);
+    const uint32_t step = total * 4u;
+    const uint32_t cob = (uint32_t)__builtin_amdgcn_readfirstlane(co0 + wco * WCO);
+    auto load16 = [&](float (&t)[16], uint32_t vo, uint32_t so) {
+#pragma unroll
+        for (int r = 0; r < 16; ++r)
+            t[r] = __builtin_bit_cast(float, __builtin_amdgcn_raw_buffer_load_b32(rs, vo, so + (uint32_t)((r & 3) + 8 * (r >> 2)) * (uint32_t)DHW * 4u, 16));
+    };
+#pragma unroll
+    for (int j = 0; j < NM; ++j) {
+        const int m = m0 + wm * WM + j * 32 + l31;
+        const int n = m / DHW;
+        const uint32_t vo = (((uint32_t)n * (uint32_t)Cout + 4u * hi) * (uint32_t)DHW + (uint32_t)(m - n * DHW)) * 4u;
+#pragma unroll
+        for (int i = 0; i < NCO; ++i) {
+            uint32_t so = (out_start + (cob + i * 32) * (uint32_t)DHW) * 4u;
+            f32x16 v;
+#pragma unroll
+            for (int r = 0; r < 16; ++r) v[r] = 0.f;
+            float t[SPLITK_DEPTH][16];
+#pragma unroll
+            for (int d = 0; d < SPLITK_DEPTH - 1; ++d) load16(t[d], vo, so + d * step);
+            for (int s = 0; s < nsplit; s += SPLITK_DEPTH, so += SPLITK_DEPTH * step) {
+#pragma unroll
+                for (int d = 0; d < SPLITK_DEPTH; ++d) {
+                    load16(t[(d + SPLITK_DEPTH - 1) % SPLITK_DEPTH], vo, so + (d + SPLITK_DEPTH - 1) * step);
+#pragma unroll
+                    for (int r = 0; r < 16; ++r) v[r] += t[d][r];
+                }
+            }
+            acc[i][j] = v;
+        }
+    }
+}
+
+template <int NCO, int NM, int WCO, int WM, bool FUSE>
 __device__ __forceinline__ void igemm_epilogue(f32x16 (&acc)[NCO][NM], const GroupTable& tab, const int gi, const t2v_conv_group& gd,
-                                               const float* __restrict__ bias, float* __restrict__ slab, const int Cout,
+                                               const float* __restrict__ bias, float* __restrict__ slab, unsigned int* ctr,
+                                               float* lds_flag, const int Cout,
                                                const int flags, const int nsplit, const int m0, const int co0, const int M,
                                                const int DHW, const int wm, const int wco, const int l31, const int hi,
                                                const int yds = 1, const int yoff = 0, const int DHWy = 0, const int HW = 1) {
-    const bool split = nsplit > 1;
+    bool split = nsplit > 1;
+    if (FUSE && split && ctr != nullptr) {
+        const size_t total = (size_t)tab.out_start[tab.n];
+        float* part = slab + (size_t)tab.out_start[gi];
+#pragma unroll
+        for (int j = 0; j < NM; ++j) {
+            const int m = m0 + wm * WM + j * 32 + l31;
+            if (m >= M) continue;
+            const int n = m / DHW;
+            float* py = part + (size_t)blockIdx.z * total + (size_t)n * Cout * DHW + (m - n * DHW);
+#pragma unroll
+            for (int i = 0; i < NCO; ++i) {
+#pragma unroll
+                for (int r = 0; r < 16; ++r) {
+                    const int co = co0 + wco * WCO + i * 32 + (r & 3) + 8 * (r >> 2) + 4 * hi;
+                    if (co < Cout) __hip_atomic_store(py + (size_t)co * DHW, acc[i][j][r], __ATOMIC_RELAXED, __HIP_MEMORY_SCOPE_AGENT);
+                }
+            }
+        }
+        asm volatile("s_waitcnt vmcnt(0)" ::: "memory");
+        __syncthreads();
+        unsigned int* cnt = ctr + (blockIdx.x + gridDim.x * blockIdx.y);
+        if (threadIdx.x == 0)
+            lds_flag[0] = __hip_atomic_fetch_add(cnt, 1u, __ATOMIC_RELAXED, __HIP_MEMORY_SCOPE_AGENT) == (unsigned int)(nsplit - 1) ? 1.f : 0.f;
+        __syncthreads();
+        if (lds_flag[0] == 0.f) return;
+        if (threadIdx.x == 0) __hip_atomic_store(cnt, 0u, __ATOMIC_RELAXED, __HIP_MEMORY_SCOPE_AGENT);
+        splitk_reload<NCO, NM, WCO, WM>(acc, slab, (uint32_t)total, (uint32_t)tab.out_start[gi], Cout, nsplit, m0, co0, DHW, wm, wco, l31, hi);
+        split = false;
+    }
     const bool has_bias = !split && (flags & T2V_CONV_BIAS) && bias != nullptr;
     const bool accum = !split && (flags & T2V_CONV_ACCUM);
     const bool mask_out = !split && (flags & T2V_CONV_MASK_OUT) && gd.mask != nullptr;
@@ -376,10 +446,11 @@
 }
 
 
-template <int BM, int BN, int WAVES_CO, int BKT, bool FAST, bool VECB>
+template <int BM, int BN, int WAVES_CO, int BKT, bool FAST, bool VECB, bool FUSED = false>
 __global__ __launch_bounds__(256) void conv_igemm_kernel(const GroupTable tab, const float* __restrict__ wp,
                                                          const float* __restrict__ bias, float* __restrict__ slab,
-                                                         const int Cin, const int Cout, const int flags, const int nsplit) {
+                                                         const int Cin, const int Cout, const int flags, const int nsplit,
+        unsigned int* __restrict__ ctr) {
     constexpr int WAVES_M = 4 / WAVES_CO;
     constexpr int WCO = BN / WAVES_CO;
     constexpr int WM = BM / WAVES_M;
@@ -565,13 +636,14 @@
         cur ^= 1;
     }
 
-    igemm_epilogue<NCO, NM, WCO, WM>(acc, tab, gi, gd, bias, slab, Cout, flags, nsplit, m0, co0, M, DHW, wm, wco, l31, hi);
-}
-
-template <int BM, int BN, int WAVES_CO, int BKT, bool VECB>
+    igemm_epilogue<NCO, NM, WCO, WM, FUSED>(acc, tab, gi, gd, bias, slab, ctr, As, Cout, flags, nsplit, m0, co0, M, DHW, wm, wco, l31, hi);
+}
+
+template <int BM, int BN, int WAVES_CO, int BKT, bool VECB, bool FUSED = false>
 __global__ __launch_bounds__(256) void conv_igemm_strip_kernel(const GroupTable tab, const float* __restrict__ wp,
                                                                const float* __restrict__ bias, float* __restrict__ slab,
-                                                               const int Cin, const int Cout, const int flags, const int nsplit) {
+                                                               const int Cin, const int Cout, const int flags, const int nsplit,
+        unsigned int* __restrict__ ctr) {
     constexpr int WAVES_M = 4 / WAVES_CO;
     constexpr int WCO = BN / WAVES_CO;
     constexpr int WM = BM / WAVES_M;
@@ -780,16 +852,17 @@
         if (next_a) acur ^= 1;
         dx_now = dx_next;
     }
-    igemm_epilogue<NCO, NM, WCO, WM>(acc, tab, gi, gd, bias, slab, Cout, flags, nsplit, m0, co0, M, DHW, wm, wco, l31, hi);
+    igemm_epilogue<NCO, NM, WCO, WM, FUSED>(acc, tab, gi, gd, bias, slab, ctr, As, Cout, flags, nsplit, m0, co0, M, DHW, wm, wco, l31, hi);
 }
 
 #ifndef DB_STAGE_LATE
 #define DB_STAGE_LATE 1
 #endif
-template <int BM, int BKT, int WAVES_CO, bool VECB, bool DB = false>
+template <int BM, int BKT, int WAVES_CO, bool VECB, bool DB = false, bool FUSED = false>
 __global__ __launch_bounds__(256, ((BM == 256 || (DB && BKT == 32)) ? 2 : (DB ? 4 : 3))) void conv_igemm_strip3_kernel(const GroupTable tab, const float* __restrict__ wp,
                                                                 const float* __restrict__ bias, float* __restrict__ slab,
-                                                                const int Cin, const int Cout, const int flags, const int nsplit) {
+                                                                const int Cin, const int Cout, const int flags, const int nsplit,
+        unsigned int* __restrict__ ctr) {
 #ifdef T2V_STAMPS
     const unsigned long long t_real = __builtin_amdgcn_s_memrealtime();
 #endif
@@ -1003,7 +1076,7 @@
             if (q + 1 < q1) round(std::integral_constant<int, 1>{}, q + 1);
         }
         __builtin_amdgcn_s_setprio(0);
-        igemm_epilogue<NCO, NM, WCO, WM>(acc, tab, gi, gd, bias, slab, Cout, flags, nsplit, m0, co0, M, DHWo, wm, wco, l31, hi, yds, gd.yoff,
+        igemm_epilogue<NCO, NM, WCO, WM, FUSED>(acc, tab, gi, gd, bias, slab, ctr, As, Cout, flags, nsplit, m0, co0, M, DHWo, wm, wco, l31, hi, yds, gd.yoff,
                                          gd.Dy * HW, HW);
         return;
     }
@@ -1123,7 +1196,7 @@
     }
     STAMP(t_loop1);
     if (ab_nostore && acc[0][0][0] != 12345.678f) return;
-    igemm_epilogue<NCO, NM, WCO, WM>(acc, tab, gi, gd, bias, slab, Cout, flags, nsplit, m0, co0, M, DHWo, wm, wco, l31, hi, yds, gd.yoff,
+    igemm_epilogue<NCO, NM, WCO, WM, FUSED>(acc, tab, gi, gd, bias, slab, ctr, As, Cout, flags, nsplit, m0, co0, M, DHWo, wm, wco, l31, hi, yds, gd.yoff,
                                      gd.Dy * HW, HW);
 #ifdef T2V_STAMPS
     {
@@ -1144,10 +1217,11 @@
 #endif
 }
 
-template <int BM, bool DB = false>
+template <int BM, bool DB = false, bool FUSED = false>
 __global__ __launch_bounds__(256, 3) void conv_pool_fwd_kernel(const GroupTable tab, const float* __restrict__ wp,
                                                                const float* __restrict__ bias, float* __restrict__ slab,
-                                                               const int Cin, const int Cout, const int flags, const int nsplit) {
+                                                               const int Cin, const int Cout, const int flags, const int nsplit,
+        unsigned int* __restrict__ ctr) {
     constexpr bool VECB = true;
     constexpr int BN = 64, BKT = DB ? 16 : 32, WAVES_CO = 2, WAVES_M = 2;
     constexpr int WCO = BN / WAVES_CO, WM = BM / WAVES_M;
@@ -1299,7 +1373,7 @@
         }
         __builtin_amdgcn_s_setprio(0);
         f32x16 (&accd)[1][NM] = reinterpret_cast<f32x16 (&)[1][NM]>(acc);
-        igemm_epilogue<1, NM, WCO, WM>(accd, tab, gi, gd, bias, slab, Cout, flags, nsplit, m0, co0, M, DHWn, wm, wco, l31, hi);
+        igemm_epilogue<1, NM, WCO, WM, FUSED>(accd, tab, gi, gd, bias, slab, ctr, As, Cout, flags, nsplit, m0, co0, M, DHWn, wm, wco, l31, hi);
         return;
     }
     float2 ra2[LA];
@@ -1384,7 +1458,7 @@
         __syncthreads();
     }
     f32x16 (&acc2)[1][NM] = reinterpret_cast<f32x16 (&)[1][NM]>(acc);
-    igemm_epilogue<1, NM, WCO, WM>(acc2, tab, gi, gd, bias, slab, Cout, flags, nsplit, m0, co0, M, DHWn, wm, wco, l31, hi);
+    igemm_epilogue<1, NM, WCO, WM, FUSED>(acc2, tab, gi, gd, bias, slab, ctr, As, Cout, flags, nsplit, m0, co0, M, DHWn, wm, wco, l31, hi);
 }
 
 template <bool DB>
@@ -1691,10 +1765,11 @@
 typedef __attribute__((ext_vector_type(8))) __bf16 bf16x8;
 #define B16_KP 40
 
-template <int BM>
+template <int BM, bool FUSED = false>
 __global__ __launch_bounds__(256) void conv_igemm_bf16_kernel(const GroupTable tab, const __bf16* __restrict__ wpb,
                                                               const float* __restrict__ bias, float* __restrict__ slab,
-                                                              const int Cin, const int Cout, const int flags, const int nsplit) {
+                                                              const int Cin, const int Cout, const int flags, const int nsplit,
+        unsigned int* __restrict__ ctr) {
     constexpr int BN = 64, BKT = 32, WAVES_CO = 2;
     constexpr int WAVES_M = 2;
     constexpr int WCO = BN / WAVES_CO, WM = BM / WAVES_M;
@@ -1822,13 +1897,14 @@
         if (q + 2 < q1) { advance(); load_chunk(); }
         cur ^= 1;
     }
-    igemm_epilogue<NCO, NM, WCO, WM>(acc, tab, gi, gd, bias, slab, Cout, flags, nsplit, m0, co0, M, DHW, wm, wco, l31, hi);
-}
-
-template <int BM>
+    igemm_epilogue<NCO, NM, WCO, WM, FUSED>(acc, tab, gi, gd, bias, slab, ctr, reinterpret_cast<float*>(Xs), Cout, flags, nsplit, m0, co0, M, DHW, wm, wco, l31, hi);
+}
+
+template <int BM, bool FUSED = false>
 __global__ __launch_bounds__(256) void conv_igemm_bf16_strip3_kernel(const GroupTable tab, const __bf16* __restrict__ wpb,
                                                                      const float* __restrict__ bias, float* __restrict__ slab,
-                                                                     const int Cin, const int Cout, const int flags, const int nsplit) {
+                                                                     const int Cin, const int Cout, const int flags, const int nsplit,
+        unsigned int* __restrict__ ctr) {
     constexpr int BN = 64, BKT = 32, WAVES_CO = 2, WAVES_M = 2;
     constexpr int WCO = BN / WAVES_CO, WM = BM / WAVES_M;
     constexpr int NCO = WCO / 32, NM = WM / 32;
@@ -2002,7 +2078,7 @@
         }
         __syncthreads();
     }
-    igemm_epilogue<NCO, NM, WCO, WM>(acc, tab, gi, gd, bias, slab, Cout, flags, nsplit, m0, co0, M, DHWo, wm, wco, l31, hi, yds, gd.yoff,
+    igemm_epilogue<NCO, NM, WCO, WM, FUSED>(acc, tab, gi, gd, bias, slab, ctr, reinterpret_cast<float*>(Xs), Cout, flags, nsplit, m0, co0, M, DHWo, wm, wco, l31, hi, yds, gd.yoff,
                                      gd.Dy * HW, HW);
 }
 
@@ -2449,7 +2525,9 @@
     bool pool_dgrad_db;
     long pool_dgrad_split_below;
     long pool_wgrad_min_cps;
+    long splitk_fused_bytes;
 };
+#define SPLITK_FUSED_BYTES_DEFAULT 65536
 static long env_long(const char* name, long dflt) { const char* e = getenv(name); return e ? atol(e) : dflt; }
 static const Tunables& tun() {
     static const Tunables t = {env_long("T2V_TILE128_MIN", 768), env_long("T2V_TILE256_MIN", 512), env_long("T2V_NOSPLIT_CHUNKS", 8),
@@ -2458,8 +2536,51 @@
                                env_long("T2V_WGRAD_TARGET", 0), env_long("T2V_WGRAD_SCAP", 256), getenv("T2V_WGRAD_NOQ") == nullptr,
                                env_long("T2V_WGRAD_MINCPS", 4), getenv("T2V_NO_WGRAD_THIN") == nullptr,
                                env_long("T2V_POOL_FWD_DB", 1) != 0, env_long("T2V_POOL_DGRAD_DB", 0) != 0,
-                               env_long("T2V_POOL_DGRAD_SPLIT_BELOW", 576), env_long("T2V_POOL_WGRAD_MINCPS", 4)};
+                               env_long("T2V_POOL_DGRAD_SPLIT_BELOW", 576), env_long("T2V_POOL_WGRAD_MINCPS", 4),
+                               env_long("T2V_SPLITK_FUSED_BYTES", SPLITK_FUSED_BYTES_DEFAULT)};
     return t;
+}
+
+#include <mutex>
+#define SPLITK_MAX_DEVICES 64
+static struct {
+    std::mutex mu;
+    unsigned int* words[SPLITK_MAX_DEVICES] = {};
+    int64_t n[SPLITK_MAX_DEVICES] = {};
+    int64_t cursor[SPLITK_MAX_DEVICES] = {};
+} g_splitk;
+static int splitk_device() {
+    int dev = 0;
+    if (hipGetDevice(&dev) != hipSuccess) { (void)hipGetLastError(); dev = 0; }
+    return dev >= 0 && dev < SPLITK_MAX_DEVICES ? dev : -1;
+}
+extern "C" int t2v_splitk_counters(void* words, int64_t n) {
+    const int dev = splitk_device();
+    if (n < 0 || (words && n == 0) || (!words && n != 0) || dev < 0) return T2V_EINVAL;
+    std::lock_guard<std::mutex> lock(g_splitk.mu);
+    g_splitk.words[dev] = (unsigned int*)words;
+    g_splitk.n[dev] = n;
+    g_splitk.cursor[dev] = 0;
+    return T2V_OK;
+}
+static bool splitk_fused(int S, long tiles, int bm, int bn, int64_t out_floats) {
+    const long T = tun().splitk_fused_bytes;
+    if (S <= 1 || bm == 256 || T == 0 || (T > 0 && (long)S * bm * bn * 4 > T)) return false;
+    if ((int64_t)S * out_floats * 4 >= (1LL << 30)) return false;
+    const int dev = splitk_device();
+    if (dev < 0) return false;
+    std::lock_guard<std::mutex> lock(g_splitk.mu);
+    return g_splitk.words[dev] != nullptr && tiles <= g_splitk.n[dev];
+}
+static unsigned int* splitk_take(long tiles) {
+    const int dev = splitk_device();
+    if (dev < 0) return nullptr;
+    std::lock_guard<std::mutex> lock(g_splitk.mu);
+    if (!g_splitk.words[dev] || tiles > g_splitk.n[dev]) return nullptr;
+    if (g_splitk.cursor[dev] + tiles > g_splitk.n[dev]) g_splitk.cursor[dev] = 0;
+    unsigned int* p = g_splitk.words[dev] + g_splitk.cursor[dev];
+    g_splitk.cursor[dev] += tiles;
+    return p;
 }
 
 static inline int out_frames(const t2v_conv_group& g) {
@@ -2630,6 +2751,7 @@
     bool occ_pad;
     int nslots;
     dim3 grid, block;
+    bool fused;
     bool reduce;
     int64_t ws_floats;
     bool needs_ws;
@@ -2686,8 +2808,9 @@
     }
     if (!is_gemm(d.kernel)) { d.bk = 0; d.fast = d.vecb = false; d.S = 1; }
     d.occ_pad = d.kernel == FwdKernel::Strip3 && d.bm == 256 && !d.db;
-    d.reduce = d.S > 1;
-    d.needs_ws = d.reduce || (d.kernel == FwdKernel::Linear && !thin && S_gemm > 1);
+    d.fused = splitk_fused(d.S, (long)d.grid.x * d.grid.y, d.bm, d.bn, tab.out_start[ngroups]);
+    d.reduce = d.S > 1 && !d.fused;
+    d.needs_ws = d.S > 1 || (d.kernel == FwdKernel::Linear && !thin && S_gemm > 1);
     d.ws_query = d.ws_floats;
     if (d.kernel == FwdKernel::Stem && S_gemm > 1) d.ws_query = (int64_t)S_gemm * out_floats;
     if (is_gemm(d.kernel) && one_voxel) d.ws_query = 0;
@@ -2714,9 +2837,10 @@
 }
 
 template <int BM, int BN, int WAVES_CO, int BKT>
-static void launch_gemm_tile(const FwdLaunch& d, const GroupTable& tab, const float* wp, const float* bias, float* slab, int Cin,
-                             int Cout, int flags, hipStream_t s) {
-#define GEMM_LAUNCH(kernel, pad) T2V_LAUNCH_PROF(kernel, d.grid, d.block, pad, s, tab, wp, bias, slab, Cin, Cout, flags, d.S)
+static void launch_gemm_tile(const FwdLaunch& d, const GroupTable& tab, const float* wp, const float* bias, float* slab,
+                             unsigned int* ctr, int Cin, int Cout, int flags, hipStream_t s) {
+#define GEMM_LAUNCH(kernel, pad) T2V_LAUNCH_PROF(kernel, d.grid, d.block, pad, s, tab, wp, bias, slab, Cin, Cout, flags, d.S, ctr)
+#define GEMM_LAUNCH_F(name, ...) do { if (ctr) GEMM_LAUNCH((name<__VA_ARGS__, true>), 0); else GEMM_LAUNCH((name<__VA_ARGS__, false>), 0); } while (0)
     switch (d.kernel) {
     case FwdKernel::Strip3:
         if constexpr (BN == 64 && ((BM != 256 && BKT == 32) || (BM == 256 && BKT == 16))) {
@@ -2726,8 +2850,15 @@
                 if (d.db) { GEMM_LAUNCH((conv_igemm_strip3_kernel<256, 16, 1, true, true>), 0); return; }
             }
             if constexpr (BM == 64) {
-                if (d.db == 32) { GEMM_LAUNCH((conv_igemm_strip3_kernel<64, 32, 2, true, true>), 0); return; }
-                if (d.db == 16) { GEMM_LAUNCH((conv_igemm_strip3_kernel<64, 16, 2, true, true>), 0); return; }
+                if (d.db == 32) { GEMM_LAUNCH_F(conv_igemm_strip3_kernel, 64, 32, 2, true, true); return; }
+                if (d.db == 16) { GEMM_LAUNCH_F(conv_igemm_strip3_kernel, 64, 16, 2, true, true); return; }
+            }
+            if constexpr (BM != 256) {
+                if (ctr) {
+                    if (d.vecb) GEMM_LAUNCH((conv_igemm_strip3_kernel<BM, BKT, WCO3, true, false, true>), 0);
+                    else GEMM_LAUNCH((conv_igemm_strip3_kernel<BM, BKT, WCO3, false, false, true>), 0);
+                    return;
+                }
             }
             if (d.vecb) {
                 static OccInfo oi;
@@ -2740,15 +2871,24 @@
         return;
     case FwdKernel::Strip:
         if constexpr (BN == 32) {
-            if (d.vecb) GEMM_LAUNCH((conv_igemm_strip_kernel<BM, BN, WAVES_CO, BKT, true>), 0);
-            else GEMM_LAUNCH((conv_igemm_strip_kernel<BM, BN, WAVES_CO, BKT, false>), 0);
+            if (d.vecb) GEMM_LAUNCH_F(conv_igemm_strip_kernel, BM, BN, WAVES_CO, BKT, true);
+            else GEMM_LAUNCH_F(conv_igemm_strip_kernel, BM, BN, WAVES_CO, BKT, false);
         }
         return;
     default:
+        if constexpr (BM != 256) {
+            if (ctr) {
+                if (!d.fast) GEMM_LAUNCH((conv_igemm_kernel<BM, BN, WAVES_CO, 16, false, false, true>), 0);
+                else if (d.vecb) GEMM_LAUNCH((conv_igemm_kernel<BM, BN, WAVES_CO, BKT, true, true, true>), 0);
+                else GEMM_LAUNCH((conv_igemm_kernel<BM, BN, WAVES_CO, BKT, true, false, true>), 0);
+                return;
+            }
+        }
         if (!d.fast) GEMM_LAUNCH((conv_igemm_kernel<BM, BN, WAVES_CO, 16, false, false>), 0);
         else if (d.vecb) GEMM_LAUNCH((conv_igemm_kernel<BM, BN, WAVES_CO, BKT, true, true>), 0);
         else GEMM_LAUNCH((conv_igemm_kernel<BM, BN, WAVES_CO, BKT, true, false>), 0);
     }
+#undef GEMM_LAUNCH_F
 #undef GEMM_LAUNCH
 }
 
@@ -2773,6 +2913,7 @@
     fwd_plan_out(d, plan_);
     FwdKernel kernel = d.kernel;
     if (kernel == FwdKernel::ThinTwoPass && !ws) kernel = FwdKernel::Thin;
+    unsigned int* ctr = d.fused ? splitk_take((long)d.grid.x * d.grid.y) : nullptr;
     {
         ProfScope prof(is_gemm(kernel) ? 0 : 3, st.flops, s, st.rows, Cin, Cout, taps, ngroups, d.S);
         ProfScope::set_plan(plan_, 8);
@@ -2799,16 +2940,16 @@
             break;
         default:
             if (d.bn == 32) {
-                if (d.bk == 32) launch_gemm_tile<128, 32, 1, 32>(d, tab, wp, bias, ws, Cin, Cout, flags, s);
-                else launch_gemm_tile<128, 32, 1, 16>(d, tab, wp, bias, ws, Cin, Cout, flags, s);
+                if (d.bk == 32) launch_gemm_tile<128, 32, 1, 32>(d, tab, wp, bias, ws, ctr, Cin, Cout, flags, s);
+                else launch_gemm_tile<128, 32, 1, 16>(d, tab, wp, bias, ws, ctr, Cin, Cout, flags, s);
             } else if (d.bm == 256) {
-                launch_gemm_tile<256, 64, 1, 16>(d, tab, wp, bias, ws, Cin, Cout, flags, s);
+                launch_gemm_tile<256, 64, 1, 16>(d, tab, wp, bias, ws, ctr, Cin, Cout, flags, s);
             } else if (d.bm == 128) {
-                if (d.bk == 32) launch_gemm_tile<128, 64, 2, 32>(d, tab, wp, bias, ws, Cin, Cout, flags, s);
-                else launch_gemm_tile<128, 64, 2, 16>(d, tab, wp, bias, ws, Cin, Cout, flags, s);
+                if (d.bk == 32) launch_gemm_tile<128, 64, 2, 32>(d, tab, wp, bias, ws, ctr, Cin, Cout, flags, s);
+                else launch_gemm_tile<128, 64, 2, 16>(d, tab, wp, bias, ws, ctr, Cin, Cout, flags, s);
             } else {
-                if (d.bk == 32) launch_gemm_tile<64, 64, 2, 32>(d, tab, wp, bias, ws, Cin, Cout, flags, s);
-                else launch_gemm_tile<64, 64, 2, 16>(d, tab, wp, bias, ws, Cin, Cout, flags, s);
+                if (d.bk == 32) launch_gemm_tile<64, 64, 2, 32>(d, tab, wp, bias, ws, ctr, Cin, Cout, flags, s);
+                else launch_gemm_tile<64, 64, 2, 16>(d, tab, wp, bias, ws, ctr, Cin, Cout, flags, s);
             }
         }
     }
@@ -2817,7 +2958,7 @@
         T2V_LAUNCH_PROF(thin_shift_sum_kernel, d.grid, d.block, 0, s, tab, ws, bias, d.nslots, flags);
     }
     int st_ = launch_status();
-    if (st_ || !d.reduce) return st_;
+    if (st_ || d.S == 1 || ctr) return st_;
     launch_splitk_reduce(tab, ws, bias, d.S, Cin, Cout, flags, st, s);
     return launch_status();
 }
@@ -2837,6 +2978,7 @@
 struct Bf16Launch : ConvPlan {
     Bf16Kernel kernel;
     dim3 grid, block;
+    bool fused;
     bool reduce;
 };
 static bool decide_bf16(const t2v_conv_group* groups, int ngroups, int Cin, int Cout, int flags, bool need_ptrs, GroupTable& tab,
@@ -2854,7 +2996,8 @@
     d.kernel = strip3 ? Bf16Kernel::Strip3 : Bf16Kernel::Igemm;
     d.grid = dim3((unsigned)tab.tile_start[ngroups], (unsigned)((Cout + 63) / 64), (unsigned)d.S);
     d.block = dim3(256);
-    d.reduce = d.S > 1;
+    d.fused = splitk_fused(d.S, (long)d.grid.x * d.grid.y, d.bm, d.bn, tab.out_start[ngroups]);
+    d.reduce = d.S > 1 && !d.fused;
     return true;
 }
 static void bf16_plan_out(const Bf16Launch& d, int32_t* out) {
@@ -2878,23 +3021,29 @@
         for (int i = 0; i < ngroups; ++i)
             if (!groups[i].mask) return T2V_EINVAL;
     }
-    if (d.reduce && !ws) return T2V_EINVAL;
+    if (d.S > 1 && !ws) return T2V_EINVAL;
     hipStream_t s = (hipStream_t)stream;
     const FwdStats st = fwd_stats(groups, ngroups, Cin, Cout);
     const __bf16* w = (const __bf16*)wpb;
+    unsigned int* ctr = d.fused ? splitk_take((long)d.grid.x * d.grid.y) : nullptr;
     {
         ProfScope prof(5, st.flops, s, st.rows, Cin, Cout, st.taps, ngroups, d.S);
         int32_t plan_[8];
         bf16_plan_out(d, plan_);
         ProfScope::set_plan(plan_, 8);
+#define BF16_LAUNCH(name, BM_) do {                                                                                                          \
+            if (ctr) T2V_LAUNCH_PROF((name<BM_, true>), d.grid, d.block, 0, s, tab, w, bias, ws, Cin, Cout, flags, d.S, ctr);                     \
+            else T2V_LAUNCH_PROF((name<BM_, false>), d.grid, d.block, 0, s, tab, w, bias, ws, Cin, Cout, flags, d.S, ctr);                        \
+        } while (0)
         if (d.kernel == Bf16Kernel::Strip3) {
-            if (d.bm == 128) T2V_LAUNCH_PROF(conv_igemm_bf16_strip3_kernel<128>, d.grid, d.block, 0, s, tab, w, bias, ws, Cin, Cout, flags, d.S);
-            else T2V_LAUNCH_PROF(conv_igemm_bf16_strip3_kernel<64>, d.grid, d.block, 0, s, tab, w, bias, ws, Cin, Cout, flags, d.S);
-        } else if (d.bm == 128) T2V_LAUNCH_PROF(conv_igemm_bf16_kernel<128>, d.grid, d.block, 0, s, tab, w, bias, ws, Cin, Cout, flags, d.S);
-        else T2V_LAUNCH_PROF(conv_igemm_bf16_kernel<64>, d.grid, d.block, 0, s, tab, w, bias, ws, Cin, Cout, flags, d.S);
+            if (d.bm == 128) BF16_LAUNCH(conv_igemm_bf16_strip3_kernel, 128);
+            else BF16_LAUNCH(conv_igemm_bf16_strip3_kernel, 64);
+        } else if (d.bm == 128) BF16_LAUNCH(conv_igemm_bf16_kernel, 128);
+        else BF16_LAUNCH(conv_igemm_bf16_kernel, 64);
+#undef BF16_LAUNCH
     }
     int st_ = launch_status();
-    if (st_ || !d.reduce) return st_;
+    if (st_ || d.S == 1 || ctr) return st_;
     launch_splitk_reduce(tab, ws, bias, d.S, Cin, Cout, flags, st, s);
     return launch_status();
 }
@@ -4472,6 +4621,7 @@
     bool db;
     bool vecb;
     int S;
+    bool fused;
     long tiles;
     dim3 grid, block;
     int64_t ws_floats;
@@ -4531,6 +4681,7 @@
     d.grid = dim3((unsigned)mt, (unsigned)((Cout + 63) / 64), (unsigned)d.S);
     d.block = dim3(256);
     d.ws_floats = d.S > 1 ? (int64_t)d.S * ot : 0;
+    d.fused = splitk_fused(d.S, d.tiles, 64, 64, ot);
     return true;
 }
 static bool decide_pool_dgrad(const t2v_conv_group* groups, int ngroups, int K, int C, bool need_ptrs, GroupTable& tab, PoolLaunch& d) {
@@ -4646,16 +4797,19 @@
     if (d.S > 1 && !ws) return T2V_EINVAL;
     hipStream_t s = (hipStream_t)stream;
     const FwdStats st = fwd_stats(groups, ngroups, Cin, Cout, pool_rows);
+    unsigned int* ctr = d.fused ? splitk_take(d.tiles) : nullptr;
     {
         ProfScope prof(0, st.flops, s, st.rows, Cin, Cout, st.taps, ngroups, d.S);
         int32_t plan_[8];
         pool_plan_out(d, plan_);
         ProfScope::set_plan(plan_, 8);
-        if (d.db) T2V_LAUNCH_PROF((conv_pool_fwd_kernel<64, true>), d.grid, d.block, 0, s, tab, wp, bias, ws, Cin, Cout, flags, d.S);
-        else T2V_LAUNCH_PROF(conv_pool_fwd_kernel<64>, d.grid, d.block, 0, s, tab, wp, bias, ws, Cin, Cout, flags, d.S);
+        if (d.db && ctr) T2V_LAUNCH_PROF((conv_pool_fwd_kernel<64, true, true>), d.grid, d.block, 0, s, tab, wp, bias, ws, Cin, Cout, flags, d.S, ctr);
+        else if (d.db) T2V_LAUNCH_PROF((conv_pool_fwd_kernel<64, true>), d.grid, d.block, 0, s, tab, wp, bias, ws, Cin, Cout, flags, d.S, ctr);
+        else if (ctr) T2V_LAUNCH_PROF((conv_pool_fwd_kernel<64, false, true>), d.grid, d.block, 0, s, tab, wp, bias, ws, Cin, Cout, flags, d.S, ctr);
+        else T2V_LAUNCH_PROF(conv_pool_fwd_kernel<64>, d.grid, d.block, 0, s, tab, wp, bias, ws, Cin, Cout, flags, d.S, ctr);
     }
     int st_ = launch_status();
-    if (st_ || d.S == 1) return st_;
+    if (st_ || d.S == 1 || ctr) return st_;
     for (int i = 0; i < ngroups; ++i) {
         tab.g[i].D = groups[i].dstride ? groups[i].D / 2 : 1;
         tab.g[i].H = groups[i].H / 2;
diff --git a/txt2vid_amd/functional.py b/txt2vid_amd/functional.py
--- a/txt2vid_amd/functional.py
+++ b/txt2vid_amd/functional.py
@@ -1986,7 +1986,42 @@
     return _group_table(ins, outs, geoms, slot_of, masks, dstride), ts
 
 
+SPLITK_COUNTER_WORDS = 1 << 18
+_splitk_buf = {}
+_splitk_on = {}
+
+
+def _device_index(device):
+    device = torch.device(device)
+    return device.index if device.index is not None else torch.cuda.current_device()
+
+
+def splitk_fusion(device, on):
+    idx = _device_index(device)
+    with torch.cuda.device(idx):
+        if on and idx not in _splitk_buf:
+            if torch.cuda.is_current_stream_capturing():
+                return None
+            _splitk_buf[idx] = torch.zeros((SPLITK_COUNTER_WORDS,), device='cuda:%d' % idx, dtype=torch.int32)
+            torch.cuda.current_stream().synchronize()
+        buf = _splitk_buf.get(idx)
+        if on:
+            check(lib().t2v_splitk_counters(_p(buf), buf.numel()), 't2v_splitk_counters')
+        else:
+            check(lib().t2v_splitk_counters(None, 0), 't2v_splitk_counters')
+        _splitk_on[idx] = bool(on)
+    return buf
+
+
+def splitk_counters(device):
+    idx = _device_index(device)
+    if idx not in _splitk_on:
+        splitk_fusion(device, True)
+    return _splitk_buf.get(idx) if _splitk_on.get(idx) else None
+
+
 def _fwd_workspace(arr, n, cin, cout, device):
+    splitk_counters(device)
     nws = int(lib().t2v_conv_fwd_grouped_ws_floats(arr, n, cin, cout))
     if nws < 0:
         raise RuntimeError('bad grouped conv geometry')
diff --git a/txt2vid_amd/functional_pool.py b/txt2vid_amd/functional_pool.py
--- a/txt2vid_amd/functional_pool.py
+++ b/txt2vid_amd/functional_pool.py
@@ -118,6 +118,7 @@
         n, d, h, w_ = pooled_shape(sh, tm)
         zs.append(torch.empty((n, cout, d, h, w_), device=t.device, dtype=torch.float32))
     arr = _fwd_table(rts, zs, shapes, tmodes, ts)
+    TF.splitk_counters(rts[0].device)
     nws = int(lib().t2v_pool_conv_fwd_ws_floats(arr, len(rts), cin, cout))
     if nws < 0:
         raise RuntimeError('bad pooled-convolution geometry')
```

New measurement: 3092 videos/s (median of 6 runs). No clear change (+0.5%).
